# JoeyT1994/TensorNetworkQuantumSimulator.jl

Hardware: AMD Instinct MI355X
Metric: two-site gates/sec at fixed chi (LxL TFIM Trotter layer) (higher is better)
Workload: dtype c64 (ComplexF32; Gram/eigen steps in f64; the chi = 32 plane products as exact bf16 x 3 splits with f32 accumulation, TNQS_NO_BF16X3=1 for f32 matrix instructions)

## Files before the change

### include/tnqs_debug.h

```cpp
#ifndef TNQS_DEBUG_H
#define TNQS_DEBUG_H
#include <stdint.h>
#include "tnqs.h"
#ifdef __cplusplus
extern "C" {
#endif
int tnqs_dbg_jacobi(int dtype, int m, int n, void* A_inout, void* V_out, int* sweeps_out);
int tnqs_dbg_theta_svd_pre(int m, int n, int nq, void* A_inout, const void* Q, void* V_out, int* sweeps_out, int copies, int reps, double* ms_out, double* phase_us_out ,
                           int cap );
int tnqs_dbg_time_jacobi_f32(int m, int n, const void* A, int copies, int reps, double* ms_out, int* sweeps_out);
int tnqs_dbg_chol(int n, const void* G, void* L_out, void* W_out, int* fail_out, double tau);
int tnqs_dbg_fiber_gemm(int dtype, int D, int PA, int K, int PB, int Do, int No, const void* in, const void* X, void* out,
                        double* norm2_out, int use_mfma);
int tnqs_dbg_gram(int dtype, int D, int PA, int K, int PB, const void* X, const void* Y, void* out, int acc64, int use_mfma);
int tnqs_dbg_gram_fused(int PA, int K, int PB, const void* X, const void* Y, const void* M, void* out);
int tnqs_dbg_gauge_gram(int z, const int* chi, int bleg, const void* X, const void* M, void* out);
int tnqs_dbg_pair(int C0, int NMID, int NHI, const void* in, const void* Mx, const void* My, void* out);
int tnqs_dbg_pair_legs(int d, int z, const int* chi, int lx, int ly, const void* in, const void* Mx, const void* My, void* out);
int tnqs_dbg_pair_gram(int d, int z, const int* chi, int lx, int ly, const void* X, const void* Y, const void* M, void* out);
int tnqs_dbg_pair_gram2(int d, int z, const int* chi, int lx, int ly, const void* X, const void* Y, const void* Mx, const void* My, void* out_y, void* out_x);
int tnqs_dbg_bench_plane(int which, int nsites, int lx, int ly, int reps, double* ms);
#define TNQS_DBG_ROUTE_X3 1
#define TNQS_DBG_ROUTE_F32 2
#define TNQS_DBG_ROUTE_F64 3
#define TNQS_DBG_ROUTE_F64_SHARED 4
#define TNQS_DBG_ROUTE_HALF_LINES 5
#define TNQS_DBG_ROUTE_WHOLE_LINES 6
#define TNQS_DBG_ROUTE_SMALL_SCALAR 7
#define TNQS_DBG_ROUTE_SMALL_MFMA16 8
int tnqs_dbg_rowgemm(int D, int K, int nitems, const int* PA, const int* PB, const int* No, const void* in, const void* X, void* out, double* norm2_out,
                     int tpw, int* route_out);
int tnqs_dbg_gram_mfma(int nitems, const int* shape, const void* X, const void* Y, void* out, int nchunks, int* route_out);
int tnqs_dbg_pair16(int d, int nitems, const int* z, const int* chi, const int* lx, const int* ly, const void* in, const void* M, void* out, int spw, int* route_out);
int tnqs_dbg_pair_gram2x16(int d, int nitems, const int* z, const int* chi, const int* lx, const int* ly, const int* both, const void* X, const void* Y, const void* M,
                           void* out_y, void* out_x, int spw);
int tnqs_dbg_svd_tall(int nitems, const int* m, const int* n, void* A, int* chol_fail, int* polished, int* sweeps);
int tnqs_dbg_small_site(int nitems, const int* d, const int* z, const int* chi, const int* jo, const void* psi, const void* M, const int* present, int form,
                        const void* old_msg, const int* has_old, int normalize, void* out, void* new_msg, double* diff_out, int* route_out);
int tnqs_dbg_msg_finalize(int dtype, int nitems, const int* chi, const int* nchunks, const void* partials, const void* old_msg, const int* has_old, int normalize,
                          void* new_msg, double* diff_out);
int tnqs_dbg_default_sequence(tnqs_handle h, int* src, int* dst, int cap, int* n_out);
int tnqs_dbg_default_sequence_graph(int nv, int ne, const int32_t* esrc, const int32_t* edst, int* src, int* dst, int* level, int cap, int* n_out);
int tnqs_dbg_gate_schedule(int nv, int ne, const int32_t* esrc, const int32_t* edst, int ngates, const int32_t* nverts, const int32_t* verts, int update_cache,
                           int* step_of_gate, int* step_is_bp, int cap, int* nsteps_out);
int tnqs_dbg_loop_cgemm(int dtype, int opB, int nitems, const int* m, const int* n, const int* k, const void* A, const void* B, void* C, int guard);
int tnqs_dbg_loop_antiproject(int dtype, int nitems, const int* nr, const int* nc, void* T_inout, const void* f, const void* b);
int tnqs_dbg_loop_trace(int dtype, int nitems, const int* p, const int* q, const void* X, const void* Y, double* out_re_im);
int tnqs_dbg_msg_rescale(int dtype, int nitems, const int* chi, const void* me, const void* mer, const int* present, void* me_out, void* mer_out, int guard);
int tnqs_dbg_edge_scalar(int dtype, int nitems, const int* chi, const void* me, const void* mer, const int* present, double* out_re_im);
int tnqs_dbg_env_prepare(int dtype, int nitems, const int* n, const void* msg, const int* present, void* H_out, void* V_out, int guard);
int tnqs_dbg_env_finish(int dtype, int nitems, const int* n, const void* A, const void* V, const double* cutoff, void* msqrt_out, void* proj_out, int* flags_out, int guard);
int tnqs_dbg_symg_build(int dtype, int nitems, const int* n, const void* AX, const void* VX, const void* AY, const void* VY, double reg, void* rx, void* ry, void* irx, void* iry,
                        void* Ce, void* Ce0, int* flag_out, int guard);
int tnqs_dbg_symg_finish(int dtype, int nitems, const int* n, const void* USigma, const void* Vsvd, const void* irx, const void* iry, void* Xs, void* Xd, double* S, int guard);
int tnqs_dbg_diag(int dtype, int nitems, const int* chi, const double* S, void* out, int guard);
int tnqs_dbg_cscale(int dtype, int nitems, const int* len, const void* src, const double* re, const double* im, void* dst, int guard);
int tnqs_dbg_pending_scale(tnqs_handle h, int v, double* factor);
#ifdef __cplusplus
}
#endif
#endif
```

### tensornetworkquantumsimulator.jl_amd/csrc/api.cpp

```cpp
#include <cmath>
#include <cstring>
#include <string>
#include "engine.hpp"

using namespace tnqs;

struct tnqs_state_s { State* s; };

static thread_local std::string g_err;

template <class F> static int guard(F&& f) {
    try { f(); return TNQS_OK; }
    catch (const Err& e) { g_err = e.what(); return e.code; }
    catch (const std::bad_alloc&) { g_err = "out of host memory"; return TNQS_ERR_HIP; }
    catch (const std::exception& e) { g_err = e.what(); return TNQS_ERR_INVALID; }
    catch (...) { g_err = "unknown error"; return TNQS_ERR_INVALID; }
}
static State* S(tnqs_handle h) { if (!h || !h->s) throw Err(TNQS_ERR_INVALID, "null handle"); return h->s; }

extern "C" {

int tnqs_version(void) { return 102; }
const char* tnqs_last_error(void) { return g_err.c_str(); }
int tnqs_device_count(int* count) {
// ... 208 lines not shown
    return guard([&] { if (nv < 0 || ne < 0 || (ne > 0 && (!esrc || !edst)) || !n_out) throw Err(TNQS_ERR_INVALID, "tnqs_dbg_default_sequence_graph: bad arguments");
                       auto g = dbg_make_graph(nv, ne, esrc, edst); std::vector<int> a, b, l; dbg_default_sequence_graph(*g, a, b, l); *n_out = (int)a.size();
                       for (int i = 0; i < (int)a.size() && i < cap; ++i) { if (src) src[i] = a[i]; if (dst) dst[i] = b[i]; if (level) level[i] = l[i]; } });
}
int tnqs_dbg_gate_schedule(int nv, int ne, const int32_t* esrc, const int32_t* edst, int ngates, const int32_t* nverts, const int32_t* verts, int update_cache,
                           int* step_of_gate, int* step_is_bp, int cap, int* nsteps_out) {
    return guard([&] { if (nv < 0 || ne < 0 || (ne > 0 && (!esrc || !edst)) || ngates < 0 || (ngates > 0 && (!nverts || !verts)) || !nsteps_out) throw Err(TNQS_ERR_INVALID, "tnqs_dbg_gate_schedule: bad arguments");
                       for (int i = 0, o = 0; i < ngates; o += nverts[i], ++i) { if (nverts[i] < 1 || nverts[i] > 2) throw Err(TNQS_ERR_INVALID, "tnqs_dbg_gate_schedule: only one- and two-site gates");
                                                                                 for (int k = 0; k < nverts[i]; ++k) if (verts[o + k] < 0 || verts[o + k] >= nv) throw Err(TNQS_ERR_INVALID, "tnqs_dbg_gate_schedule: vertex out of range"); }
                       auto g = dbg_make_graph(nv, ne, esrc, edst); const GateSchedule steps = build_gate_schedule(*g, ngates, nverts, verts, update_cache != 0); *nsteps_out = (int)steps.size();
                       for (int k = 0; k < (int)steps.size(); ++k) { if (step_is_bp && k < cap) step_is_bp[k] = steps[k].is_bp ? 1 : 0; if (step_of_gate) for (int i = steps[k].begin; i < steps[k].end; ++i) step_of_gate[i] = k; } });
}
int tnqs_dbg_jacobi(int dtype, int m, int n, void* A, void* V, int* sweeps) { return guard([&] { dbg_jacobi(dtype, m, n, A, V, sweeps); }); }
int tnqs_dbg_theta_svd_pre(int m, int n, int nq, void* A, const void* Q, void* V, int* sweeps, int copies, int reps, double* ms, double* phase_us, int cap) { return guard([&] { dbg_theta_svd_pre(m, n, nq, A, Q, V, sweeps, copies, reps, ms, phase_us, cap); }); }
int tnqs_dbg_time_jacobi_f32(int m, int n, const void* A, int copies, int reps, double* ms, int* sweeps) { return guard([&] { dbg_time_jacobi_f32(m, n, A, copies, reps, ms, sweeps); }); }
int tnqs_dbg_chol(int n, const void* G, void* L, void* W, int* fail, double tau) { return guard([&] { dbg_chol(n, G, L, W, fail, tau); }); }
int tnqs_dbg_fiber_gemm(int dtype, int D, int PA, int K, int PB, int Do, int No, const void* in, const void* X, void* out, double* norm2, int use_mfma) {
    return guard([&] { dbg_fiber_gemm(dtype, D, PA, K, PB, Do, No, in, X, out, norm2, use_mfma); });
}
int tnqs_dbg_pair(int C0, int NMID, int NHI, const void* in, const void* Mx, const void* My, void* out) { return guard([&] { dbg_pair(C0, NMID, NHI, in, Mx, My, out); }); }
int tnqs_dbg_pair_legs(int d, int z, const int* chi, int lx, int ly, const void* in, const void* Mx, const void* My, void* out) { return guard([&] { dbg_pair_legs(d, z, chi, lx, ly, in, Mx, My, out); }); }
int tnqs_dbg_pair_gram2(int d, int z, const int* chi, int lx, int ly, const void* X, const void* Y, const void* Mx, const void* My, void* out_y, void* out_x) {
    return guard([&] { dbg_pair_gram2(d, z, chi, lx, ly, X, Y, Mx, My, out_y, out_x); });
}
int tnqs_dbg_bench_plane(int which, int nsites, int lx, int ly, int reps, double* ms) { return guard([&] { dbg_bench_plane(which, nsites, lx, ly, reps, ms); }); }
int tnqs_dbg_pair_gram(int d, int z, const int* chi, int lx, int ly, const void* X, const void* Y, const void* M, void* out) { return guard([&] { dbg_pair_gram(d, z, chi, lx, ly, X, Y, M, out); }); }
int tnqs_dbg_gram_fused(int PA, int K, int PB, const void* X, const void* Y, const void* M, void* out) { return guard([&] { dbg_gram_fused(PA, K, PB, X, Y, M, out); }); }
int tnqs_dbg_gauge_gram(int z, const int* chi, int bleg, const void* X, const void* M, void* out) { return guard([&] { dbg_gauge_gram(z, chi, bleg, X, M, out); }); }
int tnqs_dbg_gram(int dtype, int D, int PA, int K, int PB, const void* X, const void* Y, void* out, int acc64, int use_mfma) {
    return guard([&] { dbg_gram(dtype, D, PA, K, PB, X, Y, out, acc64, use_mfma); });
}
int tnqs_dbg_rowgemm(int D, int K, int nitems, const int* PA, const int* PB, const int* No, const void* in, const void* X, void* out, double* norm2_out, int tpw, int* route_out) {
    return guard([&] { dbg_rowgemm(D, K, nitems, PA, PB, No, in, X, out, norm2_out, tpw, route_out); });
}
int tnqs_dbg_gram_mfma(int nitems, const int* shape, const void* X, const void* Y, void* out, int nchunks, int* route_out) {
    return guard([&] { dbg_gram_mfma(nitems, shape, X, Y, out, nchunks, route_out); });
}
int tnqs_dbg_pair16(int d, int nitems, const int* z, const int* chi, const int* lx, const int* ly, const void* in, const void* M, void* out, int spw, int* route_out) {
    return guard([&] { dbg_pair16(d, nitems, z, chi, lx, ly, in, M, out, spw, route_out); });
}
int tnqs_dbg_pair_gram2x16(int d, int nitems, const int* z, const int* chi, const int* lx, const int* ly, const int* both, const void* X, const void* Y, const void* M,
                           void* out_y, void* out_x, int spw) {
    return guard([&] { dbg_pair_gram2x16(d, nitems, z, chi, lx, ly, both, X, Y, M, out_y, out_x, spw); });
}
int tnqs_dbg_svd_tall(int nitems, const int* m, const int* n, void* A, int* chol_fail, int* polished, int* sweeps) {
    return guard([&] { dbg_svd_tall(nitems, m, n, A, chol_fail, polished, sweeps); });
}
int tnqs_dbg_small_site(int nitems, const int* d, const int* z, const int* chi, const int* jo, const void* psi, const void* M, const int* present, int form,
                        const void* old_msg, const int* has_old, int normalize, void* out, void* new_msg, double* diff_out, int* route_out) {
    return guard([&] { dbg_small_site(nitems, d, z, chi, jo, psi, M, present, form, old_msg, has_old, normalize, out, new_msg, diff_out, route_out); });
}
int tnqs_dbg_msg_finalize(int dtype, int nitems, const int* chi, const int* nchunks, const void* partials, const void* old_msg, const int* has_old, int normalize,
                          void* new_msg, double* diff_out) {
    return guard([&] { dbg_msg_finalize(dtype, nitems, chi, nchunks, partials, old_msg, has_old, normalize, new_msg, diff_out); });
}
int tnqs_dbg_loop_cgemm(int dtype, int opB, int nitems, const int* m, const int* n, const int* k, const void* A, const void* B, void* C, int guard_elems) {
    return guard([&] { dbg_loop_cgemm(dtype, opB, nitems, m, n, k, A, B, C, guard_elems); });
}
int tnqs_dbg_loop_antiproject(int dtype, int nitems, const int* nr, const int* nc, void* T, const void* f, const void* b) { return guard([&] { dbg_loop_antiproject(dtype, nitems, nr, nc, T, f, b); }); }
int tnqs_dbg_loop_trace(int dtype, int nitems, const int* p, const int* q, const void* X, const void* Y, double* out) { return guard([&] { dbg_loop_trace(dtype, nitems, p, q, X, Y, out); }); }
int tnqs_dbg_msg_rescale(int dtype, int nitems, const int* chi, const void* me, const void* mer, const int* present, void* me_out, void* mer_out, int guard_elems) {
    return guard([&] { dbg_msg_rescale(dtype, nitems, chi, me, mer, present, me_out, mer_out, guard_elems); });
}
int tnqs_dbg_edge_scalar(int dtype, int nitems, const int* chi, const void* me, const void* mer, const int* present, double* out_re_im) {
    return guard([&] { dbg_edge_scalar(dtype, nitems, chi, me, mer, present, out_re_im); });
}
int tnqs_dbg_env_prepare(int dtype, int nitems, const int* n, const void* msg, const int* present, void* H_out, void* V_out, int guard_elems) {
    return guard([&] { dbg_env_prepare(dtype, nitems, n, msg, present, H_out, V_out, guard_elems); });
}
int tnqs_dbg_env_finish(int dtype, int nitems, const int* n, const void* A, const void* V, const double* cutoff, void* msqrt_out, void* proj_out, int* flags_out, int guard_elems) {
    return guard([&] { dbg_env_finish(dtype, nitems, n, A, V, cutoff, msqrt_out, proj_out, flags_out, guard_elems); });
}
int tnqs_dbg_symg_build(int dtype, int nitems, const int* n, const void* AX, const void* VX, const void* AY, const void* VY, double reg, void* rx, void* ry, void* irx, void* iry,
                        void* Ce, void* Ce0, int* flag_out, int guard_elems) {
    return guard([&] { dbg_symg_build(dtype, nitems, n, AX, VX, AY, VY, reg, rx, ry, irx, iry, Ce, Ce0, flag_out, guard_elems); });
}
int tnqs_dbg_symg_finish(int dtype, int nitems, const int* n, const void* USigma, const void* Vsvd, const void* irx, const void* iry, void* Xs, void* Xd, double* S, int guard_elems) {
    return guard([&] { dbg_symg_finish(dtype, nitems, n, USigma, Vsvd, irx, iry, Xs, Xd, S, guard_elems); });
}
int tnqs_dbg_diag(int dtype, int nitems, const int* chi, const double* S, void* out, int guard_elems) { return guard([&] { dbg_diag(dtype, nitems, chi, S, out, guard_elems); }); }
int tnqs_dbg_cscale(int dtype, int nitems, const int* len, const void* src, const double* re, const double* im, void* dst, int guard_elems) {
    return guard([&] { dbg_cscale(dtype, nitems, len, src, re, im, dst, guard_elems); });
}
int tnqs_dbg_pending_scale(tnqs_handle h, int v, double* factor) { return guard([&] { if (!factor) throw Err(TNQS_ERR_INVALID, "dbg_pending_scale: null output"); *factor = dbg_pending_scale(S(h), v); }); }
}
```

### tensornetworkquantumsimulator.jl_amd/csrc/engine.hpp

```cpp
#pragma once
#include <hip/hip_runtime_api.h>
#include <climits>
#include <cstdint>
#include <deque>
#include <functional>
#include <map>
#include <memory>
#include <mutex>
#include <stdexcept>
#include <string>
#include <unordered_map>
#include <vector>
#include "../../include/tnqs.h"

namespace tnqs {

struct Err : std::runtime_error {
    int code;
    Err(int c, const std::string& m) : std::runtime_error(m), code(c) {}
};
void hipchk(hipError_t e, const char* what);

class Pool {
public:
// ... 27 lines not shown
    std::vector<std::vector<int>> levels;
    std::vector<int> pos_of;
    std::vector<int> level_of;
    bool in_place = false;
    int nlev = 0;
    std::vector<std::vector<int>> out_level, in_level;
    int levels_until(int L, int from) const { return L > from ? L - from : (L < from ? nlev - from + L : 0); }
    int levels_until_next(int L, int from) const { return L > from ? L - from : nlev - from + L; }
    int horizon(int src, int j, int t) const { const int L = in_level[src][j]; return L < 0 ? INT_MAX : levels_until(L, level_of[t]); }
};

struct Graph {
    int nv = 0, ne = 0;
    std::vector<int> esrc, edst;
    std::vector<std::vector<int>> nbr, nbr_e;
    std::unordered_map<uint64_t, int> emap;
    bool is_tree = false;
    std::vector<int> ecolor; int ncolors = 0;
    mutable std::vector<int> default_seq;
    mutable std::vector<int> default_set_starts;
    mutable std::shared_ptr<const BPPlan> default_plan;
    mutable std::shared_ptr<const BPPlan> forest_plan;
    mutable int spec_penalty = 0;
    int edge(int u, int v) const;
    int leg(int v, int w) const;
    int dedge(int src, int dst) const;
    int src_of(int de) const { return (de & 1) ? edst[de / 2] : esrc[de / 2]; }
    int dst_of(int de) const { return (de & 1) ? esrc[de / 2] : edst[de / 2]; }
};
std::shared_ptr<const BPPlan> plan_for(const Graph& g, const tnqs_bp_opts* o);

struct GateStep { bool is_bp; int begin, end; };
using GateSchedule = std::vector<GateStep>;
struct State;
void validate_gates(const State& s, int ngates, const int32_t* nverts, const int32_t* verts, std::vector<int>& voff, std::vector<size_t>& moff);
GateSchedule build_gate_schedule(const Graph& g, int ngates, const int32_t* nverts, const int32_t* verts, bool update_cache);

struct ProfClass { int64_t launches = 0; double ms = 0, bytes = 0, flops = 0; };
struct Prof {
    bool on = false; ProfClass cls[TNQS_PROF_NCLASSES];
    struct Pending { int cls; hipEvent_t a, b; bool own_a; };
    std::vector<Pending> pending; std::vector<hipEvent_t> ev_free;
    hipEvent_t last_b = nullptr; bool chain = false; hipStream_t last_stream = nullptr;
    ~Prof() { for (auto& p : pending) { if (p.own_a) (void)hipEventDestroy(p.a); (void)hipEventDestroy(p.b); } for (auto e : ev_free) (void)hipEventDestroy(e); }
};

struct RcclComm {
    void* comm = nullptr; int device = 0; void* exch_owned = nullptr;
    long long n_exchanges = 0, bytes_exchanged = 0;
    ~RcclComm();
};

constexpr int kCheckEvents = 16;
struct HostArena {
    char* base = nullptr; size_t cap = 0, off = 0;
    char* ring = nullptr; size_t ring_cap = 0, ring_off = 0;
    hipEvent_t cev[kCheckEvents] = {}; unsigned cevn = 0;
};

struct Check {
    int kind = 0;
    int step = 0;
    int iters_done = 0;
    hipEvent_t ev = nullptr;
    std::function<bool(State*)> eval;
};

struct State {
    std::shared_ptr<Graph> g;
    int dtype = TNQS_C64;
    bool real_io = false;
    int device = 0;
    std::vector<int> d;
    std::vector<char> projected;
    std::vector<int> chi;
    std::vector<Buf> site;
    std::vector<Buf> sscale;
    std::vector<std::vector<double>> pend1; std::vector<char> unit_norm;
    bool in_apply = false;
    std::vector<Buf> msg;
    std::shared_ptr<Pool> pool;
    hipStream_t stream = nullptr; bool own_stream = false;
    hipStream_t aux_stream = nullptr; hipEvent_t ev_fork = nullptr, ev_join = nullptr;
    int rank = 0, nranks = 1; std::vector<int> owner; tnqs_allgather_fn ag_fn = nullptr; void* ag_ctx = nullptr;
    void* exch = nullptr; size_t exch_bytes = 0;
    std::shared_ptr<RcclComm> comm;
    std::shared_ptr<Prof> prof;
    std::vector<Buf> keepalive;
    size_t keep_mark = 0;
    HostArena arena;
    tnqs_apply_stats stats{};
    std::deque<Check> checks;
    int cur_step = -1;

    size_t esz() const { return dtype == TNQS_C64 ? 8 : 16; }
    int scalartype() const { return real_io ? (dtype == TNQS_C64 ? TNQS_F32 : TNQS_F64) : dtype; }
    size_t io_esz() const { return real_io ? esz() / 2 : esz(); }
    bool owns(int v) const { return nranks == 1 || owner[v] == rank; }
    bool force_exchange = false;
    bool msg_hermitian = true;
    bool sharded() const { return nranks > 1 || force_exchange; }
    ~State();
};

State* state_create(int nv, int ne, const int32_t* es, const int32_t* ed, const int32_t* sd, int dtype, int device);
State* state_copy(const State* s);
void state_set_site(State* s, int v, const void* host, int ndim, const int64_t* dims, const int32_t* role);
void state_get_site(State* s, int v, void* host, int ndim, const int32_t* role);
void state_set_site_random(State* s, int v, int nn, const int64_t* bond_dims, uint64_t seed, double scale);
int64_t state_site_size(const State* s, int v);
void state_set_message(State* s, int src, int dst, const void* host, int chi);
void state_get_message(State* s, int src, int dst, void* host, int chi);
void bp_update(State* s, const tnqs_bp_opts* opts, int* niter, double* diff);
void apply_gates(State* s, int ngates, const int32_t* nverts, const int32_t* verts, const double* mats,
                 const tnqs_apply_opts* opts, const tnqs_bp_opts* bp, double* errs);
void truncate_bp(State* s, int maxdim, double cutoff, int normalize, int ngroups, const int32_t* offs,
                 const int32_t* eu, const int32_t* ev, const tnqs_bp_opts* bp);
void rdm_1site(State* s, int v, double* out);
void expect_all(State* s, const double* ops, double* out);
void expect_region(State* s, int nr, const int32_t* rv, const int32_t* parent, const double* ops, double* out4);
void vertex_scalars(State* s, double* out);
void edge_scalars(State* s, double* out);
void rescale(State* s);
void rescale_messages(State* s, int n, const int32_t* eu, const int32_t* ev);
void rescale_vertices(State* s, int n, const int32_t* verts);
void symmetric_gauge(State* s, double regularization);
void site_dim(const State* s, int v, int* d);
void project_site(State* s, int v, int config);
void site_probabilities(State* s, int v, double* out_p);
void sample_bp(State* s, int nsamples, const tnqs_bp_opts* bp, uint64_t seed, const double* uniforms, int32_t* out_config, double* out_prob, tnqs_apply_stats* stats);
void loop_weights(State* s, int ncycles, const int32_t* cycle_len, const int32_t* cycle_verts, double* out_re_im);
void prof_collect(State* s);
void materialize_pending_all(State* s);
void rccl_unique_id(void* out128);
void set_sharding_rccl(State* s, int rank, int nranks, const int32_t* owner, const void* unique_id128, int64_t exch_bytes);
void rccl_allgather(State* s, size_t bytes_per_rank);
void rccl_selftest(int device, int64_t bytes);
void rccl_preflight();

}
```

### tensornetworkquantumsimulator.jl_amd/csrc/engine_batch.cpp

```cpp
#include "engine_internal.hpp"

namespace tnqs {

template <class T> void run_chains(State* s, std::vector<Chain>& chains, int cls, int cls_pair) {
    if (cls_pair < 0) cls_pair = cls;
    const size_t esz = s->esz();
    std::vector<int> nt(chains.size(), 0);
    std::vector<size_t> done(chains.size(), 0);
    for (auto& c : chains) c.result = c.src;
    if (std::is_same<T, float>::value && use_mfma() && use_pair()) {
        std::vector<PairItem> items; double bytes = 0, flops = 0;
        std::vector<std::pair<size_t, std::pair<int, int>>> sel;
        for (size_t ci = 0; ci < chains.size(); ++ci) {
            Chain& c = chains[ci];
            if (c.steps.size() < 2) continue;
            int py = -1, px = -1;
            for (int q = (int)c.steps.size() - 1; q >= 0 && px < 0; --q) {
                int leg = c.steps[q].first;
                bool ok = c.sd.chi[leg] == 32 && leg >= 1 && (c.sd.pre(leg) % 16 == 0);
                if (!ok) continue;
                if (py < 0) py = q; else px = q;
            }
            if (px < 0) continue;
            sel.push_back({ci, {px, py}});
// ... 114 lines not shown
        }
        const int tiles = plan_fiber_gemm(items.data(), (int)items.size(), TR, mf ? tpw : 1);
        const FiberItem* d = upload(s, items);
        ProfScope ps(s, cls, bytes, flops);
        if (mf) launch_mfma_fiber_gemm(s->stream, d, (int)items.size(), tiles, (int)KKmax, (int)KKmax, nullptr);
        else launch_fiber_gemm<T>(s->stream, d, (int)items.size(), tiles, TR, (int)KKmax, nullptr);
    }
    (void)done;
}

void svd_tall(State* s, const std::vector<JacobiItem>& tall, int* d_fail_out, int* d_polish_sweeps) {
    const size_t esz = sizeof(float) * 2;
    const size_t nt = tall.size();
    size_t off = 0; std::vector<size_t> oG(nt), oL(nt), oW(nt), oR0(nt), oRr(nt), oJ(nt), oT(nt);
    for (size_t i = 0; i < nt; ++i) {
        const size_t nn = (size_t)tall[i].n * tall[i].n, mn = (size_t)tall[i].m * tall[i].n;
        oG[i] = off; off += round256(nn * 16); oL[i] = off; off += round256(nn * 16); oW[i] = off; off += round256(nn * 16);
        oR0[i] = off; off += round256(nn * 8); oRr[i] = off; off += round256(nn * 8); oJ[i] = off; off += round256(nn * 16); oT[i] = off; off += round256(mn * 8);
    }
    Buf arena = dalloc(s, off); s->keepalive.push_back(arena);
    Buf fail_buf; if (!d_fail_out) { fail_buf = dalloc(s, nt * sizeof(int)); s->keepalive.push_back(fail_buf); }
    int* const d_fail = d_fail_out ? d_fail_out : reinterpret_cast<int*>(fail_buf->p);
    HIPCHK(hipMemsetAsync(d_fail, 0, nt * sizeof(int), s->stream));
    char* ap = reinterpret_cast<char*>(arena->p);
    std::vector<TallSvdItem> ti, wi; std::vector<CholItem> ci; std::vector<JacobiItem> rj; std::vector<SmallGemmItem> gi; std::vector<CopyItem> cp;
    int nmax = 1, mmax = 1;
    for (size_t i = 0; i < nt; ++i) {
        const int m = tall[i].m, n = tall[i].n; nmax = std::max(nmax, n); mmax = std::max(mmax, m);
        ti.push_back(TallSvdItem{tall[i].A, ap + oG[i], ap + oL[i], ap + oR0[i], ap + oRr[i], m, n});
        ci.push_back(CholItem{ap + oG[i], ap + oL[i], ap + oW[i], n, d_fail + i, 0.0, 1e-14});
        rj.push_back(JacobiItem{ap + oRr[i], nullptr, n, n, tall[i].sweeps_out});
        wi.push_back(TallSvdItem{nullptr, d_fail + i, ap + oW[i], ap + oJ[i], ap + oRr[i], n, n});
        gi.push_back(SmallGemmItem{tall[i].A, ap + oJ[i], ap + oT[i], m, n, n});
        cp.push_back(CopyItem{ap + oT[i], tall[i].A, (size_t)m * n * 8 / 16});
    }
    const TallSvdItem* dt = upload(s, ti); const CholItem* dc = upload(s, ci); const JacobiItem* dj = upload(s, rj);
    const TallSvdItem* dw = upload(s, wi); const SmallGemmItem* dg = upload(s, gi); const CopyItem* dcp = upload(s, cp);
    launch_tall_gram(s->stream, dt, (int)nt, nmax);
    launch_chol_packed(s->stream, dc, (int)nt, nmax);
    launch_tall_rt(s->stream, dt, (int)nt);
    size_t lds = 0; for (auto& j : rj) lds = std::max(lds, jacobi_lds_bytes(j.m, j.n, false, esz));
    launch_jacobi<float>(s->stream, dj, (int)nt, 60, lds, nmax);
    launch_tall_w(s->stream, dw, (int)nt, nmax);
    launch_tall_mj(s->stream, dg, (int)nt);
    launch_copy_items(s->stream, dcp, (int)nt);
    std::vector<JacobiItem> pol;
    for (size_t i = 0; i < nt; ++i) { JacobiItem j{tall[i].A, nullptr, tall[i].m, tall[i].n, d_polish_sweeps ? d_polish_sweeps + i : nullptr}; j.only_if = d_fail + i; pol.push_back(j); }
    const JacobiItem* dp = upload(s, pol);
    launch_jacobi<float>(s->stream, dp, (int)nt, 60, 0, mmax);
    s->stats.n_tall_svd += (int)nt;
}

template <class T> void svd_batch(State* s, const std::vector<JacobiItem>& all, bool with_v) {
    const size_t esz = s->esz();
    const size_t cap = 160 * 1024 - 2048;
    std::vector<JacobiItem> fit, tall, rest, pre;
    static const bool force_global = [] { const char* e = std::getenv("TNQS_JACOBI_GLOBAL"); return e && e[0] == '1'; }();
    for (auto& j : all) {
        if (j.n < 1 || j.m < 1) continue;
        if (j.pre) pre.push_back(j);
        if (!force_global && jacobi_lds_bytes(j.m, j.n, with_v, esz) <= cap && std::max(j.m, j.n) <= 256) fit.push_back(j);
        else if (!force_global && std::is_same<T, float>::value && !with_v && !j.V && use_mfma() && use_chi64() && j.m >= j.n && j.n <= 128 && j.n >= 2 &&
                 jacobi_lds_bytes(j.n, j.n, false, esz) <= cap) tall.push_back(j);
        else rest.push_back(j);
    }
    if (!pre.empty()) {
        const JacobiItem* d = upload_small(s, pre);
        int mm = 1, nn = 1; for (auto& j : pre) { mm = std::max(mm, std::min(j.m, 128)); nn = std::max(nn, std::min(j.n, 64)); }
        launch_theta_svd_pre(s->stream, d, (int)pre.size(), 60, mm, nn);
    }
    if (!fit.empty()) {
        size_t lds = 0; for (auto& j : fit) lds = std::max(lds, jacobi_lds_bytes(j.m, j.n, with_v, esz));
        const JacobiItem* d = upload_small(s, fit);
        int ncols = 1; for (auto& j : fit) ncols = std::max(ncols, j.nhint > 0 ? j.nhint : j.n);
        launch_jacobi<T>(s->stream, d, (int)fit.size(), 60, lds, mmax_of(fit), ncols);
    }
    if (!rest.empty()) {
        const JacobiItem* d = upload(s, rest);
        launch_jacobi<T>(s->stream, d, (int)rest.size(), 60, 0, mmax_of(rest));
    }
    if (!tall.empty()) svd_tall(s, tall);
}

template <class T, class Acc> void run_grams(State* s, std::vector<GramJob>& jobs, int cls) {
    if (jobs.empty()) return;
    const size_t esz = s->esz();
    size_t KKmax = 1;
    for (auto& j : jobs) { j.KK = (j.keep_site ? j.sd.d : 1) * (j.leg >= 0 ? j.sd.chi[j.leg] : 1); KKmax = std::max<size_t>(KKmax, j.KK); }
    constexpr bool f32 = std::is_same<T, float>::value, f32_acc64 = f32 && std::is_same<Acc, double>::value, acc32 = std::is_same<Acc, float>::value;
    bool same = true, f64in = std::is_same<T, double>::value && use_mfma();
    for (auto& j : jobs) { same = same && j.X == j.Y; f64in = f64in && j.M == nullptr && gram_f64in_covers(j.keep_site ? j.sd.d : 1, j.leg >= 0 ? j.sd.chi[j.leg] : 1); }
    GramRoute r = GramRoute::Generic;
    if (jobs[0].M) r = f32_acc64 ? (KKmax == 32 ? GramRoute::Gauge32 : GramRoute::Gauge64) : GramRoute::Fused32;
    else if (f32_acc64 && use_mfma() && same && KKmax <= 64 && KKmax >= 16) r = GramRoute::F64x64;
    else if (f32_acc64 && use_mfma() && use_chi64() && same && KKmax <= 128 && KKmax > 64) r = GramRoute::F64x128;
    else if (f64in) r = GramRoute::F64In;
    else if (f32 && acc32 && use_mfma() && KKmax <= (use_chi64() ? 64 : 32) && KKmax >= 8) r = KKmax <= 32 ? GramRoute::Mfma32 : GramRoute::Mfma64;
    const bool gauge = r == GramRoute::Gauge32 || r == GramRoute::Gauge64;
    const int TR = gram_tile_rows(r, KKmax, esz);
    std::vector<GramItem> items; double bytes = 0, flops = 0; bool all_full = true;
    for (auto& j : jobs) {
        GramItem it{};
        it.X = j.X; it.Y = j.Y; it.M = j.M;
        if (j.leg >= 0) {
            size_t pre = j.sd.pre(j.leg);
            if (j.keep_site) { it.D = j.sd.d; it.PA = (int)(pre / j.sd.d); } else { it.D = 1; it.PA = (int)pre; }
            it.K = j.sd.chi[j.leg]; it.PB = (int)j.sd.post(j.leg);
        } else { it.D = j.sd.d; it.PA = (int)(j.sd.n / j.sd.d); it.K = 1; it.PB = 1; }
        tile_params(it.PA, it.PB, TR, it.TA, it.TB, it.nta, it.ntb);
        if (r == GramRoute::Gauge32) { it.nta = gauge_gram32_units(j.sd.z, j.sd.chi.data(), j.leg); it.ntb = 1; }
        items.push_back(it);
        all_full = all_full && j.KK == (r == GramRoute::F64x128 ? 128 : 64);
        bytes += (j.X == j.Y ? 1.0 : 2.0) * j.sd.n * esz; flops += gauge ? 8.0 * j.sd.n * (j.KK + (r == GramRoute::Gauge32 ? 16.0 : 32.0)) : 8.0 * j.sd.n * j.KK * (j.M ? 2.0 : 1.0);
    }
    std::vector<int> npart(jobs.size());
    const int chunks = plan_gram(items.data(), (int)items.size(), r, f32_acc64, 0, npart.data());
    for (size_t q = 0; q < jobs.size(); ++q) {
        GramJob& j = jobs[q];
        j.nchunks = npart[q];
        j.partial = dalloc(s, (size_t)j.nchunks * j.KK * j.KK * 2 * sizeof(Acc));
        items[q].partial = j.partial->p;
    }
    const GramItem* d = upload(s, items);
    ProfScope ps(s, cls, bytes, flops);
    launch_gram_route<T, Acc>(s->stream, r, d, (int)items.size(), chunks, TR, (int)KKmax, all_full);
}

template void run_chains<float>(State*, std::vector<Chain>&, int, int);
template void run_chains<double>(State*, std::vector<Chain>&, int, int);
template void svd_batch<float>(State*, const std::vector<JacobiItem>&, bool);
template void svd_batch<double>(State*, const std::vector<JacobiItem>&, bool);
template void run_grams<float, float>(State*, std::vector<GramJob>&, int);
template void run_grams<float, double>(State*, std::vector<GramJob>&, int);
template void run_grams<double, double>(State*, std::vector<GramJob>&, int);

}
```

### tensornetworkquantumsimulator.jl_amd/csrc/engine_core.cpp

```cpp
#include "engine_internal.hpp"

namespace tnqs {

double HostTimer::acc[16] = {0}; long HostTimer::cnt[16] = {0};
static struct HostTimerReport { ~HostTimerReport() { if (envflag("TNQS_HOST_TIMING")) for (int k = 0; k < 16; ++k) if (HostTimer::cnt[k])
    std::fprintf(stderr, "[tnqs host timing] phase %d: %.2f ms total, %ld calls, %.1f us each\n", k, HostTimer::acc[k], HostTimer::cnt[k], 1e3 * HostTimer::acc[k] / HostTimer::cnt[k]); } } g_host_timer_report;

void hipchk(hipError_t e, const char* what) {
    if (e != hipSuccess) throw Err(TNQS_ERR_HIP, std::string(what) + ": " + hipGetErrorString(e));
}
void throw_unsupported(const char* what) { throw Err(TNQS_ERR_UNSUPPORTED, what); }

static size_t round_size(size_t b) {
    if (b < 256) return 256;
    if (b <= (1u << 20)) return (b + 255) & ~size_t(255);
    size_t p = size_t(1) << (63 - __builtin_clzll(b));
    size_t step = p >> 3;
    return (b + step - 1) / step * step;
}
Pool::~Pool() { set_defer(false); trim(); }
void Pool::trim() {
    std::lock_guard<std::mutex> lk(mu_);
    for (auto& kv : free_) for (void* p : kv.second) (void)hipFree(p);
    free_.clear(); cached_ = 0;
// ... 32 lines not shown
    const auto& n = nbr[v];
    auto it = std::lower_bound(n.begin(), n.end(), w);
    return (it != n.end() && *it == w) ? int(it - n.begin()) : -1;
}
int Graph::dedge(int src, int dst) const { int e = edge(src, dst); if (e < 0) return -1; return 2 * e + (src == edst[e] ? 1 : 0); }

static std::shared_ptr<Graph> make_graph(int nv, int ne, const int32_t* es, const int32_t* ed) {
    auto g = std::make_shared<Graph>();
    g->nv = nv; g->ne = ne; g->esrc.assign(es, es + ne); g->edst.assign(ed, ed + ne);
    g->nbr.resize(nv); g->nbr_e.resize(nv);
    for (int e = 0; e < ne; ++e) {
        int a = es[e], b = ed[e];
        if (a < 0 || a >= nv || b < 0 || b >= nv || a == b) throw Err(TNQS_ERR_INVALID, "tnqs_create: bad edge endpoints");
        if (g->emap.count(ekey(a, b))) throw Err(TNQS_ERR_INVALID, "tnqs_create: duplicate edge");
        g->emap[ekey(a, b)] = e;
    }
    for (int v = 0; v < nv; ++v) {
        std::vector<std::pair<int, int>> tmp;
        for (int e = 0; e < ne; ++e) { if (es[e] == v) tmp.push_back({ed[e], e}); else if (ed[e] == v) tmp.push_back({es[e], e}); }
        std::sort(tmp.begin(), tmp.end());
        for (auto& p : tmp) { g->nbr[v].push_back(p.first); g->nbr_e[v].push_back(p.second); }
    }
    std::vector<int> par(nv); std::iota(par.begin(), par.end(), 0);
    auto find = [&](int x) { while (par[x] != x) { par[x] = par[par[x]]; x = par[x]; } return x; };
    g->is_tree = true;
    for (int e = 0; e < ne; ++e) { int a = find(es[e]), b = find(ed[e]); if (a == b) { g->is_tree = false; break; } par[a] = b; }
    g->ecolor.assign(ne, -1);
    std::vector<std::vector<char>> used(nv);
    for (int e = 0; e < ne; ++e) {
        int a = es[e], b = ed[e], c = 0;
        for (;; ++c) {
            bool ua = c < (int)used[a].size() && used[a][c], ub = c < (int)used[b].size() && used[b][c];
            if (!ua && !ub) break;
        }
        if ((int)used[a].size() <= c) used[a].resize(c + 1, 0);
        if ((int)used[b].size() <= c) used[b].resize(c + 1, 0);
        used[a][c] = used[b][c] = 1; g->ecolor[e] = c; g->ncolors = std::max(g->ncolors, c + 1);
    }
    return g;
}

std::shared_ptr<Graph> dbg_make_graph(int nv, int ne, const int32_t* es, const int32_t* ed) { return make_graph(nv, ne, es, ed); }

static std::mutex g_recycle_mu;
static std::vector<HostArena> g_spare_arenas;
struct SpareStream { int device; int hi; hipStream_t st; };
static std::vector<SpareStream> g_spare_streams;
static const size_t kMaxSpares = 16;
HostArena acquire_arena() {
    HostArena ar{};
    { std::lock_guard<std::mutex> lk(g_recycle_mu); if (!g_spare_arenas.empty()) { ar = g_spare_arenas.back(); g_spare_arenas.pop_back(); ar.off = 0; ar.ring_off = 0; } }
    if (!ar.base) {
        static const size_t cap = [] { const char* e = std::getenv("TNQS_ARENA_KB"); return e ? std::max<size_t>(16, (size_t)std::atoll(e)) << 10 : size_t(32) << 20; }();
        const size_t ring = size_t(2) << 20;
        HIPCHK(hipHostMalloc((void**)&ar.base, cap + ring, hipHostMallocDefault)); ar.cap = cap - 256;
        ar.ring = ar.base + cap; ar.ring_cap = ring; ar.ring_off = 0;
    }
    return ar;
}
static void arena_free(HostArena& ar) {
    for (hipEvent_t& e : ar.cev) if (e) { (void)hipEventDestroy(e); e = nullptr; }
    if (ar.base) { (void)hipHostFree(ar.base); ar.base = nullptr; }
}
void recycle_arena(HostArena ar) {
    if (!ar.base) return;
    { std::lock_guard<std::mutex> lk(g_recycle_mu); if (g_spare_arenas.size() < kMaxSpares) { ar.off = 0; ar.ring_off = 0; g_spare_arenas.push_back(ar); ar.base = nullptr; } }
    if (ar.base) arena_free(ar);
}
static hipStream_t acquire_stream(int device, int hi = 0) {
    {
        std::lock_guard<std::mutex> lk(g_recycle_mu);
        for (size_t i = 0; i < g_spare_streams.size(); ++i)
            if (g_spare_streams[i].device == device && g_spare_streams[i].hi == hi) { hipStream_t st = g_spare_streams[i].st; g_spare_streams.erase(g_spare_streams.begin() + (std::ptrdiff_t)i); return st; }
    }
    hipStream_t st = nullptr;
    if (hi) { int least = 0, greatest = 0; HIPCHK(hipDeviceGetStreamPriorityRange(&least, &greatest)); HIPCHK(hipStreamCreateWithPriority(&st, hipStreamNonBlocking, greatest)); }
    else HIPCHK(hipStreamCreateWithFlags(&st, hipStreamNonBlocking));
    return st;
}

State::~State() {
    if (own_stream && stream) (void)hipStreamSynchronize(stream);
    if (aux_stream) (void)hipStreamSynchronize(aux_stream);
    keepalive.clear(); site.clear(); msg.clear();
    HostArena ar = arena; arena = HostArena{};
    SpareStream st[2] = {{device, 0, (own_stream && stream) ? stream : nullptr}, {device, 0, aux_stream}};
    {
        std::lock_guard<std::mutex> lk(g_recycle_mu);
        if (ar.base && g_spare_arenas.size() < kMaxSpares) { ar.off = 0; g_spare_arenas.push_back(ar); ar.base = nullptr; }
        for (auto& q : st) if (q.st && g_spare_streams.size() < kMaxSpares) { g_spare_streams.push_back(q); q.st = nullptr; }
    }
    if (ar.base) arena_free(ar);
    for (auto& q : st) if (q.st) (void)hipStreamDestroy(q.st);
    for (hipEvent_t e : {ev_fork, ev_join}) if (e) (void)hipEventDestroy(e);
}
hipStream_t aux_stream_of(State* s) {
    if (!s->aux_stream) {
        s->aux_stream = acquire_stream(s->device);
        HIPCHK(hipEventCreateWithFlags(&s->ev_fork, hipEventDisableTiming));
        HIPCHK(hipEventCreateWithFlags(&s->ev_join, hipEventDisableTiming));
    }
    return s->aux_stream;
}
void sync(State* s) {
    HIPCHK(hipStreamSynchronize(s->stream));
    s->keepalive.clear(); s->keep_mark = 0;
    s->arena.off = 0;
    if (s->prof) s->prof->chain = false;
}

void prof_collect(State* s) {
    Prof& P = *s->prof;
    if (P.pending.empty()) return;
    HIPCHK(hipStreamSynchronize(s->stream));
    for (auto& p : P.pending) {
        float ms = 0; (void)hipEventElapsedTime(&ms, p.a, p.b);
        P.cls[p.cls].ms += ms;
    }
    for (auto& p : P.pending) { if (p.own_a) P.ev_free.push_back(p.a); P.ev_free.push_back(p.b); }
    P.pending.clear(); P.last_b = nullptr; P.chain = false;
}

int64_t state_site_size(const State* s, int v) { return (int64_t)site_dims(s, v).n; }

template <class T> static void fill_product_up(State* s, int v) {
    std::vector<T> h(2 * s->d[v], T(0)); h[0] = T(1);
    Buf b = dalloc(s, s->d[v] * s->esz());
    HIPCHK(hipMemcpyAsync(b->p, h.data(), s->d[v] * s->esz(), hipMemcpyHostToDevice, s->stream));
    HIPCHK(hipStreamSynchronize(s->stream));
    s->site[v] = b;
}

State* state_create(int nv, int ne, const int32_t* es, const int32_t* ed, const int32_t* sd, int dtype, int device) {
    if (nv <= 0 || ne < 0) throw Err(TNQS_ERR_INVALID, "tnqs_create: nv must be > 0 and ne >= 0");
    if (dtype != TNQS_C64 && dtype != TNQS_C128 && dtype != TNQS_F32 && dtype != TNQS_F64) throw Err(TNQS_ERR_INVALID, "tnqs_create: unknown dtype");
    const bool real_io = (dtype == TNQS_F32 || dtype == TNQS_F64);
    if (dtype == TNQS_F32) dtype = TNQS_C64; else if (dtype == TNQS_F64) dtype = TNQS_C128;
    int ndev = 0;
    if (hipGetDeviceCount(&ndev) != hipSuccess || ndev <= 0) throw Err(TNQS_ERR_HIP, "tnqs_create: no HIP device available (the HIP path has no CPU fallback)");
    if (device < 0 || device >= ndev) throw Err(TNQS_ERR_INVALID, "tnqs_create: bad device index");
    HIPCHK(hipSetDevice(device));
    auto s = std::make_unique<State>();
    s->g = make_graph(nv, ne, es, ed);
    s->dtype = dtype; s->real_io = real_io; s->device = device;
    s->d.assign(nv, 2);
    if (sd) for (int v = 0; v < nv; ++v) { if (sd[v] < 1 || sd[v] > 16) throw Err(TNQS_ERR_INVALID, "tnqs_create: site dimension out of range"); s->d[v] = sd[v]; }
    s->chi.assign(ne, 1);
    s->site.resize(nv); s->sscale.assign(nv, nullptr); s->msg.assign(2 * (size_t)ne, nullptr);
    s->pend1.assign(nv, {}); s->unit_norm.assign(nv, 0); s->projected.assign(nv, 0);
    s->pool = std::make_shared<Pool>(device);
    s->prof = std::make_shared<Prof>();
    s->stream = acquire_stream(device); s->own_stream = true;
    for (int v = 0; v < nv; ++v) { if (dtype == TNQS_C64) fill_product_up<float>(s.get(), v); else fill_product_up<double>(s.get(), v); }
    return s.release();
}

State* state_copy(const State* o) {
    auto s = std::make_unique<State>();
    s->g = o->g; s->dtype = o->dtype; s->real_io = o->real_io; s->device = o->device; s->d = o->d; s->chi = o->chi;
    s->site = o->site; s->sscale = o->sscale; s->msg = o->msg; s->pool = o->pool; s->prof = o->prof;
    s->pend1 = o->pend1; s->unit_norm = o->unit_norm; s->projected = o->projected;
    s->rank = o->rank; s->nranks = o->nranks; s->owner = o->owner; s->ag_fn = o->ag_fn; s->ag_ctx = o->ag_ctx;
    s->exch = o->exch; s->exch_bytes = o->exch_bytes; s->comm = o->comm; s->force_exchange = o->force_exchange; s->msg_hermitian = o->msg_hermitian;
    HIPCHK(hipSetDevice(o->device));
    if (o->own_stream) { HIPCHK(hipStreamSynchronize(o->stream)); s->stream = acquire_stream(o->device); s->own_stream = true; }
    else { s->stream = o->stream; s->own_stream = false; }
    return s.release();
}

template <class T> static void permute_dispatch(State* s, const PermItem& it) { launch_permute<T>(s->stream, it); }

static std::vector<char> widen_real(const State* s, const void* host, size_t n) {
    std::vector<char> out(n * s->esz());
    if (s->dtype == TNQS_C64) { const float* p = static_cast<const float*>(host); float* q = reinterpret_cast<float*>(out.data()); for (size_t i = 0; i < n; ++i) { q[2 * i] = p[i]; q[2 * i + 1] = 0.f; } }
    else { const double* p = static_cast<const double*>(host); double* q = reinterpret_cast<double*>(out.data()); for (size_t i = 0; i < n; ++i) { q[2 * i] = p[i]; q[2 * i + 1] = 0.0; } }
    return out;
}
// ... 146 lines not shown
```

### tensornetworkquantumsimulator.jl_amd/csrc/engine_gates.cpp

```cpp
#include "engine_internal.hpp"

namespace tnqs {

struct Gate1 { int v; const double* mat; };
struct Gate2 { int v1, v2; const double* mat; int index; };

template <class T> static void materialize_scale_t(State* s, const std::vector<int>& verts) {
    std::vector<ScaleItem> sc; std::vector<Buf> outs; std::vector<int> vs;
    for (int v : verts) {
        if (v < 0 || v >= (int)s->site.size() || !s->site[v] || !s->sscale[v]) continue;
        Buf out = dalloc(s, s->site[v]->bytes);
        ScaleItem it{}; it.src = s->site[v]->p; it.dst = out->p; it.n = s->site[v]->bytes / s->esz(); it.factor = reinterpret_cast<const double*>(s->sscale[v]->p);
        sc.push_back(it); outs.push_back(out); vs.push_back(v);
    }
    if (sc.empty()) return;
    HIPCHK(hipSetDevice(s->device));
    const ScaleItem* d = upload(s, sc);
    { ProfScope ps(s, TNQS_PROF_SMALL, 0, 0); launch_scale<T>(s->stream, d, (int)sc.size()); }
    for (size_t i = 0; i < vs.size(); ++i) { s->keepalive.push_back(s->site[vs[i]]); s->keepalive.push_back(s->sscale[vs[i]]); s->site[vs[i]] = outs[i]; s->sscale[vs[i]] = nullptr; }
}
void materialize_scale(State* s, const std::vector<int>& verts) {
    if (s->dtype == TNQS_C64) materialize_scale_t<float>(s, verts); else materialize_scale_t<double>(s, verts);
}
void materialize_scale_all(State* s) {
    std::vector<int> all(s->site.size()); std::iota(all.begin(), all.end(), 0);
    materialize_scale(s, all);
}
template <class T> static void apply_one_site_batch(State* s, const std::vector<Gate1>& gates_in, bool normalize, bool force);
void materialize_pending(State* s, const std::vector<int>& verts) {
    std::vector<std::vector<double>> mats; std::vector<Gate1> gs; std::vector<char> norm_was;
    for (int v : verts) {
        if (v < 0 || v >= (int)s->pend1.size() || s->pend1[v].empty()) continue;
        mats.push_back(std::move(s->pend1[v])); s->pend1[v].clear(); norm_was.push_back(s->unit_norm[v]);
        gs.push_back(Gate1{v, nullptr});
    }
    if (gs.empty()) return;
    for (size_t k = 0; k < gs.size(); ++k) gs[k].mat = mats[k].data();
    HIPCHK(hipSetDevice(s->device));
    if (s->dtype == TNQS_C64) apply_one_site_batch<float>(s, gs, false, true); else apply_one_site_batch<double>(s, gs, false, true);
    for (size_t k = 0; k < gs.size(); ++k) s->unit_norm[gs[k].v] = norm_was[k];
}
void materialize_pending_all(State* s) {
    std::vector<int> all(s->site.size()); std::iota(all.begin(), all.end(), 0);
    materialize_pending(s, all);
}

template <class T> static void norm_and_replace(State* s, const std::vector<int>& verts, const std::vector<Buf>& outs, const Buf& norm_partials,
                                                const std::vector<int>& tile_begin, const std::vector<int>& ntiles, bool normalize) {
    if (normalize) {
        std::vector<NormFactorItem> nf;
        Buf fac = dalloc(s, verts.size() * 256);
        for (size_t i = 0; i < verts.size(); ++i) {
            NormFactorItem it{}; it.norm_partials = reinterpret_cast<const double*>(norm_partials->p) + tile_begin[i]; it.npart = ntiles[i];
            it.factor = reinterpret_cast<double*>(reinterpret_cast<char*>(fac->p) + 256 * i);
            nf.push_back(it);
        }
        const NormFactorItem* d = upload_small(s, nf);
        { ProfScope ps(s, TNQS_PROF_SMALL, 0, 0); launch_norm_factor(s->stream, d, (int)nf.size()); }
        for (size_t i = 0; i < verts.size(); ++i) { s->site[verts[i]] = outs[i]; s->sscale[verts[i]] = sub_buffer(fac, 256 * i, 8); }
    } else {
        for (size_t i = 0; i < verts.size(); ++i) s->site[verts[i]] = outs[i];
    }
}

static bool is_unitary(const double* m, int d, double tol) {
    for (int a = 0; a < d; ++a) for (int b = 0; b < d; ++b) {
        double re = 0, im = 0;
        for (int t = 0; t < d; ++t) { const double* x = m + 2 * (t + d * a); const double* y = m + 2 * (t + d * b); re += x[0] * y[0] + x[1] * y[1]; im += x[0] * y[1] - x[1] * y[0]; }
        if (std::fabs(re - (a == b ? 1.0 : 0.0)) > tol || std::fabs(im) > tol) return false;
    }
    return true;
}
static std::vector<double> matmul_dd(const double* a, const double* b, int d) {
    std::vector<double> c(2 * (size_t)d * d, 0.0);
    for (int i = 0; i < d; ++i) for (int j = 0; j < d; ++j) {
        double re = 0, im = 0;
        for (int t = 0; t < d; ++t) { const double* x = a + 2 * (i + d * t); const double* y = b + 2 * (t + d * j); re += x[0] * y[0] - x[1] * y[1]; im += x[0] * y[1] + x[1] * y[0]; }
        c[2 * (i + d * j)] = re; c[2 * (i + d * j) + 1] = im;
    }
    return c;
}

template <class T> static void apply_one_site_batch(State* s, const std::vector<Gate1>& gates_in, bool normalize, bool force) {
    if (gates_in.empty()) return;
    const size_t esz = s->esz();
    std::vector<std::vector<double>> composed; composed.reserve(gates_in.size());
    std::vector<Gate1> gates;
    const bool may_defer = !force && defer_site1() && (!s->sharded() || s->in_apply);
    const double utol = s->dtype == TNQS_C64 ? 1e-6 : 1e-13;
    for (auto& g1 : gates_in) {
        const int d = s->d[g1.v];
        std::vector<double>& pend = s->pend1[g1.v];
        if (may_defer && is_unitary(g1.mat, d, utol) && (!normalize || s->unit_norm[g1.v])) {
            pend = pend.empty() ? std::vector<double>(g1.mat, g1.mat + 2 * (size_t)d * d) : matmul_dd(g1.mat, pend.data(), d);
            s->stats.n_deferred_1site += 1;
            continue;
        }
        if (!pend.empty()) { composed.push_back(matmul_dd(g1.mat, pend.data(), d)); pend.clear(); gates.push_back(Gate1{g1.v, composed.back().data()}); }
        else gates.push_back(g1);
        s->unit_norm[g1.v] = normalize ? 1 : 0;
    }
    if (gates.empty()) return;
    if (std::is_same<T, float>::value) {
        bool all2 = true; for (auto& g1 : gates) all2 = all2 && s->d[g1.v] == 2;
        if (all2) {
            const int NBX = 64;
            std::vector<Site1Item> items; std::vector<int> verts, tb, nt; std::vector<Buf> outs; double bytes = 0, flops = 0;
            for (auto& g1 : gates) {
                if (!s->owns(g1.v)) continue;
                SD sd = site_dims(s, g1.v);
                Site1Item it{}; Buf out = dalloc(s, sd.n * esz);
                it.in = s->site[g1.v]->p; it.out = out->p; it.npairs = sd.n / 2;
                const double* m = g1.mat;
                it.g[0] = (float)m[0]; it.g[1] = (float)m[1]; it.g[2] = (float)m[4]; it.g[3] = (float)m[5];
                it.g[4] = (float)m[2]; it.g[5] = (float)m[3]; it.g[6] = (float)m[6]; it.g[7] = (float)m[7];
                verts.push_back(g1.v); outs.push_back(out); tb.push_back((int)items.size() * NBX); nt.push_back(NBX);
                items.push_back(it);
                bytes += 2.0 * sd.n * esz; flops += 8.0 * sd.n * 2;
            }
            if (items.empty()) return;
            Buf np = dalloc(s, items.size() * NBX * sizeof(double));
            const Site1Item* d = upload(s, items);
            { ProfScope ps(s, TNQS_PROF_GATE_APPLY, bytes, flops);
              launch_site1_c64(s->stream, d, (int)items.size(), NBX, normalize ? reinterpret_cast<double*>(np->p) : nullptr); }
            norm_and_replace<T>(s, verts, outs, np, tb, nt, normalize);
            return;
        }
    }
    std::vector<FiberItem> items; std::vector<int> verts, tb, nt; std::vector<Buf> outs;
    size_t KKmax = 1; double bytes = 0, flops = 0;
    for (auto& g1 : gates) KKmax = std::max<size_t>(KKmax, s->d[g1.v]);
    const int TR = pick_TR(KKmax, esz, 1);
    std::vector<T> hx;
    std::vector<size_t> xoff;
    for (auto& g1 : gates) {
        int d = s->d[g1.v]; xoff.push_back(hx.size());
        for (int nn = 0; nn < d; ++nn) for (int kk = 0; kk < d; ++kk) { hx.push_back((T)g1.mat[2 * (nn + d * kk)]); hx.push_back((T)g1.mat[2 * (nn + d * kk) + 1]); }
    }
    const char* dxp;
    {
        std::vector<char> raw(reinterpret_cast<char*>(hx.data()), reinterpret_cast<char*>(hx.data()) + hx.size() * sizeof(T));
        dxp = upload(s, raw);
    }
    size_t gi = 0;
// ... 15 lines not shown
    const FiberItem* d = upload(s, items);
    { ProfScope ps(s, TNQS_PROF_GATE_APPLY, bytes, flops);
      launch_fiber_gemm<T>(s->stream, d, (int)items.size(), tiles, TR, (int)KKmax, reinterpret_cast<double*>(np->p)); }
    norm_and_replace<T>(s, verts, outs, np, tb, nt, normalize);
}

static std::vector<Gate2> absorb_pending(const State* s, const std::vector<Gate2>& gates_in, std::vector<std::vector<double>>& absorbed) {
    absorbed.reserve(gates_in.size());
    std::vector<Gate2> gates = gates_in;
    for (auto& g2 : gates) {
        const std::vector<double>& p1 = s->pend1[g2.v1]; const std::vector<double>& p2 = s->pend1[g2.v2];
        if (p1.empty() && p2.empty()) continue;
        const int d1 = s->d[g2.v1], d2 = s->d[g2.v2], dd = d1 * d2;
        std::vector<double> kron(2 * (size_t)dd * dd, 0.0);
        for (int t1 = 0; t1 < d1; ++t1) for (int s1 = 0; s1 < d1; ++s1) for (int t2 = 0; t2 < d2; ++t2) for (int s2 = 0; s2 < d2; ++s2) {
            const double ar = p1.empty() ? (t1 == s1 ? 1.0 : 0.0) : p1[2 * (t1 + d1 * s1)], ai = p1.empty() ? 0.0 : p1[2 * (t1 + d1 * s1) + 1];
            const double br = p2.empty() ? (t2 == s2 ? 1.0 : 0.0) : p2[2 * (t2 + d2 * s2)], bi = p2.empty() ? 0.0 : p2[2 * (t2 + d2 * s2) + 1];
            const size_t e = (size_t)(t1 * d2 + t2) + (size_t)dd * (s1 * d2 + s2);
            kron[2 * e] = ar * br - ai * bi; kron[2 * e + 1] = ar * bi + ai * br;
        }
        absorbed.push_back(matmul_dd(g2.mat, kron.data(), dd));
        g2.mat = absorbed.back().data();
    }
    return gates;
}

static int operator_sum(const double* mat, int d1, int d2, std::vector<std::complex<double>>& fa, std::vector<std::complex<double>>& fb) {
    const int dd = d1 * d2, na = d1 * d1, nb = d2 * d2;
    std::vector<std::complex<double>> O((size_t)na * nb);
    const std::complex<double>* gm = reinterpret_cast<const std::complex<double>*>(mat);
    double amax = 0;
    for (int s1p = 0; s1p < d1; ++s1p) for (int s1 = 0; s1 < d1; ++s1) for (int s2p = 0; s2p < d2; ++s2p) for (int s2 = 0; s2 < d2; ++s2) {
        auto v = gm[(s1p * d2 + s2p) + (size_t)dd * (s1 * d2 + s2)];
        O[(s1p + d1 * s1) + (size_t)na * (s2p + d2 * s2)] = v; amax = std::max(amax, std::abs(v));
    }
    int kp = 0;
    for (; kp < std::min(na, nb); ++kp) {
        int pi = 0, pj = 0; double best = 0;
        for (int j = 0; j < nb; ++j) for (int i = 0; i < na; ++i) { double a = std::abs(O[i + (size_t)na * j]); if (a > best) { best = a; pi = i; pj = j; } }
        if (!(best > 1e-13 * amax)) break;
        const std::complex<double> piv = O[pi + (size_t)na * pj];
        std::vector<std::complex<double>> col(na), row(nb);
        for (int i = 0; i < na; ++i) col[i] = O[i + (size_t)na * pj];
        for (int j = 0; j < nb; ++j) row[j] = O[pi + (size_t)na * j] / piv;
        for (int j = 0; j < nb; ++j) for (int i = 0; i < na; ++i) O[i + (size_t)na * j] -= col[i] * row[j];
        fa.insert(fa.end(), col.begin(), col.end()); fb.insert(fb.end(), row.begin(), row.end());
    }
    return kp;
}

struct ReadBack {
    size_t info = 0, low = 0, low2 = 0, terr = 0, chol = 0, env = 0, total = 0;
    ReadBack(size_t ngates, size_t nsites, size_t nflags)
        : low(round256(ngates * 32)), low2(low + round256(ngates * 4)), terr(low2 + round256(ngates * 4)), chol(terr + round256(ngates * 8)),
          env(chol + round256(nsites * sizeof(int))), total(env + round256(nflags * sizeof(int))) {}
    const int* info_of(const char* st) const { return reinterpret_cast<const int*>(st + info); }
    const double* terr_of(const char* st) const { return reinterpret_cast<const double*>(st + terr); }
    const int* chol_of(const char* st) const { return reinterpret_cast<const int*>(st + chol); }
    const int* env_of(const char* st) const { return reinterpret_cast<const int*>(st + env); }
};

struct GateBook {
    int index, cap, d1, d2, K, chi_cap; bool low;
    void book(tnqs_apply_stats& st, const int* hi) const {
        int Mr, Nc, ncolJ; theta_dims(hi, d1, d2, Mr, Nc, ncolJ);
        st.n_lowrank_svd += (ncolJ < Nc) ? 1 : 0; st.n_svd_sweeps += hi[4]; st.n_svd_sweeps_max = std::max(st.n_svd_sweeps_max, hi[4]);
        const int r1d = hi[0] * d1, r2d = hi[1] * d2;
        if (low && ncolJ == Nc && r1d >= r2d && K < r2d && chi_cap <= K) st.n_lowrank_fallbacks += 1;
    }
};

template <class T> static void launch_small_svd(hipStream_t st, const SmallSvdItem* ds, const JacobiItem* dj, const std::vector<JacobiItem>& sji) {
    launch_small_svd_prepare<T>(st, ds, (int)sji.size());
    size_t lds = 0; for (auto& j : sji) lds = std::max(lds, jacobi_lds_bytes(j.m, j.n, false, 16));
    launch_jacobi<double>(st, dj, (int)sji.size(), 60, jacobi_lds(lds), mmax_of(sji));
    launch_small_svd_finish(st, ds, (int)sji.size());
}
template <class T> static void launch_eigen_from_identity(State* s, const EnvItem* di, const JacobiItem* dj, const std::vector<JacobiItem>& ji) {
    size_t lds = 0; for (auto& j : ji) lds = std::max(lds, jacobi_lds_bytes(j.n, j.n, true, 16));
    { ProfScope ps(s, TNQS_PROF_SMALL, 0, 0); launch_env_prepare<T>(s->stream, di, (int)ji.size()); }
    { ProfScope ps(s, TNQS_PROF_JACOBI, 0, 0); launch_jacobi<double>(s->stream, dj, (int)ji.size(), 60, jacobi_lds(lds), mmax_of(ji)); }
}

enum class ReadRoute { deferred, one_trip, two_trips };

template <class T> struct TwoSiteBatch {
    static constexpr bool F32 = std::is_same<T, float>::value;
    struct SiteJob { int v, other, bleg; bool owned; SD sd; std::vector<int> env_idx; std::vector<int> env_leg; };
    struct EnvRec { int de; int n; void *H, *V, *msq, *prj; };
    struct GateWS { Buf lam1, lam2, idx1, idx2, theta, thetaV, theta0, X1, X2, S, lowA, lowB, lowG, lowL, lowW, lowQ, lowB1, lowG2, lowL2, lowLc; int n1, n2, chi, cap; };
    struct RgGroup { int kk = 0; std::vector<FiberItem> sub; std::vector<int> sv, stb, snt; std::vector<Buf> so; int wgs = 0; Buf npr; const FiberItem* d = nullptr; };
    struct RgPlan { bool valid = false; std::vector<RgGroup> groups; std::vector<char> via; double rby = 0, rfl = 0; };

    State* s; const Graph& g; const tnqs_apply_opts& ao; double* errs;
    const size_t esz; const bool sharded;
    const bool qr2;
    bool may_defer = false; double sqrt_cutoff = 0;
    std::vector<std::vector<double>> absorbed; std::vector<Gate2> gates; int ng;
    std::vector<SiteJob> sj; std::vector<char> part;
    std::vector<EnvRec> envs; Buf env_arena;
    std::vector<int> own_idx;
    std::vector<Chain> chains; std::vector<const void*> fused_M, gauged_of; std::vector<GramJob> jobs;
    std::vector<Buf> GA, GV, GW; std::vector<char> is_chol, is_small, small_done;
    hipEvent_t ev_small = nullptr;
    std::vector<size_t> slot; size_t stride = 0; std::vector<char> cross;
    ReadBack rb{0, 0, 0}; Buf d_rb, d_texp; const char* st_all = nullptr;
    std::vector<int> h_flags, h_cholfail, hinfo, info; std::vector<double> hterr, terr;
    std::vector<GateWS> ws; std::vector<int> pg; int npg = 0;
    std::vector<GateItem> gitems; const GateItem* d_gitems = nullptr; bool lowrank_on_batch = false; int cap_max = 1; size_t x2_max = 0;
    ReadRoute route = ReadRoute::two_trips;
    RgPlan spec_plan;
    std::vector<const double*> Sptr; Buf S_keep;
    std::vector<Chain> pch;

    TwoSiteBatch(State* st, const std::vector<Gate2>& gates_in, const tnqs_apply_opts& o, double* e, bool allow_spec)
        : s(st), g(*st->g), ao(o), errs(e), esz(st->esz()), sharded(st->sharded()), qr2(!F32 && use_qr2()), ng((int)gates_in.size()) {
        may_defer = allow_spec && !sharded && ao.maxdim > 0 && !qr2;
        for (size_t k = 0; k < gates_in.size() && may_defer; ++k) {
            const int v1 = gates_in[k].v1, v2 = gates_in[k].v2; const int chi = s->chi[g.edge(v1, v2)];
            const int Mr = std::max(s->d[v1], s->d[v2]) * std::max(s->d[v1], s->d[v2]) * chi, Nc = std::min(s->d[v1], s->d[v2]) * std::min(s->d[v1], s->d[v2]) * chi;
            may_defer = chi == ao.maxdim && Nc >= chi && Mr <= 256 && jacobi_lds(jacobi_lds_bytes(Mr, Nc, false, esz)) > 0;
        }
        sqrt_cutoff = ao.sqrt_cutoff >= 0 ? ao.sqrt_cutoff : 10.0 * (s->dtype == TNQS_C64 ? 1.1920928955078125e-07 : 2.220446049250313e-16);
        gates = absorb_pending(s, gates_in, absorbed);
    }
    ~TwoSiteBatch() { if (ev_small) (void)hipStreamWaitEvent(s->stream, ev_small, 0); }

    int nof(size_t i) const { return sj[i].sd.d * sj[i].sd.chi[sj[i].bleg]; }
    bool small_shape(size_t i) const { const int n = nof(i); return sj[i].sd.n / (size_t)n < (size_t)n && n <= 256 && use_small_svd(); }
    template <class X> X* dev(size_t off) const { return reinterpret_cast<X*>(reinterpret_cast<char*>(d_rb->p) + off); }
    GateBook book_of(int q) const { const GateItem& it = gitems[q]; return GateBook{gates[pg[q]].index, ws[pg[q]].cap, it.d1, it.d2, it.kappa * it.chi, it.chi_cap, it.lowG != nullptr}; }

    void materialize_inputs() { std::vector<int> vs; for (auto& g2 : gates) { vs.push_back(g2.v1); vs.push_back(g2.v2); } materialize_scale(s, vs); }

    void environments() {
        sj.resize(2 * (size_t)ng); part.assign(ng, 0);
        for (int gi = 0; gi < ng; ++gi) {
            for (int side = 0; side < 2; ++side) {
                SiteJob& j = sj[2 * gi + side];
                j.v = side == 0 ? gates[gi].v1 : gates[gi].v2; j.other = side == 0 ? gates[gi].v2 : gates[gi].v1;
                j.sd = site_dims(s, j.v); j.bleg = g.leg(j.v, j.other); j.owned = s->owns(j.v);
                if (j.owned) part[gi] = 1;
                if (!j.owned) continue;
                for (int l = 0; l < j.sd.z; ++l) {
                    if (l == j.bleg) continue;
                    int de = g.dedge(g.nbr[j.v][l], j.v);
                    if (!s->msg[de]) continue;
                    EnvRec r; r.de = de; r.n = j.sd.chi[l];
                    j.env_idx.push_back((int)envs.size()); j.env_leg.push_back(l);
                    envs.push_back(r);
                }
            }
        }
        for (int gi = 0; gi < ng; ++gi) if (part[gi]) pg.push_back(gi);
        npg = (int)pg.size();
        h_flags.assign(2 * envs.size() + 2, 0); h_cholfail.assign(sj.size(), 0);
        rb = ReadBack((size_t)npg, sj.size(), h_flags.size());
        d_rb = dalloc(s, rb.total);
        std::vector<EnvItem> ei; std::vector<JacobiItem> ji; std::vector<EnvFinishItem> fi;
        size_t env_bytes = 0;
        for (auto& r : envs) { const size_t nn = (size_t)r.n * r.n; env_bytes += 2 * round256(nn * 16) + 2 * round256(nn * esz); }
        env_arena = dalloc(s, std::max<size_t>(256, env_bytes));
        char* ap = reinterpret_cast<char*>(env_arena->p);
        ei.reserve(envs.size()); ji.reserve(envs.size()); fi.reserve(envs.size());
        for (size_t i = 0; i < envs.size(); ++i) {
            EnvRec& r = envs[i]; size_t nn = (size_t)r.n * r.n;
            r.H = ap; ap += round256(nn * 16); r.V = ap; ap += round256(nn * 16); r.msq = ap; ap += round256(nn * esz); r.prj = ap; ap += round256(nn * esz);
            ei.push_back(EnvItem{s->msg[r.de]->p, r.H, r.V, r.n});
            ji.push_back(JacobiItem{r.H, r.V, r.n, r.n, nullptr});
            fi.push_back(EnvFinishItem{r.H, r.V, r.msq, r.prj, r.n, sqrt_cutoff, dev<int>(rb.env) + 2 * i});
        }
        if (envs.empty()) return;
        const EnvItem* de = upload_small(s, ei); const JacobiItem* dj = upload_small(s, ji); const EnvFinishItem* df = upload_small(s, fi);
        { ProfScope ps(s, TNQS_PROF_SMALL, 0, 0); launch_env_prepare<T>(s->stream, de, (int)ei.size()); }
        size_t lds = 0; for (auto& r : envs) lds = std::max(lds, jacobi_lds_bytes(r.n, r.n, true, 16));
        { ProfScope ps(s, TNQS_PROF_JACOBI, 0, 0); launch_jacobi<double>(s->stream, dj, (int)ji.size(), 60, jacobi_lds(lds), mmax_of(ji)); }
        { ProfScope ps(s, TNQS_PROF_SMALL, 0, 0); launch_env_finish<T>(s->stream, df, (int)fi.size()); }
    }

    void gauge() {
        for (size_t i = 0; i < sj.size(); ++i) if (sj[i].owned) own_idx.push_back((int)i);
        chains.resize(own_idx.size());
        fused_M.assign(own_idx.size(), nullptr);
        for (size_t q = 0; q < own_idx.size(); ++q) {
            const SiteJob& j = sj[own_idx[q]];
            Chain& c = chains[q]; c.v = j.v; c.src = s->site[j.v]->p; c.sd = j.sd;
            for (size_t e = 0; e < j.env_idx.size(); ++e) c.steps.push_back({j.env_leg[e], envs[j.env_idx[e]].msq});
            if (!(F32 && use_mfma() && use_pair() && !c.steps.empty() && c.steps[0].first == (j.bleg == 0 ? 1 : 0))) continue;
            const bool bulk = c.steps.size() == 3 && j.sd.n / ((size_t)j.sd.d * j.sd.chi[j.bleg]) >= (size_t)j.sd.d * j.sd.chi[j.bleg] &&
                              gauge_gram64_covers(j.sd.d, j.sd.z, j.sd.chi.data(), j.bleg, c.steps[0].first);
            const bool legs16 = j.sd.n >= (size_t)(1u << 14) && gauge_gram32_covers(j.sd.d, j.sd.z, j.sd.chi.data(), j.bleg, c.steps[0].first);
            if (bulk || legs16) { fused_M[q] = c.steps[0].second; c.steps.erase(c.steps.begin()); }
        }
        if (!may_defer) settle(s, true);
        run_chains<T>(s, chains, TNQS_PROF_GATE_MODEPROD);
        GA.resize(sj.size()); GV.resize(sj.size()); GW.resize(sj.size()); is_chol.assign(sj.size(), 0); is_small.assign(sj.size(), 0); small_done.assign(sj.size(), 0);
        gauged_of.assign(sj.size(), nullptr);
        for (size_t q = 0; q < own_idx.size(); ++q) gauged_of[own_idx[q]] = chains[q].result;
    }

    void add_small_svd(size_t i, std::vector<SmallSvdItem>& si, std::vector<JacobiItem>& sji) {
        const int n = nof(i); const size_t Nout = sj[i].sd.n / (size_t)n;
        Buf M = dalloc(s, (size_t)n * Nout * 16); s->keepalive.push_back(M);
        const SD& sd = sj[i].sd; const int b = sj[i].bleg;
        si.push_back(SmallSvdItem{gauged_of[i], M->p, GA[i]->p, GV[i]->p, sd.d, (int)(sd.pre(b) / sd.d), sd.chi[b], (int)sd.post(b)});
        sji.push_back(JacobiItem{M->p, nullptr, n, (int)Nout, nullptr});
    }

    void early_small_svd() {
        if (sharded) return;
        std::vector<SmallSvdItem> si; std::vector<JacobiItem> sji;
        for (size_t q = 0; q < own_idx.size(); ++q) {
            const size_t i = own_idx[q];
            if (!small_shape(i) || fused_M[q]) continue;
            const int n = nof(i);
            GA[i] = dalloc(s, (size_t)n * n * 16); GV[i] = dalloc(s, (size_t)n * n * 16); GW[i] = GV[i]; is_small[i] = 1; small_done[i] = 1;
            add_small_svd(i, si, sji);
        }
        if (si.empty()) return;
        const SmallSvdItem* ds = upload_small(s, si); const JacobiItem* dj = upload_small(s, sji);
        hipStream_t side = aux_stream_of(s);
        HIPCHK(hipEventRecord(s->ev_fork, s->stream)); HIPCHK(hipStreamWaitEvent(side, s->ev_fork, 0));
        launch_small_svd<T>(side, ds, dj, sji);
        HIPCHK(hipEventRecord(s->ev_join, side)); ev_small = s->ev_join;
    }

    void* my_slot(size_t i) const { return reinterpret_cast<char*>(s->exch) + (size_t)s->rank * stride + slot[i]; }
    Buf gather_grams() {
        exchange(s, stride);
        Buf keep = dalloc(s, std::max<size_t>(256, stride * (size_t)s->nranks));
        HIPCHK(hipMemcpyAsync(keep->p, s->exch, stride * (size_t)s->nranks, hipMemcpyDeviceToDevice, s->stream));
        return keep;
    }
    Buf gathered(const Buf& keep, size_t i) const { return sub_buffer(keep, (size_t)s->owner[sj[i].v] * stride + slot[i], (size_t)nof(i) * nof(i) * 16); }

    void grams() {
        std::vector<int> job_of(own_idx.size(), -1);
        for (size_t q = 0; q < own_idx.size(); ++q) {
            const SiteJob& sjq = sj[own_idx[q]];
            if (small_done[own_idx[q]]) continue;
            GramJob j{}; j.X = chains[q].result; j.Y = chains[q].result; j.sd = sjq.sd; j.leg = sjq.bleg; j.keep_site = true; j.M = fused_M[q];
            job_of[q] = (int)jobs.size(); jobs.push_back(j);
        }
        {
            std::vector<GramJob> jf, jf16, jp; std::vector<size_t> idf, idf16, idp;
            for (size_t q = 0; q < jobs.size(); ++q) {
                if (jobs[q].M && jobs[q].sd.chi[jobs[q].leg] == 16) { jf16.push_back(jobs[q]); idf16.push_back(q); }
                else if (jobs[q].M) { jf.push_back(jobs[q]); idf.push_back(q); } else { jp.push_back(jobs[q]); idp.push_back(q); }
            }
            run_grams<T, double>(s, jf, TNQS_PROF_GATE_GRAM);
            run_grams<T, double>(s, jf16, TNQS_PROF_GATE_GRAM);
            run_grams<T, double>(s, jp, TNQS_PROF_GATE_GRAM);
            for (size_t q = 0; q < jf.size(); ++q) jobs[idf[q]] = jf[q];
            for (size_t q = 0; q < jf16.size(); ++q) jobs[idf16[q]] = jf16[q];
            for (size_t q = 0; q < jp.size(); ++q) jobs[idp[q]] = jp[q];
        }
        slot.assign(sj.size(), 0); cross.assign(sj.size(), 0);
        if (sharded) {
            std::vector<size_t> rank_bytes(s->nranks, 0);
            for (size_t i = 0; i < sj.size(); ++i) {
                if (s->owner[sj[i].v] == s->owner[sj[i].other]) continue;
                cross[i] = 1;
                int r = s->owner[sj[i].v]; slot[i] = rank_bytes[r]; rank_bytes[r] += round256((size_t)nof(i) * nof(i) * 16);
            }
            for (size_t b : rank_bytes) stride = std::max(stride, b);
            if (stride) check_exchange(s, stride);
        }
        std::vector<ReduceItem> ri; int elems = 0;
        for (size_t q = 0; q < own_idx.size(); ++q) {
            if (job_of[q] < 0) continue;
            const GramJob& jb = jobs[job_of[q]];
            size_t i = own_idx[q]; int n = jb.KK; size_t nn = (size_t)n * n;
            GA[i] = dalloc(s, nn * 16);
            ri.push_back(ReduceItem{jb.partial->p, cross[i] ? my_slot(i) : GA[i]->p, (int)nn, jb.nchunks, 1, elems}); elems += (int)nn;
        }
        const ReduceItem* dr = upload(s, ri);
        { ProfScope ps(s, TNQS_PROF_SMALL, 0, 0); launch_reduce<double, double>(s->stream, dr, (int)ri.size(), elems); }
        if (sharded && stride) {
            Buf keep = gather_grams();
            for (size_t i = 0; i < sj.size(); ++i) if (part[i / 2] && cross[i]) GA[i] = gathered(keep, i);
        }
    }

    void factor_G(bool allow_chol, bool fallback = false) {
        std::vector<JacobiItem> ji, sji; std::vector<EnvItem> idn; std::vector<CholItem> ci; std::vector<SmallSvdItem> si; int cmax = 1;
        int* d_cholfail = dev<int>(rb.chol);
        if (!fallback) HIPCHK(hipMemsetAsync(d_cholfail, 0, std::max<size_t>(1, sj.size()) * sizeof(int), s->stream));
        for (size_t i = 0; i < sj.size(); ++i) {
            if (!part[i / 2] || small_done[i]) continue;
            if (fallback && !(is_chol[i] && h_cholfail[i])) continue;
            int n = nof(i);
            if (!GV[i]) GV[i] = dalloc(s, (size_t)n * n * 16);
            const size_t Nout = sj[i].sd.n / (size_t)n;
            const bool ch = allow_chol && n <= (use_chi64() ? 128 : 96) && Nout >= (size_t)n;
            is_chol[i] = ch ? 1 : 0;
            if (!ch && sj[i].owned && Nout < (size_t)n && n <= 256 && use_small_svd()) {
                GW[i] = GV[i]; is_small[i] = 1;
                add_small_svd(i, si, sji);
                continue;
            }
            if (ch) {
                GW[i] = dalloc(s, (size_t)n * n * 16);
                ci.push_back(CholItem{GA[i]->p, GV[i]->p, GW[i]->p, n, d_cholfail + i, qr2 ? 1e-15 : rank_tau(F32, n)}); cmax = std::max(cmax, n);
            } else {
                GW[i] = GV[i];
                idn.push_back(EnvItem{nullptr, GV[i]->p, GV[i]->p, n});
                ji.push_back(JacobiItem{GA[i]->p, GV[i]->p, n, n, nullptr});
            }
        }
        if (!si.empty()) {
            const SmallSvdItem* ds = upload_small(s, si); const JacobiItem* dj = upload_small(s, sji);
            ProfScope ps(s, TNQS_PROF_JACOBI, 0, 0);
            launch_small_svd<T>(s->stream, ds, dj, sji);
        }
        if (!ci.empty()) {
            const CholItem* dc = upload_small(s, ci); ProfScope ps(s, TNQS_PROF_JACOBI, 0, 0);
            if (cmax <= 96) launch_chol(s->stream, dc, (int)ci.size(), cmax); else launch_chol_packed(s->stream, dc, (int)ci.size(), cmax);
        }
        if (!ji.empty()) {
            const EnvItem* di = upload_small(s, idn); const JacobiItem* dj = upload_small(s, ji);
            launch_eigen_from_identity<T>(s, di, dj, ji);
        }
    }

    void gate_items() {
        ws.resize(ng); gitems.resize(pg.size());
        for (int gi = 0; gi < ng; ++gi) {
            GateWS& w = ws[gi];
            const SiteJob& a = sj[2 * gi]; const SiteJob& b = sj[2 * gi + 1];
            int chi = a.sd.chi[a.bleg];
            w.n1 = a.sd.d * chi; w.n2 = b.sd.d * chi; w.chi = chi;
            int Mr = w.n1 * a.sd.d, Nc = w.n2 * b.sd.d;
            if (Mr > 512 || Nc > 512) throw Err(TNQS_ERR_UNSUPPORTED, "two-site gate: d^2*chi > 512 is not supported by the theta SVD kernels");
            int cap = std::min(Mr, Nc); if (ao.maxdim > 0) cap = std::min(cap, ao.maxdim);
            w.cap = cap; cap_max = std::max(cap_max, cap);
// ... 56 lines not shown
            it.theta = w.theta->p; it.thetaV = w.thetaV->p; it.theta0 = w.theta0->p; it.X1 = w.X1->p; it.X2 = w.X2->p; it.S = (double*)w.S->p;
            it.maxdim = ao.maxdim; it.cutoff = ao.cutoff; it.normalize = ao.normalize_tensors; it.chi_cap = cap;
            auto site_tau = [&](size_t i, int n) { return (qr2 && !small_shape(i)) ? -rank_tau(false, n) : rank_tau(F32, n); };
            it.tau1 = site_tau(2 * (size_t)gi, w.n1); it.tau2 = site_tau(2 * (size_t)gi + 1, w.n2); it.rk1 = nullptr; it.rk2 = nullptr;
        }
        d_texp = dalloc(s, std::max<size_t>(1, (size_t)npg * sizeof(int)));
        for (int q = 0; q < npg; ++q) {
            gitems[q].info = dev<int>(rb.info) + 8 * q; gitems[q].truncerr = dev<double>(rb.terr) + q;
            gitems[q].lowfail = dev<const int>(rb.low) + q; gitems[q].texp = reinterpret_cast<int*>(d_texp->p) + q;
        }
        d_gitems = upload(s, gitems);
    }

    void run_theta() {
        HIPCHK(hipMemsetAsync(d_rb->p, 0, rb.terr, s->stream));
        ProfScope ps(s, TNQS_PROF_SMALL, 0, 0);
        launch_gate_theta<T>(s->stream, d_gitems, npg);
        if (lowrank_on_batch) launch_gate_theta_mm<T>(s->stream, d_gitems, npg);
        std::vector<CholItem> lc, lc2; int kmax = 1;
        std::vector<GateItem> g2, g3; std::vector<LowQr2Item> qi;
        for (int q = 0; q < npg; ++q) {
            if (!gitems[q].lowG) continue;
            const int K = gitems[q].kappa * gitems[q].chi; GateWS& w = ws[pg[q]];
            int* fail1 = dev<int>(rb.low) + q;
            lc.push_back(CholItem{gitems[q].lowG, const_cast<void*>(gitems[q].lowL), (K <= 96 || !F32) ? w.lowW->p : nullptr, K, fail1, !F32 ? 1e-12 : rank_tau(true, K)});
            kmax = std::max(kmax, K);
            if (!F32) {
                int* fail2 = dev<int>(rb.low2) + q;
                lc2.push_back(CholItem{w.lowG2->p, w.lowL2->p, nullptr, K, fail2, 1e-3});
                GateItem a = gitems[q]; a.lowB = w.lowB1->p; a.lowG = w.lowG2->p; a.lowL = w.lowL2->p; g2.push_back(a);
                GateItem b = gitems[q]; b.lowL = w.lowLc->p; g3.push_back(b);
                qi.push_back(LowQr2Item{w.lowB->p, w.lowW->p, w.lowB1->p, gitems[q].lowL, w.lowL2->p, w.lowLc->p, gitems[q].info, gitems[q].d2, fail1, fail2});
            }
        }
        if (!lc.empty()) {
            const CholItem* dc = upload_small(s, lc); launch_lowrank_g(s->stream, d_gitems, npg);
            if (kmax <= 96) launch_chol(s->stream, dc, (int)lc.size(), kmax); else launch_chol_packed(s->stream, dc, (int)lc.size(), kmax);
            if (F32) launch_lowrank_m<T>(s->stream, d_gitems, npg);
            else {
                const LowQr2Item* dq = upload_small(s, qi); const GateItem* d2 = upload_small(s, g2); const GateItem* d3 = upload_small(s, g3); const CholItem* dc2 = upload_small(s, lc2);
                launch_lowrank_bw(s->stream, dq, (int)qi.size());
                launch_lowrank_g(s->stream, d2, (int)g2.size());
                if (kmax <= 96) launch_chol(s->stream, dc2, (int)lc2.size(), kmax); else launch_chol_packed(s->stream, dc2, (int)lc2.size(), kmax);
                launch_lowrank_ll(s->stream, dq, (int)qi.size());
                launch_lowrank_m<T>(s->stream, d3, (int)g3.size());
            }
        }
        launch_theta_scale<T>(s->stream, d_gitems, npg);
    }

    void svd_and_finish(const int* dims) {
        std::vector<JacobiItem> ji; std::vector<int> ncfull;
        for (int q = 0; q < npg; ++q) {
            int gi = pg[q];
            JacobiItem j{};
            if (dims) {
                int Mr, Nc, ncolJ; theta_dims(dims + 8 * q, gitems[q].d1, gitems[q].d2, Mr, Nc, ncolJ);
                j = JacobiItem{ws[gi].theta->p, ws[gi].thetaV->p, Mr, ncolJ, gitems[q].info + 4};
                ncfull.push_back(Nc);
            } else {
                const int Mr = std::max(ws[gi].n1 * gitems[q].d1, ws[gi].n2 * gitems[q].d2), Nc = std::min(ws[gi].n1 * gitems[q].d1, ws[gi].n2 * gitems[q].d2);
                j = JacobiItem{ws[gi].theta->p, ws[gi].thetaV->p, Mr, Nc, gitems[q].info + 4, gitems[q].info, gitems[q].d1, gitems[q].d2,
                               gitems[q].lowG ? gitems[q].kappa * gitems[q].chi : 0};
                if (F32 && use_precond_svd()) {
                    auto rub = [&](size_t i) { const int n = nof(i); return (int)std::min<size_t>((size_t)n, sj[i].sd.n / (size_t)n); };
                    const int a1 = rub(2 * (size_t)gi) * gitems[q].d1, a2 = rub(2 * (size_t)gi + 1) * gitems[q].d2;
                    if (gitems[q].lowQ) { j.QB = gitems[q].lowQ; j.Vout = ws[gi].thetaV->p; j.pre = 2; }
                    else if (theta_svd_pre_covers(std::max(a1, a2), std::min(a1, a2))) { j.Vout = ws[gi].thetaV->p; j.pre = 1; }
                    j.cap = ws[gi].cap;
                }
                ncfull.push_back(Nc);
            }
            j.V = nullptr;
            ji.push_back(j);
        }
        { ProfScope ps(s, TNQS_PROF_JACOBI, 0, 0); svd_batch<T>(s, ji, false); }
        std::vector<RecoverItem> rv;
        for (int q = 0; q < npg; ++q) rv.push_back(RecoverItem{ws[pg[q]].theta0->p, ws[pg[q]].theta->p, ws[pg[q]].thetaV->p, ji[q].m, ncfull[q], ji[q].n, ji[q].dyn, ji[q].dm, ji[q].dn, ji[q].pre});
        const RecoverItem* dr = upload_small(s, rv);
        { ProfScope ps(s, TNQS_PROF_JACOBI, 0, 0); { int nmax = 1; for (int nc : ncfull) nmax = std::max(nmax, nc); if (F32 && use_mfma()) launch_recover_v_mfma(s->stream, dr, npg, nmax); else launch_recover_v<T>(s->stream, dr, npg, nmax); } }
        { ProfScope ps(s, TNQS_PROF_SMALL, 0, 0); launch_gate_finish<T>(s->stream, d_gitems, npg); }
    }

    void read_results() {
        st_all = readback<char>(s, d_rb->p, rb.total);
        HIPCHK(hipStreamSynchronize(s->stream)); drained(s);
        if (npg) { const int* a = rb.info_of(st_all); const double* b = rb.terr_of(st_all);
                   std::copy(a, a + (size_t)npg * 8, hinfo.begin()); std::copy(b, b + npg, hterr.begin()); }
    }
    void read_and_settle() {
        read_results();
        if (!envs.empty()) std::copy(rb.env_of(st_all), rb.env_of(st_all) + 2 * envs.size(), h_flags.begin());
        if (!sj.empty()) std::copy(rb.chol_of(st_all), rb.chol_of(st_all) + sj.size(), h_cholfail.begin());
        settle(s, true);
    }
    void retheta() {
        d_gitems = upload(s, gitems);
        run_theta();
        if (npg) HIPCHK(hipMemcpyAsync(hinfo.data(), dev<int>(rb.info), (size_t)npg * 32, hipMemcpyDeviceToHost, s->stream));
        HIPCHK(hipStreamSynchronize(s->stream)); drained(s);
    }
    bool chol_failures() const { for (size_t i = 0; i < sj.size(); ++i) if (part[i / 2] && is_chol[i] && h_cholfail[i]) return true; return false; }
    void redo_with_eigen() {
        factor_G(false, true);
        for (int q = 0; q < npg; ++q) { int gi = pg[q]; GateItem& it = gitems[q]; it.GW1 = GW[2 * gi]->p; it.GW2 = GW[2 * gi + 1]->p; it.chol1 = is_chol[2 * gi]; it.chol2 = is_chol[2 * gi + 1]; }
        retheta();
        s->stats.n_chol_fallbacks += 1;
    }

    void second_pass() {
        std::vector<size_t> rs; std::vector<int> rq;
        for (int q = 0; q < npg; ++q) for (int side = 0; side < 2; ++side) {
            const size_t i = 2 * (size_t)pg[q] + side;
            if (((hinfo[8 * q + 6] >> side) & 1) && !small_shape(i)) { rs.push_back(i); rq.push_back(q); }
        }
        if (!sharded && rs.empty()) return;
        const size_t m = rs.size();
        std::vector<Buf> X1(m), Q1(m), G2(m), V2(m), GVn(m), GWn(m); Buf d_rk = dalloc(s, std::max<size_t>(1, m) * sizeof(int));
        std::vector<Qr2RinvItem> ri; std::vector<FiberItem> fi; std::vector<GramJob> gj; std::vector<size_t> own_k; size_t KKmax = 1;
        for (size_t k = 0; k < m; ++k) {
            const size_t i = rs[k]; const int q = rq[k]; const bool second = (i & 1) != 0; const int n = nof(i); const size_t nn = (size_t)n * n;
            X1[k] = dalloc(s, nn * 16); V2[k] = dalloc(s, nn * 16); GVn[k] = dalloc(s, nn * 16); GWn[k] = dalloc(s, nn * 16);
            ri.push_back(Qr2RinvItem{GW[i]->p, second ? gitems[q].lam2 : gitems[q].lam1, second ? gitems[q].idx2 : gitems[q].idx1, gitems[q].info + (second ? 1 : 0), n, X1[k]->p});
            if (sj[i].owned) { own_k.push_back(k); KKmax = std::max<size_t>(KKmax, (size_t)n); Q1[k] = dalloc(s, sj[i].sd.n * esz); }
        }
        const int TR = pick_TR(KKmax, esz, 1);
        for (size_t k : own_k) {
            const size_t i = rs[k]; const SiteJob& j = sj[i]; const int chi = j.sd.chi[j.bleg];
            FiberItem it{}; it.in = gauged_of[i]; it.out = Q1[k]->p; it.X = X1[k]->p;
            it.D = j.sd.d; it.PA = (int)(j.sd.pre(j.bleg) / j.sd.d); it.K = chi; it.PB = (int)j.sd.post(j.bleg); it.Do = j.sd.d; it.No = chi;
            fi.push_back(it);
            GramJob g2{}; g2.X = Q1[k]->p; g2.Y = Q1[k]->p; g2.sd = j.sd; g2.leg = j.bleg; g2.keep_site = true; gj.push_back(g2);
        }
        if (m) { const Qr2RinvItem* d = upload(s, ri); ProfScope ps(s, TNQS_PROF_SMALL, 0, 0); launch_qr2_rinv(s->stream, d, (int)m); }
        if (!fi.empty()) {
            const int tiles = plan_fiber_gemm(fi.data(), (int)fi.size(), TR, 1);
            Buf np = dalloc(s, std::max(1, tiles) * sizeof(double)); const FiberItem* d = upload(s, fi);
            { ProfScope ps(s, TNQS_PROF_GATE_APPLY, 0, 0); launch_fiber_gemm<T>(s->stream, d, (int)fi.size(), tiles, TR, (int)KKmax, reinterpret_cast<double*>(np->p)); }
            s->keepalive.push_back(np);
            run_grams<T, double>(s, gj, TNQS_PROF_GATE_GRAM);
            std::vector<ReduceItem> rd; int elems = 0;
            for (size_t t = 0; t < own_k.size(); ++t) {
                const size_t k = own_k[t], i = rs[k]; const int nn = gj[t].KK * gj[t].KK;
                void* dst;
                if (cross[i]) dst = my_slot(i);
                else { G2[k] = dalloc(s, (size_t)nn * 16); dst = G2[k]->p; }
                rd.push_back(ReduceItem{gj[t].partial->p, dst, nn, gj[t].nchunks, 1, elems}); elems += nn;
            }
            const ReduceItem* d2 = upload(s, rd); ProfScope ps(s, TNQS_PROF_SMALL, 0, 0); launch_reduce<double, double>(s->stream, d2, (int)rd.size(), elems);
        }
        if (sharded && stride) {
            Buf keep = gather_grams();
            for (size_t k = 0; k < m; ++k) if (cross[rs[k]]) G2[k] = gathered(keep, rs[k]);
        }
        if (!m) return;
        std::vector<EnvItem> idn; std::vector<JacobiItem> ji;
        for (size_t k = 0; k < m; ++k) { const int n = nof(rs[k]); idn.push_back(EnvItem{nullptr, V2[k]->p, V2[k]->p, n}); ji.push_back(JacobiItem{G2[k]->p, V2[k]->p, n, n, nullptr}); }
        const EnvItem* di = upload(s, idn); const JacobiItem* dj = upload(s, ji);
        launch_eigen_from_identity<T>(s, di, dj, ji);
        std::vector<Qr2ComposeItem> ci;
        for (size_t k = 0; k < m; ++k) {
            const size_t i = rs[k]; const int q = rq[k]; const bool second = (i & 1) != 0; const int n = nof(i);
            ci.push_back(Qr2ComposeItem{G2[k]->p, V2[k]->p, X1[k]->p, GV[i]->p, second ? gitems[q].lam2 : gitems[q].lam1, second ? gitems[q].idx2 : gitems[q].idx1,
                                        gitems[q].info + (second ? 1 : 0), n, rank_tau(false, n), GVn[k]->p, GWn[k]->p, reinterpret_cast<int*>(d_rk->p) + k});
        }
        { const Qr2ComposeItem* d = upload(s, ci); ProfScope ps(s, TNQS_PROF_SMALL, 0, 0); launch_qr2_compose(s->stream, d, (int)m); }
        for (size_t k = 0; k < m; ++k) {
            const size_t i = rs[k]; GateItem& it = gitems[rq[k]];
            GV[i] = GVn[k]; GW[i] = GWn[k]; s->keepalive.push_back(X1[k]); if (Q1[k]) s->keepalive.push_back(Q1[k]); s->keepalive.push_back(G2[k]); s->keepalive.push_back(V2[k]);
            if (i & 1) { it.GV2 = GV[i]->p; it.GW2 = GW[i]->p; it.chol2 = 2; it.rk2 = reinterpret_cast<int*>(d_rk->p) + k; }
            else { it.GV1 = GV[i]->p; it.GW1 = GW[i]->p; it.chol1 = 2; it.rk1 = reinterpret_cast<int*>(d_rk->p) + k; }
        }
        s->keepalive.push_back(d_rk);
        retheta();
        for (size_t k = 0; k < m; ++k) s->stats.n_qr2_sites += sj[rs[k]].owned ? 1 : 0;
    }

    void defer(char* stage) {
        std::vector<GateBook> books(npg);
        for (int q = 0; q < npg; ++q) books[q] = book_of(q);
        std::vector<char> chol_site(sj.size(), 0);
        for (size_t i = 0; i < sj.size(); ++i) chol_site[i] = (part[i / 2] && is_chol[i]) ? 1 : 0;
        post_check(s, stage, d_rb->p, rb.total, 0, s->cur_step, 0, [st = (const char*)stage, L = rb, books = std::move(books), chol_site = std::move(chol_site), nenv = envs.size(), errs = errs, qr2 = qr2](State* z) {
            const int* hi = L.info_of(st); const double* ht = L.terr_of(st); const int* fl = L.env_of(st); const int* cf = L.chol_of(st);
            for (size_t q = 0; q < books.size(); ++q) if (hi[8 * q + 2] != books[q].cap || hi[8 * q + 3] != 0 || (qr2 && hi[8 * q + 6] != 0)) return false;
            for (size_t i = 0; i < nenv; ++i) if (!fl[2 * i] || fl[2 * i + 1]) return false;
            for (size_t i = 0; i < chol_site.size(); ++i) if (chol_site[i] && cf[i]) return false;
            for (size_t q = 0; q < books.size(); ++q) {
                books[q].book(z->stats, hi + 8 * q);
                if (errs) errs[books[q].index] = ht[q];
            }
            return true;
        });
        for (size_t i = 0; i < envs.size(); ++i) { h_flags[2 * i] = 1; h_flags[2 * i + 1] = 0; }
        s->stats.n_spec_batches += 1;
    }

    void theta_svd(HostTimer& ht_a, HostTimer& ht_s4) {
        if (ev_small) { HIPCHK(hipStreamWaitEvent(s->stream, ev_small, 0)); ev_small = nullptr; }
        run_theta();
        info.assign(8 * (size_t)ng, 0); terr.assign(ng, 0.0);
        hinfo.assign(8 * (size_t)std::max(1, npg), 0); hterr.assign(std::max(1, npg), 0.0);
        bool one_trip = (!qr2 || may_defer) && npg > 0;
        for (int q = 0; q < npg && one_trip; ++q) {
            const int gi = pg[q];
            const int Mr = std::max(ws[gi].n1 * gitems[q].d1, ws[gi].n2 * gitems[q].d2), Nc = std::min(ws[gi].n1 * gitems[q].d1, ws[gi].n2 * gitems[q].d2);
            one_trip = jacobi_lds(jacobi_lds_bytes(Mr, Nc, false, esz)) > 0 && Mr <= 256;
        }
        const size_t rb_bytes = rb.total + 1024;
        char* stage = (may_defer && one_trip) ? ring_alloc(s, rb.total) : nullptr;
        route = stage ? ReadRoute::deferred : one_trip ? ReadRoute::one_trip : ReadRoute::two_trips;
        auto run_ahead = [&]() {
            svd_and_finish(nullptr);
            if (!sharded && ao.maxdim > 0) spec_plan = plan_epilogue([&](int gi) { return ws[gi].cap; }, [&](size_t q) { return (const void*)s->site[sj[own_idx[q]].v]->p; }, nullptr);
            ht_a.stop(); ht_s4.stop();
        };
        switch (route) {
        case ReadRoute::deferred:
            run_ahead();
            defer(stage);
            break;
        case ReadRoute::one_trip:
            run_ahead();
            reserve_readback(s, rb_bytes);
            read_and_settle();
            if (chol_failures()) { redo_with_eigen(); svd_and_finish(hinfo.data()); read_results(); }
            break;
        case ReadRoute::two_trips:
            reserve_readback(s, rb_bytes);
            ht_a.stop(); ht_s4.stop();
            read_and_settle();
            if (chol_failures()) redo_with_eigen();
            if (qr2) second_pass();
            svd_and_finish(hinfo.data());
            read_results();
            break;
        }
    }

    void book_results() {
        for (size_t i = 0; i < envs.size(); ++i)
            if (h_flags[2 * i + 1]) throw Err(TNQS_ERR_NUMERIC, "simple_update: incoming message has a negative eigenvalue above sqrt_cutoff (DomainError in the reference, src/utils.jl:21)");
        for (int q = 0; q < npg; ++q) {
            if (route == ReadRoute::deferred) { info[8 * (size_t)pg[q] + 2] = ws[pg[q]].cap; continue; }
            const int* hi = hinfo.data() + 8 * q;
            std::copy(hi, hi + 8, info.begin() + 8 * (size_t)pg[q]);
            { static const bool dbg = envflag("TNQS_DEBUG_SWEEPS");
              if (dbg) { int Mr, Nc, ncolJ; theta_dims(hi, gitems[q].d1, gitems[q].d2, Mr, Nc, ncolJ);
                         std::fprintf(stderr, "[tnqs sweeps] gate %d: r1 %d r2 %d theta %d x %d, SVD on %d columns, %d sweeps, chi' %d\n", pg[q], hi[0], hi[1], Mr, Nc, ncolJ, hi[4], hi[2]); } }
            book_of(q).book(s->stats, hi);
            terr[pg[q]] = hterr[q];
        }
    }

    void share_records() {
        Sptr.assign(ng, nullptr);
        if (!sharded) { for (int gi = 0; gi < ng; ++gi) Sptr[gi] = (const double*)ws[gi].S->p; return; }
        std::vector<size_t> slot(ng, 0); std::vector<size_t> rank_bytes(s->nranks, 0);
        for (int gi = 0; gi < ng; ++gi) {
            int r = s->owner[gates[gi].v1]; slot[gi] = rank_bytes[r];
            rank_bytes[r] += round256(32 + (size_t)cap_max * 8 + (s->owner[gates[gi].v1] != s->owner[gates[gi].v2] ? x2_max : 0));
        }
        size_t stride = 0; for (size_t b : rank_bytes) stride = std::max(stride, b);
        check_exchange(s, stride);
        char* base = reinterpret_cast<char*>(s->exch);
        std::vector<RecordPackItem> rp;
        std::vector<int> qof(ng, -1); for (int q = 0; q < npg; ++q) qof[pg[q]] = q;
        for (int gi = 0; gi < ng; ++gi) {
            if (s->owner[gates[gi].v1] != s->rank) continue;
            const SiteJob& b = sj[2 * gi + 1]; const int q = qof[gi];
            const bool straddles = s->owner[gates[gi].v1] != s->owner[gates[gi].v2];
            rp.push_back(RecordPackItem{base + (size_t)s->rank * stride + slot[gi], gitems[q].info, gitems[q].truncerr, reinterpret_cast<const double*>(ws[gi].S->p),
                                        ws[gi].cap, ws[gi].X2->p, straddles ? (long long)((size_t)ws[gi].n2 * b.sd.d * ws[gi].cap * esz / 8) : 0LL, (long long)(32 + (size_t)cap_max * 8)});
        }
        if (!rp.empty()) { const RecordPackItem* d = upload(s, rp); launch_record_pack(s->stream, d, (int)rp.size()); }
        exchange(s, stride);
        S_keep = dalloc(s, std::max<size_t>(256, stride * (size_t)s->nranks));
        HIPCHK(hipMemcpyAsync(S_keep->p, base, stride * (size_t)s->nranks, hipMemcpyDeviceToDevice, s->stream));
        std::vector<double> allhdr(4 * (size_t)std::max(1, ng));
        std::vector<const void*> srcs(ng);
        for (int gi = 0; gi < ng; ++gi) srcs[gi] = reinterpret_cast<char*>(S_keep->p) + (size_t)s->owner[gates[gi].v1] * stride + slot[gi];
        Buf d_hdr = dalloc(s, (size_t)std::max(1, ng) * 32);
        const void* const* d_srcs = upload(s, srcs);
        launch_header_gather(s->stream, d_srcs, ng, reinterpret_cast<double*>(d_hdr->p));
        if (ng) HIPCHK(hipMemcpyAsync(allhdr.data(), d_hdr->p, (size_t)ng * 32, hipMemcpyDeviceToHost, s->stream));
        HIPCHK(hipStreamSynchronize(s->stream)); drained(s);
        for (int gi = 0; gi < ng; ++gi) {
            info[8 * gi + 2] = (int)allhdr[4 * gi]; info[8 * gi + 3] = (int)allhdr[4 * gi + 1]; terr[gi] = allhdr[4 * gi + 2];
            const size_t off = (size_t)s->owner[gates[gi].v1] * stride + slot[gi];
            Sptr[gi] = reinterpret_cast<const double*>(reinterpret_cast<const char*>(S_keep->p) + off + 32);
            const SiteJob& b = sj[2 * gi + 1];
            if (b.owned && s->owner[gates[gi].v1] != s->rank)
                ws[gi].X2 = sub_buffer(S_keep, off + 32 + (size_t)cap_max * 8, (size_t)ws[gi].n2 * b.sd.d * ws[gi].cap * esz);
        }
    }

    template <class ChiOf, class InOf> RgPlan plan_epilogue(ChiOf chi_of, InOf in_of, std::vector<char>* skip) {
        RgPlan P; P.via.assign(own_idx.size(), 0);
        std::vector<FiberItem> rg; std::vector<int> rverts; std::vector<Buf> routs;
        if (F32 && use_mfma())
            for (size_t q = 0; q < own_idx.size(); ++q) {
                if (skip && (*skip)[q]) continue;
                size_t i = own_idx[q]; int gi = (int)i / 2; int chin = chi_of(gi); const SiteJob& j = sj[i];
                FiberItem it{};
                it.D = j.sd.d; it.PA = (int)(j.sd.pre(j.bleg) / j.sd.d); it.K = j.sd.chi[j.bleg]; it.PB = (int)j.sd.post(j.bleg); it.Do = j.sd.d; it.No = chin;
                if (!rowgemm_covers(it) || it.D != 2 || (it.K == 64 && !use_chi64())) continue;
                const size_t nout = j.sd.n / it.K * chin;
                Buf out = dalloc(s, nout * esz);
                it.in = in_of(q); it.out = out->p; it.X = (i & 1) ? ws[gi].X2->p : ws[gi].X1->p;
                rowgemm_tiles(it); it.want_norm = ao.normalize_tensors ? 1 : 0;
                rg.push_back(it); rverts.push_back(j.v); routs.push_back(out);
                P.rby += (double)(j.sd.n + nout) * esz; P.rfl += 8.0 * j.sd.n * j.sd.d * chin; P.via[q] = 1; if (skip) (*skip)[q] = 1;
            }
        for (int kk : {64, 32}) {
            RgGroup G; G.kk = kk;
            for (size_t q = 0; q < rg.size(); ++q) if (rg[q].K == kk) { G.sub.push_back(rg[q]); G.sv.push_back(rverts[q]); G.so.push_back(routs[q]); }
            if (G.sub.empty()) continue;
            G.snt.resize(G.sub.size());
            G.wgs = tnqs::plan_rowgemm(G.sub.data(), (int)G.sub.size(), 32, G.snt.data());
            for (auto& it : G.sub) G.stb.push_back(it.tile_begin);
            G.npr = dalloc(s, (size_t)G.wgs * sizeof(double));
            G.d = upload(s, G.sub);
            P.groups.push_back(std::move(G));
        }
        P.valid = true;
        return P;
    }

    void epilogue() {
        pch.resize(own_idx.size());
        for (size_t q = 0; q < own_idx.size(); ++q) {
            const SiteJob& j = sj[own_idx[q]];
            Chain& c = pch[q]; c.v = j.v; c.src = s->site[j.v]->p; c.sd = j.sd;
            for (size_t e = 0; e < j.env_idx.size(); ++e)
                if (!h_flags[2 * j.env_idx[e]]) c.steps.push_back({j.env_leg[e], envs[j.env_idx[e]].prj});
        }
        run_chains<T>(s, pch, TNQS_PROF_GATE_MODEPROD);
        if (own_idx.empty()) return;
        std::vector<FiberItem> items; std::vector<int> verts, tb, nt; std::vector<Buf> outs;
        size_t KKmax = 1, NNmax = 1; double bytes = 0, flops = 0;
        for (size_t q = 0; q < own_idx.size(); ++q) {
            size_t i = own_idx[q];
            KKmax = std::max<size_t>(KKmax, (size_t)sj[i].sd.d * sj[i].sd.chi[sj[i].bleg]);
            NNmax = std::max<size_t>(NNmax, (size_t)sj[i].sd.d * info[8 * (i / 2) + 2]);
        }
        int TR = pick_TR(KKmax, esz, 1);
        bool mf = false;
        if (F32 && use_mfma() && KKmax >= 8) { int t = mfma_fiber_tile_rows((int)KKmax, (int)NNmax); if (t > 0) { TR = t; mf = true; } }
        const bool f64mf = !F32 && use_mfma() && KKmax >= 4 && KKmax <= 64 && NNmax <= 64;
        std::vector<char> via64(own_idx.size(), 0);
        {
            bool spec_ok = spec_plan.valid;
            for (size_t q = 0; q < own_idx.size() && spec_ok; ++q) { const int gi = (int)own_idx[q] / 2; spec_ok = info[8 * gi + 2] == ws[gi].cap && pch[q].steps.empty() && pch[q].result == s->site[sj[own_idx[q]].v]->p; }
            RgPlan fresh_plan;
            if (!spec_ok) {
                spec_plan = RgPlan{};
                fresh_plan = plan_epilogue([&](int gi) { return info[8 * gi + 2]; }, [&](size_t q) { return pch[q].result; }, &via64);
            } else for (size_t q = 0; q < own_idx.size(); ++q) via64[q] = via64[q] || spec_plan.via[q];
            RgPlan& P = spec_ok ? spec_plan : fresh_plan;
            bool booked = false;
            for (auto& G : P.groups) {
                { ProfScope ps(s, TNQS_PROF_GATE_APPLY, booked ? 0.0 : P.rby, booked ? 0.0 : P.rfl); booked = true; launch_mfma_rowgemm(s->stream, G.d, (int)G.sub.size(), G.wgs, 2, G.kk, reinterpret_cast<double*>(G.npr->p)); }
                norm_and_replace<T>(s, G.sv, G.so, G.npr, G.stb, G.snt, ao.normalize_tensors != 0);
            }
        }
        for (size_t q = 0; q < own_idx.size(); ++q) {
            if (via64[q]) continue;
            size_t i = own_idx[q];
            int gi = (int)i / 2; int chin = info[8 * gi + 2];
            const SiteJob& j = sj[i];
            size_t pre = j.sd.pre(j.bleg), post = j.sd.post(j.bleg);
            int chi = j.sd.chi[j.bleg];
            size_t nout = j.sd.n / chi * chin;
            FiberItem it{}; Buf out = dalloc(s, nout * esz);
            it.in = pch[q].result; it.out = out->p; it.X = (i & 1) ? ws[gi].X2->p : ws[gi].X1->p;
            it.D = j.sd.d; it.PA = (int)(pre / j.sd.d); it.K = chi; it.PB = (int)post; it.Do = j.sd.d; it.No = chin;
            it.want_norm = ao.normalize_tensors ? 1 : 0;
            verts.push_back(j.v); outs.push_back(out); items.push_back(it);
            bytes += (double)(j.sd.n + nout) * esz; flops += 8.0 * j.sd.n * j.sd.d * chin;
        }
        nt.resize(items.size());
        const int tiles = f64mf ? plan_fiber_gemm_f64(items.data(), (int)items.size(), nt.data(), 32)
                                : plan_fiber_gemm(items.data(), (int)items.size(), TR, mf ? (TR == 32 ? 16 : 4) : 1, nt.data());
        for (auto& it : items) tb.push_back(it.tile_begin);
        Buf np = dalloc(s, std::max(1, tiles) * sizeof(double));
        const FiberItem* d = upload(s, items);
        if (!items.empty())
        { ProfScope ps(s, TNQS_PROF_GATE_APPLY, bytes, flops);
          if (f64mf) launch_mfma_fiber_gemm_f64(s->stream, d, (int)items.size(), tiles, (int)KKmax, (int)NNmax, reinterpret_cast<double*>(np->p), true);
          else if (mf) launch_mfma_fiber_gemm(s->stream, d, (int)items.size(), tiles, (int)KKmax, (int)NNmax, reinterpret_cast<double*>(np->p));
          else launch_fiber_gemm<T>(s->stream, d, (int)items.size(), tiles, TR, (int)KKmax, reinterpret_cast<double*>(np->p)); }
        norm_and_replace<T>(s, verts, outs, np, tb, nt, ao.normalize_tensors != 0);
    }

    void bond_messages() {
        std::vector<DiagItem> di;
        for (int gi = 0; gi < ng; ++gi) {
            int e = g.edge(gates[gi].v1, gates[gi].v2); int chin = info[8 * gi + 2];
            s->chi[e] = chin;
            for (int dir = 0; dir < 2; ++dir) {
                Buf m = dalloc(s, (size_t)chin * chin * esz);
                di.push_back(DiagItem{m->p, Sptr[gi], chin});
                s->msg[2 * e + dir] = m;
            }
            if (errs && route != ReadRoute::deferred) errs[gates[gi].index] = terr[gi];
        }
        const DiagItem* d = upload_small(s, di);
        { ProfScope ps(s, TNQS_PROF_SMALL, 0, 0); launch_diag<T>(s->stream, d, (int)di.size()); }
        for (auto& g2 : gates) { s->pend1[g2.v1].clear(); s->pend1[g2.v2].clear(); s->unit_norm[g2.v1] = s->unit_norm[g2.v2] = ao.normalize_tensors ? 1 : 0; }
        s->stats.n_two_site += ng;
    }
};

template <class T> static void apply_two_site_batch(State* s, const std::vector<Gate2>& gates_in, const tnqs_apply_opts& ao, double* errs, bool allow_spec = false) {
    if (gates_in.empty()) return;
    TwoSiteBatch<T> b(s, gates_in, ao, errs, allow_spec);
    PhaseScope phase_scope(s, TNQS_PROF_PHASE_GATE_BATCH);
    HostTimer ht_a(3);
    if (!ao.normalize_tensors) b.materialize_inputs();
    HostTimer ht_s1(8);
    b.environments();
    ht_s1.stop(); HostTimer ht_s2(9);
    b.gauge();
    b.early_small_svd();
    ht_s2.stop(); HostTimer ht_s3(10);
    b.grams();
    b.factor_G(use_chol());
    ht_s3.stop(); HostTimer ht_s4(11);
    b.gate_items();
    b.theta_svd(ht_a, ht_s4);
    { HostTimer ht_b(4); b.book_results(); }
    b.share_records();
    HostTimer ht_c(5);
    for (int gi = 0; gi < b.ng; ++gi) if (b.info[8 * gi + 3] != 0) throw Err(TNQS_ERR_NUMERIC, "simple_update: internal bond capacity exceeded");
    b.epilogue();
    b.bond_messages();
    soft_sync(s);
}

template <class T> static void apply_gates_t(State* s, int ngates, const int32_t* nverts, const int32_t* verts, const double* mats,
                                             const tnqs_apply_opts* opts, const tnqs_bp_opts* bp, double* errs) {
    HIPCHK(hipSetDevice(s->device));
    tnqs_apply_opts ao; ao.maxdim = 0; ao.cutoff = -1; ao.normalize_tensors = 1; ao.sqrt_cutoff = -1; ao.update_cache = 1;
    if (opts) ao = *opts;
    std::vector<int> voff; std::vector<size_t> moff;
    validate_gates(*s, ngates, nverts, verts, voff, moff);
    if (errs) std::fill(errs, errs + ngates, 0.0);
    if (s->real_io) {
        bool cplx = false;
        for (size_t k = 1; k < moff[ngates] && !cplx; k += 2) cplx = mats[k] != 0.0;
        if (cplx) s->real_io = false;
    }
    const GateSchedule steps = build_gate_schedule(*s->g, ngates, nverts, verts, ao.update_cache != 0);
    auto batch = [&](const GateStep& st, bool ahead) {
        std::vector<Gate1> b1; std::vector<Gate2> b2;
        for (int i = st.begin; i < st.end; ++i) {
            const int32_t* vs = verts + voff[i];
            if (nverts[i] == 1) b1.push_back(Gate1{vs[0], mats + moff[i]}); else b2.push_back(Gate2{vs[0], vs[1], mats + moff[i], i});
        }
        apply_one_site_batch<T>(s, b1, ao.normalize_tensors != 0, false);
        apply_two_site_batch<T>(s, b2, ao, errs, ahead);
        s->stats.n_batches += 1;
        soft_sync(s);
    };
    auto update = [&](int iters_before) { bp_update_t<T>(s, bp, nullptr, nullptr, iters_before == 0, iters_before); };
    RunAhead run_ahead(s, steps, batch, update);
    run_ahead.run();
    if (s->sharded()) materialize_pending_all(s);
    sync(s);
}

void apply_gates(State* s, int ngates, const int32_t* nverts, const int32_t* verts, const double* mats,
                 const tnqs_apply_opts* opts, const tnqs_bp_opts* bp, double* errs) {
    s->stats = tnqs_apply_stats{};
    if (s->dtype == TNQS_C64) apply_gates_t<float>(s, ngates, nverts, verts, mats, opts, bp, errs);
    else apply_gates_t<double>(s, ngates, nverts, verts, mats, opts, bp, errs);
}

template <class T> static void truncate_t(State* s, int maxdim, double cutoff, int normalize, int ngroups, const int32_t* offs,
                                          const int32_t* eu, const int32_t* ev, const tnqs_bp_opts* bp) {
    const Graph& g = *s->g;
    HIPCHK(hipSetDevice(s->device));
    if (maxdim <= 0) throw Err(TNQS_ERR_INVALID, "truncate: maxdim must be a positive integer");
    tnqs_apply_opts ao; ao.maxdim = maxdim; ao.cutoff = cutoff; ao.normalize_tensors = normalize; ao.sqrt_cutoff = -1; ao.update_cache = 1;
    std::vector<std::vector<double>> idmats;
    auto ident = [&](int dd) { std::vector<double> m(2 * (size_t)dd * dd, 0.0); for (int i = 0; i < dd; ++i) m[2 * (size_t)(i + (size_t)dd * i)] = 1.0; return m; };
    auto run_group = [&](const std::vector<std::pair<int, int>>& edges) {
        std::vector<Gate2> b2; std::set<int> seen; idmats.clear(); idmats.reserve(edges.size());
        for (auto& pr : edges) {
            int e = g.edge(pr.first, pr.second);
            if (e < 0) throw Err(TNQS_ERR_INVALID, "truncate: colour group contains a non-edge");
            if (s->chi[e] == 1) continue;
            if (seen.count(pr.first) || seen.count(pr.second)) throw Err(TNQS_ERR_INVALID, "truncate: edges of one colour group must be vertex-disjoint");
            seen.insert(pr.first); seen.insert(pr.second);
            idmats.push_back(ident(s->d[pr.first] * s->d[pr.second]));
            b2.push_back(Gate2{pr.first, pr.second, idmats.back().data(), 0});
        }
        apply_two_site_batch<T>(s, b2, ao, nullptr);
        if (!b2.empty()) s->stats.n_batches += 1;
// ... 22 lines not shown
```

### tensornetworkquantumsimulator.jl_amd/csrc/engine_internal.hpp

```cpp
#pragma once
#include "engine.hpp"
#include "kernels.hpp"
#include <algorithm>
#include <array>
#include <chrono>
#include <climits>
#include <cmath>
#include <complex>
#include <cstdio>
#include <cstdlib>
#include <cstring>
#include <functional>
#include <limits>
#include <memory>
#include <mutex>
#include <numeric>
#include <set>
#include <type_traits>
#include <unordered_map>

namespace tnqs {

#define HIPCHK(x) hipchk((x), #x)

inline bool envflag(const char* name) { const char* e = std::getenv(name); return e && e[0] == '1'; }
#define TNQS_SWITCH(fn, expr) inline bool fn() { static const bool v = (expr); return v; }
TNQS_SWITCH(use_mfma, !envflag("TNQS_NO_MFMA"))
TNQS_SWITCH(use_pair, !envflag("TNQS_NO_PAIR"))
TNQS_SWITCH(use_bra_products, !envflag("TNQS_NO_BRA_PRODUCTS"))
TNQS_SWITCH(use_prodcache, !envflag("TNQS_NO_PRODCACHE"))
TNQS_SWITCH(use_chol, !envflag("TNQS_NO_CHOL"))
TNQS_SWITCH(use_qr2, !envflag("TNQS_NO_QR2"))
TNQS_SWITCH(use_lowrank, !envflag("TNQS_NO_LOWRANK"))
TNQS_SWITCH(use_precond_svd, !envflag("TNQS_NO_PRECOND_SVD"))
TNQS_SWITCH(use_small_svd, !envflag("TNQS_NO_SMALLSVD"))
TNQS_SWITCH(defer_site1, !envflag("TNQS_NO_DEFER_1SITE"))
TNQS_SWITCH(use_chi64, !envflag("TNQS_NO_CHI64"))
TNQS_SWITCH(speculation_on, !envflag("TNQS_NO_SPECULATION"))
#undef TNQS_SWITCH
inline size_t bp_cache_budget() { static const size_t v = [] { const char* e = std::getenv("TNQS_BP_CACHE_MB"); return (e ? (size_t)std::atoll(e) : (size_t)49152) << 20; }(); return v; }
inline size_t bp_ws_budget() { static const size_t v = [] { const char* e = std::getenv("TNQS_BP_WS_MB"); return (e ? (size_t)std::atoll(e) : (size_t)24576) << 20; }(); return v; }
inline size_t jacobi_lds(size_t bytes) { static const bool g = envflag("TNQS_JACOBI_GLOBAL"); return (g || bytes > 160 * 1024 - 2048) ? 0 : bytes; }
inline int mmax_of(const std::vector<JacobiItem>& ji) { int m = 1; for (auto& j : ji) m = std::max(m, std::max(j.m, j.n)); return m; }

struct HostTimer {
    static double acc[16]; static long cnt[16];
    int k; std::chrono::steady_clock::time_point t0; bool on;
    explicit HostTimer(int kk) : k(kk), t0(std::chrono::steady_clock::now()), on(true) {}
    void stop() { if (on) { static std::mutex mu; std::lock_guard<std::mutex> lk(mu); acc[k] += std::chrono::duration<double, std::milli>(std::chrono::steady_clock::now() - t0).count(); cnt[k]++; on = false; } }
    ~HostTimer() { stop(); }
};

void sync(State* s);
hipStream_t aux_stream_of(State* s);
void recycle_arena(HostArena ar);
HostArena acquire_arena();
inline void drain_for_arena_reuse(State* s) {
    HIPCHK(hipStreamSynchronize(s->stream));
    if (s->aux_stream && s->aux_stream != s->stream) HIPCHK(hipStreamSynchronize(s->aux_stream));
}
template <class X> const X* readback(State* s, const void* dsrc, size_t count) {
    const size_t bytes = count * sizeof(X);
    HostArena& ar = s->arena;
    if (!ar.base) ar = acquire_arena();
    const size_t aligned = (std::max<size_t>(bytes, 1) + 255) & ~size_t(255);
    if (aligned > ar.cap) throw Err(TNQS_ERR_UNSUPPORTED, "read-back too large for the staging arena");
    if (ar.off + aligned > ar.cap) { drain_for_arena_reuse(s); ar.off = 0; }
    char* h = ar.base + ar.off; ar.off += aligned;
    if (bytes) HIPCHK(hipMemcpyAsync(h, dsrc, bytes, hipMemcpyDeviceToHost, s->stream));
    return reinterpret_cast<const X*>(h);
}
inline void reserve_readback(State* s, size_t bytes) {
    HostArena& ar = s->arena;
    if (!ar.base) ar = acquire_arena();
    if (bytes > ar.cap) throw Err(TNQS_ERR_UNSUPPORTED, "read-backs of one batch too large for the staging arena");
    if (ar.off + bytes > ar.cap) { drain_for_arena_reuse(s); ar.off = 0; }
}
inline void soft_sync(State* s) { s->keep_mark = s->keepalive.size(); }
inline void drained(State* s) {
    s->prof->chain = false;
    s->arena.off = 0;
    if (s->keep_mark) { s->keepalive.erase(s->keepalive.begin(), s->keepalive.begin() + (std::ptrdiff_t)std::min(s->keep_mark, s->keepalive.size())); s->keep_mark = 0; }
}
void materialize_scale(State* s, const std::vector<int>& verts);
void materialize_scale_all(State* s);
void materialize_pending(State* s, const std::vector<int>& verts);
void materialize_pending_all(State* s);
inline Buf dalloc(State* s, size_t bytes) {
    auto b = std::make_shared<DevBuf>();
    b->pool = s->pool; b->bytes = bytes;
    b->p = s->pool->alloc(bytes ? bytes : 1, &b->rounded);
    return b;
}
template <class Item> const Item* upload(State* s, const std::vector<Item>& v) {
    if (v.empty()) return nullptr;
    size_t bytes = v.size() * sizeof(Item);
    HostArena& ar = s->arena;
    if (!ar.base) ar = acquire_arena();
    size_t aligned = (bytes + 255) & ~size_t(255);
    if (aligned > ar.cap) throw Err(TNQS_ERR_UNSUPPORTED, "descriptor batch too large");
    if (ar.off + aligned > ar.cap) { drain_for_arena_reuse(s); ar.off = 0; s->prof->chain = false; }
    char* h = ar.base + ar.off; ar.off += aligned;
    std::memcpy(h, v.data(), bytes);
    Buf b = dalloc(s, bytes);
    HIPCHK(hipMemcpyAsync(b->p, h, bytes, hipMemcpyHostToDevice, s->stream));
    s->keepalive.push_back(b);
    return reinterpret_cast<const Item*>(b->p);
}

template <class Item> const Item* upload_small(State* s, const std::vector<Item>& v) {
    if (v.empty()) return nullptr;
    const size_t bytes = v.size() * sizeof(Item);
    HostArena& ar = s->arena;
    if (!ar.base) ar = acquire_arena();
    const size_t aligned = (bytes + 255) & ~size_t(255);
    if (aligned > ar.cap) throw Err(TNQS_ERR_UNSUPPORTED, "descriptor batch too large");
    if (ar.off + aligned > ar.cap) { drain_for_arena_reuse(s); ar.off = 0; s->prof->chain = false; }
    char* h = ar.base + ar.off; ar.off += aligned;
    std::memcpy(h, v.data(), bytes);
    return reinterpret_cast<const Item*>(h);
}

struct ProfScope {
    State* s; int cls; hipEvent_t a = nullptr, b = nullptr; bool own_a = true;
    ProfScope(State* st, int c, double bytes, double flops) : s(st), cls(c) {
        Prof& P = *s->prof;
        if (!P.on) return;
        P.cls[c].bytes += bytes; P.cls[c].flops += flops; P.cls[c].launches += 1;
        auto get = [&]() { hipEvent_t e; if (!P.ev_free.empty()) { e = P.ev_free.back(); P.ev_free.pop_back(); } else HIPCHK(hipEventCreate(&e)); return e; };
        if (P.chain && P.last_b && P.last_stream == s->stream) { a = P.last_b; own_a = false; }
        else { a = get(); own_a = true; HIPCHK(hipEventRecord(a, s->stream)); }
        b = get();
    }
    ~ProfScope() {
        if (!a) return;
        Prof& P = *s->prof;
        (void)hipEventRecord(b, s->stream);
        P.pending.push_back({cls, a, b, own_a});
        P.last_b = b; P.chain = true; P.last_stream = s->stream;
    }
};

struct PhaseScope {
    State* s; int cls; hipEvent_t a = nullptr, b = nullptr; long count = 1;
    PhaseScope(State* st, int c) : s(st), cls(c) {
        Prof& P = *s->prof;
        if (!P.on) return;
        auto get = [&]() { hipEvent_t e; if (!P.ev_free.empty()) { e = P.ev_free.back(); P.ev_free.pop_back(); } else HIPCHK(hipEventCreate(&e)); return e; };
        a = get(); b = get();
        HIPCHK(hipEventRecord(a, s->stream));
    }
    ~PhaseScope() {
        if (!a) return;
        Prof& P = *s->prof;
        (void)hipEventRecord(b, s->stream);
        P.cls[cls].launches += count;
        P.pending.push_back({cls, a, b, true});
    }
};

struct ChiVec {
    int inl[8]; int n = 0; std::vector<int> big;
    void push_back(int c) { if (n < 8 && big.empty()) inl[n++] = c; else { if (big.empty()) big.assign(inl, inl + n); big.push_back(c); ++n; } }
    int* data() { return big.empty() ? inl : big.data(); }
    const int* data() const { return big.empty() ? inl : big.data(); }
    int& operator[](size_t i) { return data()[i]; }
    const int& operator[](size_t i) const { return data()[i]; }
    size_t size() const { return (size_t)n; }
    bool empty() const { return n == 0; }
    const int* begin() const { return data(); }
    const int* end() const { return data() + n; }
};
struct SD {
    int z = 0, d = 1; ChiVec chi; size_t n = 1;
    size_t pre(int j) const { size_t p = d; for (int i = 0; i < j; ++i) p *= chi[i]; return p; }
    size_t post(int j) const { size_t p = 1; for (int i = j + 1; i < z; ++i) p *= chi[i]; return p; }
};
inline SD site_dims(const State* s, int v) {
    SD r; const Graph& g = *s->g;
    r.z = (int)g.nbr[v].size(); r.d = s->d[v]; r.n = r.d;
    for (int j = 0; j < r.z; ++j) { int c = s->chi[g.nbr_e[v][j]]; r.chi.push_back(c); r.n *= c; }
    return r;
}

inline size_t site_nelem(const State* s, int v) { size_t n = (size_t)s->d[v]; for (int e : s->g->nbr_e[v]) n *= (size_t)s->chi[e]; return n; }
inline size_t round256(size_t b) { return (b + 255) & ~size_t(255); }
void exchange(State* s, size_t bytes_per_rank);
void check_exchange(const State* s, size_t bytes_per_rank);



struct Chain {
    int v = -1; const void* src = nullptr; SD sd;
    const void* y = nullptr;
    std::vector<std::pair<int, const void*>> steps;
    const void* result = nullptr; Buf tmp[2];
    bool ordered = false;
    std::vector<std::vector<int>> trail;
};


struct GramJob {
    const void* X; const void* Y; SD sd; int leg;   bool keep_site;
    Buf partial; int nchunks = 0; int KK = 0;
    const void* M = nullptr;
    Buf final_msg;
};

template <class T> void run_chains(State* s, std::vector<Chain>& chains, int cls, int cls_pair = -1);
template <class T, class Acc> void run_grams(State* s, std::vector<GramJob>& jobs, int cls);
template <class T> void svd_batch(State* s, const std::vector<JacobiItem>& all, bool with_v);
void svd_tall(State* s, const std::vector<JacobiItem>& tall, int* d_fail = nullptr, int* d_polish_sweeps = nullptr);
template <class T> void bp_update_t(State* s, const tnqs_bp_opts* o, int* niter_out, double* diff_out, bool optimistic = false, int iters_before = 0);

constexpr size_t kMaxPendingChecks = 12;
static_assert(kMaxPendingChecks < (size_t)kCheckEvents, "a pending check's event must not be handed out again (HostArena::cev is a ring)");
constexpr int kPenaltySteps = 12;
constexpr size_t kRunAheadMaxSiteBytes = size_t(2) << 30;

struct Snapshot {
    std::vector<int> chi; std::vector<Buf> site, sscale, msg; std::vector<std::vector<double>> pend1; std::vector<char> unit_norm;
    tnqs_apply_stats stats{}; bool real_io = false;
    explicit Snapshot(const State& s) : chi(s.chi), site(s.site), sscale(s.sscale), msg(s.msg), pend1(s.pend1), unit_norm(s.unit_norm), stats(s.stats), real_io(s.real_io) {}
    void restore(State& s) const { s.chi = chi; s.site = site; s.sscale = sscale; s.msg = msg; s.pend1 = pend1; s.unit_norm = unit_norm; s.stats = stats; s.real_io = real_io; }
};
struct SpecFailed { int kind, step, iters_done; };

void settle(State* s, bool block);
char* ring_alloc(State* s, size_t bytes);
void post_check(State* s, char* stage, const void* dsrc, size_t bytes, int kind, int cur_step, int iters_done, std::function<bool(State*)> eval);
void drop_checks(State* s);

struct RunAhead {
    using BatchFn = std::function<void(const GateStep&, bool ahead)>;
    using UpdateFn = std::function<void(int iters_before)>;
    RunAhead(State* s, const GateSchedule& steps, BatchFn batch, UpdateFn update);
    void run();
private:
    State* const s; const Graph& g; const GateSchedule& steps; const BatchFn batch; const UpdateFn update;
    struct InApply { State* s; explicit InApply(State* st) : s(st) { s->in_apply = true; } ~InApply() { s->in_apply = false; s->cur_step = -1; } } in_apply;
    const bool deep;
    std::vector<std::unique_ptr<Snapshot>> snaps;
    size_t k = 0; bool careful = false;
    bool ahead() const { return deep && g.spec_penalty == 0 && !careful; }
    void step();
    void snapshot_in_front();
    void settle_behind(bool was_ahead);
    void drop_old_snaps();
    const Snapshot* snapshot_for(const SpecFailed& f) const;
    void recover(const SpecFailed& f);
    void unwind();
};

}
```

### tensornetworkquantumsimulator.jl_amd/csrc/kernels.hip

```cpp
#include "kernels.hpp"
#include "device_common.hpp"

namespace tnqs {

template <class T, int NB>
__global__ __launch_bounds__(256) void fiber_gemm_kernel(const FiberItem* __restrict__ items, int nitems, int TR,
                                                         double* __restrict__ norm_partials) {
    extern __shared__ __attribute__((aligned(16))) char smem[];
    cx<T>* tile = reinterpret_cast<cx<T>*>(smem);
    __shared__ double sh_red[17];
    const int tid = threadIdx.x;
    int lo = 0, hi = nitems - 1;
    const int gt = blockIdx.x;
    while (lo < hi) { int mid = (lo + hi + 1) >> 1; if (items[mid].tile_begin <= gt) lo = mid; else hi = mid - 1; }
    const FiberItem it = items[lo];
    const int lt = gt - it.tile_begin;
    const int ta = lt % it.nta, tb = lt / it.nta;
    const int a0 = ta * it.TA, b0 = tb * it.TB;
    const int na = min(it.TA, it.PA - a0), nb = min(it.TB, it.PB - b0);
    const int D = it.D, K = it.K, TA = it.TA, TB = it.TB, KK = D * K;
    const size_t PA = it.PA;
    const cx<T>* __restrict__ in = reinterpret_cast<const cx<T>*>(it.in);
    const int ntile_el = D * TA * K * TB;
    for (int e = tid; e < ntile_el; e += 256) {
// ... 68 lines not shown
    const int KB = (KK + 1) >> 1;
    const int nblk = KB * KB;
    const int ntiles = it.nta * it.ntb;
    const int t_begin = lc * it.tiles_per_chunk;
    const int t_end = min(ntiles, t_begin + it.tiles_per_chunk);
    cx<Acc>* __restrict__ part = reinterpret_cast<cx<Acc>*>(it.partial) + (size_t)lc * KK * KK;
    const int ntile_el = D * TA * K * TB;
    for (int pass0 = 0; pass0 < nblk; pass0 += 256 * MAXB) {
        cx<Acc> acc[MAXB][4];
        int bi[MAXB], bj[MAXB];
#pragma unroll
        for (int j = 0; j < MAXB; ++j) {
            int q = pass0 + tid + 256 * j;
            int qq = min(q, nblk - 1);
            bi[j] = qq % KB; bj[j] = qq / KB;
#pragma unroll
            for (int c = 0; c < 4; ++c) acc[j][c] = cmake<Acc>(0, 0);
        }
        for (int t = t_begin; t < t_end; ++t) {
            const int ta = t % it.nta, tb = t / it.nta;
            const int a0 = ta * TA, b0 = tb * TB;
            const int na = min(TA, it.PA - a0), nb = min(TB, it.PB - b0);
            __syncthreads();
            for (int e = tid; e < ntile_el; e += 256) {
                int s = e % D; int r1 = e / D; int al = r1 % TA; int r2 = r1 / TA; int k = r2 % K; int bl = r2 / K;
                cx<T> vx = cmake<T>(0, 0), vy = cmake<T>(0, 0);
                if (al < na && bl < nb) {
                    size_t off = s + D * ((size_t)(a0 + al) + PA * ((size_t)k + (size_t)K * (b0 + bl)));
                    vx = Xg[off];
                    if (!same) vy = Yg[off];
                }
                int li = (al + TA * bl) * KKp + (s + D * k);
                Xt[li] = vx;
                if (!same) Yt[li] = vy;
            }
            for (int e = tid; e < TA * TB; e += 256) { Xt[e * KKp + KK] = cmake<T>(0, 0); if (!same) Yt[e * KKp + KK] = cmake<T>(0, 0); }
            __syncthreads();
            const int nrow = TA * TB;
            for (int rr = 0; rr < nrow; ++rr) {
                const cx<T>* xr = Xt + rr * KKp;
                const cx<T>* yr = Yt + rr * KKp;
#pragma unroll
                for (int j = 0; j < MAXB; ++j) {
                    cx<T> x0 = xr[2 * bi[j]], x1 = xr[2 * bi[j] + 1];
                    cx<T> y0 = yr[2 * bj[j]], y1 = yr[2 * bj[j] + 1];
                    cx<Acc> X0 = cmake<Acc>(x0.re, x0.im), X1 = cmake<Acc>(x1.re, x1.im);
                    cx<Acc> Y0 = cmake<Acc>(y0.re, y0.im), Y1 = cmake<Acc>(y1.re, y1.im);
                    cfma_conj(acc[j][0], X0, Y0); cfma_conj(acc[j][1], X1, Y0);
                    cfma_conj(acc[j][2], X0, Y1); cfma_conj(acc[j][3], X1, Y1);
                }
            }
        }
#pragma unroll
        for (int j = 0; j < MAXB; ++j) {
            int q = pass0 + tid + 256 * j;
            if (q < nblk) {
                int i0 = 2 * bi[j], j0 = 2 * bj[j];
                part[i0 + (size_t)KK * j0] = acc[j][0];
                if (i0 + 1 < KK) part[i0 + 1 + (size_t)KK * j0] = acc[j][1];
                if (j0 + 1 < KK) {
                    part[i0 + (size_t)KK * (j0 + 1)] = acc[j][2];
                    if (i0 + 1 < KK) part[i0 + 1 + (size_t)KK * (j0 + 1)] = acc[j][3];
                }
            }
        }
    }
}

template <class T, class Acc>
void launch_gram(hipStream_t s, const GramItem* d_items, int nitems, int total_chunks, int TR, int KKmax) {
    if (total_chunks <= 0) return;
    size_t lds = 2 * (size_t)TR * (KKmax + 1) * sizeof(cx<T>);
    hipLaunchKernelGGL((gram_kernel<T, Acc, 4>), dim3(total_chunks), dim3(256), lds, s, d_items, nitems, TR); TNQS_CHECK_LAUNCH();
}
template void launch_gram<float, float>(hipStream_t, const GramItem*, int, int, int, int);
template void launch_gram<float, double>(hipStream_t, const GramItem*, int, int, int, int);
template void launch_gram<double, double>(hipStream_t, const GramItem*, int, int, int, int);

int gram_tile_rows(GramRoute r, size_t KKmax, size_t esz) {
    const int tr = pick_TR(KKmax + 1, esz, 2);
    return r == GramRoute::Generic ? tr : r == GramRoute::F64In ? 32 : 64;
}
int plan_gram(GramItem* it, int n, GramRoute r, bool f32_acc64, int max_chunks, int* npart) {
    if (max_chunks <= 0) max_chunks = std::max(1, (f32_acc64 ? 1024 : 2048) / n);
    const int per_chunk = (r == GramRoute::Mfma32 || r == GramRoute::Fused32) ? 4 : (r == GramRoute::F64x64 || r == GramRoute::Gauge64) ? 2 : 1;
    const int chunks = lay_out(it, n, &GramItem::chunk_begin, npart, [&](GramItem& g) {
        const int ntiles = g.nta * g.ntb, nch = std::min(max_chunks, ntiles);
        g.tiles_per_chunk = (ntiles + nch - 1) / nch; g.nchunks = (ntiles + g.tiles_per_chunk - 1) / g.tiles_per_chunk;
        return g.nchunks; });
    if (npart) for (int i = 0; i < n; ++i) npart[i] *= per_chunk;
    return chunks;
}
template <class T, class Acc>
void launch_gram_route(hipStream_t s, GramRoute r, const GramItem* d, int n, int chunks, int TR, int KKmax, bool all_full) {
    switch (r) {
    case GramRoute::Gauge32: launch_mfma_gauge_gram32(s, d, n, chunks); break; case GramRoute::Gauge64: launch_mfma_gauge_gram64(s, d, n, chunks); break;
    case GramRoute::F64x64: launch_mfma_gram64_f64(s, d, n, chunks, KKmax, all_full); break; case GramRoute::F64x128: launch_mfma_gram128_f64(s, d, n, chunks, KKmax, all_full); break;
    case GramRoute::Mfma32: launch_mfma_gram32(s, d, n, chunks, KKmax); break; case GramRoute::Mfma64: launch_mfma_gram64(s, d, n, chunks, KKmax); break;
    case GramRoute::Fused32: launch_mfma_gram32_fused(s, d, n, chunks); break; case GramRoute::F64In: launch_mfma_gram_f64in(s, d, n, chunks); break;
    case GramRoute::Generic: launch_gram<T, Acc>(s, d, n, chunks, TR, KKmax); break;
    }
}
template void launch_gram_route<float, float>(hipStream_t, GramRoute, const GramItem*, int, int, int, int, bool);
template void launch_gram_route<float, double>(hipStream_t, GramRoute, const GramItem*, int, int, int, int, bool);
template void launch_gram_route<double, double>(hipStream_t, GramRoute, const GramItem*, int, int, int, int, bool);

template <class Acc, class Out>
__global__ __launch_bounds__(256) void reduce_kernel(const ReduceItem* __restrict__ items, int nitems, int total) {
    int ge = blockIdx.x * 256 + threadIdx.x;
    if (ge >= total) return;
    int lo = 0, hi = nitems - 1;
    while (lo < hi) { int mid = (lo + hi + 1) >> 1; if (items[mid].elem_begin <= ge) lo = mid; else hi = mid - 1; }
    const ReduceItem it = items[lo];
    int e = ge - it.elem_begin;
    const cx<Acc>* p = reinterpret_cast<const cx<Acc>*>(it.partial);
    Acc re = 0, im = 0;
    for (int c = 0; c < it.nchunks; ++c) { cx<Acc> v = p[(size_t)c * it.n2 + e]; re += v.re; im += v.im; }
    if (it.conj) im = -im;
    reinterpret_cast<cx<Out>*>(it.out)[e] = cmake<Out>((Out)re, (Out)im);
}
template <class Acc, class Out>
void launch_reduce(hipStream_t s, const ReduceItem* d_items, int nitems, int total_elems) {
    if (total_elems <= 0) return;
    hipLaunchKernelGGL((reduce_kernel<Acc, Out>), dim3((total_elems + 255) / 256), dim3(256), 0, s, d_items, nitems, total_elems); TNQS_CHECK_LAUNCH();
}
template void launch_reduce<double, double>(hipStream_t, const ReduceItem*, int, int);
template void launch_reduce<float, float>(hipStream_t, const ReduceItem*, int, int);
template void launch_reduce<double, float>(hipStream_t, const ReduceItem*, int, int);

}
```

### tensornetworkquantumsimulator.jl_amd/csrc/kernels.hpp

```cpp
#pragma once
#include <algorithm>
#include <cstdlib>
#include <hip/hip_runtime_api.h>
#include <cstddef>
#include <cstdint>

namespace tnqs {

struct FiberItem {
    const void* in; void* out; const void* X;
    int D, PA, K, PB;
    int Do, No;
    int TA, TB, nta, ntb;
    int tile_begin;
    int tpw;
    int want_norm;
};

struct GramItem {
    const void* X; const void* Y; void* partial;
    int D, PA, K, PB;
    int TA, TB, nta, ntb;
    int chunk_begin, nchunks, tiles_per_chunk;
    const void* M;
// ... 48 lines not shown

struct EnvItem {
    const void* msg; void* H; void* V; int n;
};
struct EnvFinishItem {
    const void* A; const void* V; void* msqrt; void* proj; int n; double cutoff; int* flags;
};

struct GateItem {
    const void* GA1; const void* GV1; const void* GA2; const void* GV2;
    const void* GW1; const void* GW2; int chol1, chol2;
    int n1, n2;
    int d1, d2, chi;
    const double* gate;
    double* lam1; double* lam2;
    int* idx1; int* idx2;
    void* theta; void* thetaV;
    void* theta0;
    void* X1; void* X2;
    double* S;
    int* info;
    double* truncerr;
    int maxdim; double cutoff; int normalize; int chi_cap;
    double tau1, tau2; const int* rk1; const int* rk2;
    int kappa; const double* opA; const double* opB; void* lowA; void* lowB; void* lowG; const void* lowL; const int* lowfail;
    int* texp;
    const void* lowW; void* lowQ;
};
template <class T> void launch_theta_scale(hipStream_t s, const GateItem* d_items, int nitems);
void launch_lowrank_g(hipStream_t s, const GateItem* d_items, int nitems);
template <class T> void launch_lowrank_m(hipStream_t s, const GateItem* d_items, int nitems);
struct LowQr2Item { const void* B; const void* W1; void* B1; const void* L1; const void* L2; void* Lc; const int* info; int d2; int* fail1; const int* fail2; };
void launch_lowrank_bw(hipStream_t s, const LowQr2Item* d_items, int nitems);
void launch_lowrank_ll(hipStream_t s, const LowQr2Item* d_items, int nitems);
struct Qr2RinvItem { const void* GW; const double* lam; const int* idx; const int* r; int n; void* X1; };
struct Qr2ComposeItem { const void* A2; const void* V2; const void* X1; const void* GV1; const double* lam1; const int* idx1; const int* r1;
                        int n; double tau; void* GVout; void* GWout; int* rk; };
void launch_qr2_rinv(hipStream_t s, const Qr2RinvItem* d_items, int nitems);
void launch_qr2_compose(hipStream_t s, const Qr2ComposeItem* d_items, int nitems);

struct Site1Item { const void* in; void* out; float g[8]; size_t npairs; };
struct DiagItem { void* out; const double* S; int chi; };
struct ScaleItem { const void* src; void* dst; size_t n; const double* factor; };
struct NormFactorItem { const double* norm_partials; int npart; double* factor; };
struct MsgRescaleItem { const void* me; const void* mer; void* me_out; void* mer_out; int chi; };
template <class T> void launch_msg_rescale(hipStream_t s, const MsgRescaleItem* d_items, int nitems);
struct EdgeScalarItem { const void* me; const void* mer; int chi; double* out; };
template <class T> void launch_edge_scalar(hipStream_t s, const EdgeScalarItem* d_items, int nitems);
struct CScaleItem { const void* src; void* dst; size_t n; double re, im; };
template <class T> void launch_cscale(hipStream_t s, const CScaleItem* d_items, int nitems);
struct SymGaugeItem { const void* AX; const void* VX; const void* AY; const void* VY; void* rx; void* ry; void* irx; void* iry;
                      void* Ce; void* Ce0; void* Vsvd; void* Xs; void* Xd; double* S; int n; double reg; int* flag; };
template <class T> void launch_symg_build(hipStream_t s, const SymGaugeItem* d_items, int nitems);
template <class T> void launch_symg_finish(hipStream_t s, const SymGaugeItem* d_items, int nitems);
struct RecordPackItem { void* dst; const int* info; const double* terr; const double* S; int nS; const void* X2; long long x2_words; long long x2_off; };
void launch_record_pack(hipStream_t s, const RecordPackItem* d_items, int nitems);
void launch_header_gather(hipStream_t s, const void* const* d_srcs, int n, double* d_out);
struct PermItem { const void* in; void* out; int ndim; int dims_out[8]; long long stride_in[8]; size_t n; };

template <class Item, class Count> int lay_out(Item* it, int n, int Item::*begin, int* nwg, Count count) {
    int w = 0; for (int i = 0; i < n; ++i) { const int c = count(it[i]); it[i].*begin = w; w += c; if (nwg) nwg[i] = c; } return w;
}
[[noreturn]] void throw_unsupported(const char* what);
inline int pick_TR(size_t KK, size_t esz, int copies) {
    for (int tr : {64, 32, 16, 8, 4}) if (KK * tr * esz * copies <= 64 * 1024) return tr;
    throw_unsupported("bond dimension too large for the fiber-tile kernels (d*chi*16*elemsize must fit 64 KiB of LDS)");
}
inline void tile_params(size_t PA, size_t PB, int TR, int& TA, int& TB, int& nta, int& ntb) {
    TA = (int)std::min<size_t>(PA, TR); TB = std::max(1, TR / TA); TB = (int)std::min<size_t>(TB, PB);
    nta = (int)((PA + TA - 1) / TA); ntb = (int)((PB + TB - 1) / TB);
}

template <class T> void launch_fiber_gemm(hipStream_t s, const FiberItem* d_items, int nitems, int total_tiles,
                                          int TR, int KKmax, double* d_norm_partials);
inline int plan_fiber_gemm(FiberItem* it, int n, int TR, int tpw, int* nwg = nullptr) {
    for (int i = 0; i < n; ++i) tile_params(it[i].PA, it[i].PB, TR, it[i].TA, it[i].TB, it[i].nta, it[i].ntb);
    return lay_out(it, n, &FiberItem::tile_begin, nwg, [&](FiberItem& f) { f.tpw = tpw; return (f.nta * f.ntb + tpw - 1) / tpw; });
}
template <class T, class Acc> void launch_gram(hipStream_t s, const GramItem* d_items, int nitems, int total_chunks,
                                               int TR, int KKmax);
enum class GramRoute { Generic, Mfma32, Mfma64, Fused32, F64x64, F64x128, F64In, Gauge64, Gauge32 };
int gram_tile_rows(GramRoute r, size_t KKmax, size_t esz);
int plan_gram(GramItem* it, int n, GramRoute r, bool f32_acc64, int max_chunks, int* npart);
template <class T, class Acc> void launch_gram_route(hipStream_t s, GramRoute r, const GramItem* d_items, int nitems, int total_chunks, int TR, int KKmax,
                                                     bool all_full = false);
template <class Acc, class Out> void launch_reduce(hipStream_t s, const ReduceItem* d_items, int nitems, int total_elems);
template <class T> void launch_msg_finalize(hipStream_t s, const MsgFinalItem* d_items, int nitems);
struct RecoverItem { const void* A0; const void* A; void* V; int m; int n; int nu; const int* dyn; int dm, dn; int pre;  };
inline size_t jacobi_lds_bytes(int m, int n, bool withV, size_t esz) { return ((size_t)(m + 2) * n + (withV ? (size_t)(n + 2) * n : 0)) * esz; }
template <class T> void launch_jacobi(hipStream_t s, const JacobiItem* d_items, int nitems, int max_sweeps, size_t lds_bytes, int mmax, int ncols = 0);
inline bool theta_svd_pre_covers(int m, int n) { return n >= 2 && n <= 64 && m >= n && m <= 128; }
inline size_t theta_svd_pre_lds_bytes(int m, int n) { return ((((size_t)(m + 2) * n * 8) + 15) & ~(size_t)15) + (size_t)(n + 1) * n * 16; }
void launch_theta_svd_pre(hipStream_t s, const JacobiItem* d_items, int nitems, int max_sweeps, int mmax, int nmax);
struct SmallSvdItem { const void* src; void* M; void* GA; void* GV; int d, low, chi_b, hi; };
template <class T> void launch_small_svd_prepare(hipStream_t s, const SmallSvdItem* d_items, int nitems);
void launch_small_svd_finish(hipStream_t s, const SmallSvdItem* d_items, int nitems);
__host__ __device__ inline double rank_tau(bool f32_state, int n) { return f32_state ? 1e-12 : 4.0 * (double)n * 2.220446049250313e-16; }
struct CholItem { const void* G; void* L; void* Winv; int n; int* fail; double tau; double shift; };
struct TallSvdItem { const void* A; void* G; const void* L; void* R0; void* Rrot; int m, n; };
struct SmallGemmItem { const void* A; const void* B; void* C; int m, n, k; };
struct CopyItem { const void* src; void* dst; size_t n16; };
bool rowgemm_covers(const FiberItem& it);
void rowgemm_tiles(FiberItem& it);
int plan_rowgemm(FiberItem* it, int n, int cap, int* nwg = nullptr, int tpw = 0);
void launch_mfma_rowgemm(hipStream_t s, const FiberItem* d_items, int nitems, int total_wgs, int D, int K, double* d_norm_partials);
bool launch_x3_gram64(hipStream_t s, const GramItem* d_items, int nitems, int total_chunks, int KKmax);
void launch_x3_rowgemm64(hipStream_t s, const FiberItem* d_items, int nitems, int total_wgs, int D, double* d_norm_partials);
void launch_tall_gram(hipStream_t s, const TallSvdItem* d_items, int nitems, int nmax);
void launch_tall_rt(hipStream_t s, const TallSvdItem* d_items, int nitems);
void launch_tall_w(hipStream_t s, const TallSvdItem* d_items, int nitems, int nmax);
void launch_tall_mj(hipStream_t s, const SmallGemmItem* d_items, int nitems);
void launch_copy_items(hipStream_t s, const CopyItem* d_items, int nitems);
void launch_chol(hipStream_t s, const CholItem* d_items, int nitems, int nmax);
void launch_chol_packed(hipStream_t s, const CholItem* d_items, int nitems, int nmax);
template <class T> void launch_recover_v(hipStream_t s, const RecoverItem* d_items, int nitems, int nmax);
void launch_recover_v_mfma(hipStream_t s, const RecoverItem* d_items, int nitems, int nmax);
template <class T> void launch_env_prepare(hipStream_t s, const EnvItem* d_items, int nitems);
template <class T> void launch_env_finish(hipStream_t s, const EnvFinishItem* d_items, int nitems);
template <class T> void launch_gate_theta(hipStream_t s, const GateItem* d_items, int nitems);
template <class T> void launch_gate_theta_mm(hipStream_t s, const GateItem* d_items, int nitems);
template <class T> void launch_gate_finish(hipStream_t s, const GateItem* d_items, int nitems);
template <class T> void launch_diag(hipStream_t s, const DiagItem* d_items, int nitems);
template <class T> void launch_scale(hipStream_t s, const ScaleItem* d_items, int nitems);
void launch_norm_factor(hipStream_t s, const NormFactorItem* d_items, int nitems);
template <class T> void launch_permute(hipStream_t s, const PermItem& item);
template <class T> void launch_identity(hipStream_t s, void* out, int n);
template <class T> void launch_random_fill(hipStream_t s, void* out, size_t n, unsigned long long seed, double scale, bool real_only);
void launch_sum_doubles(hipStream_t s, const double* in, int n, double* out);
int plan_site_prob(size_t n, int d);
template <class T> void launch_site_prob_partial(hipStream_t s, const void* tabs, const void* psi, size_t n, int d, int nblocks, double* d_partial);
void launch_site_draw(hipStream_t s, const double* d_partial, int nblocks, int d, double neg_tol, const double* d_uniform, unsigned long long seed,
                      unsigned long long sample, unsigned long long step, bool draw, double* d_p, int* d_x, double* d_px, int* d_status);
template <class T> void launch_site_project(hipStream_t s, const void* psi, void* out, size_t nout, int d, const int* d_x, int x_host);
struct LoopGemmItem { const void* A; const void* B; void* C; int m, n, k, opB; int I0, J0; long long si0, si1, sj0, sj1;
                      int tile_begin, ntm, ntn; };
int plan_loop_cgemm(LoopGemmItem* it, int n);
template <class T> void launch_loop_cgemm(hipStream_t s, const LoopGemmItem* d_items, int nitems, int total_tiles);
struct LoopProjItem { void* T; const void* f; const void* b; int nr, nc; int wg_begin; };
int plan_loop_antiproject(LoopProjItem* it, int n);
template <class T> void launch_loop_antiproject(hipStream_t s, const LoopProjItem* d_items, int nitems, int total_wgs);
struct LoopTraceItem { const void* X; const void* Y; int p, q; double* partial; double* out; int wg_begin, nwg; };
int plan_loop_trace(LoopTraceItem* it, int n);
template <class T> void launch_loop_trace(hipStream_t s, const LoopTraceItem* d_items, int nitems, int total_wgs);
void launch_site1_c64(hipStream_t s, const Site1Item* d_items, int nitems, int nbx, double* d_norm_partials);

struct PairGeom { long long cstr, sx, sy, t0, t1, t2; int n0, n1, n2; };
struct PairItem {
    const void* in; void* out; const void* Mx; const void* My;
    PairGeom g;
    int slice_begin;
    int spw;
};
struct PairGramItem {
    const void* X; const void* Y; const void* M; void* partial;
    PairGeom g;
    int wg_begin;
    int spw;
};

struct PlaneGeom { long long cstr, sx, sy, t0, t1, t2, t3; int n0, n1, n2, n3; int nslices() const { return n0 * n1 * n2 * n3; } };
inline bool plane_geometry(int d, int z, const int* chi, int lx, int ly, int DIM, PlaneGeom& g) {
    if (lx == ly || lx < 0 || ly < 0 || lx >= z || ly >= z || chi[lx] != DIM || chi[ly] != DIM) return false;
    auto pre = [&](int j) { long long p = d; for (int i = 0; i < j; ++i) p *= chi[i]; return p; };
    const int p = lx < ly ? lx : ly, q = lx < ly ? ly : lx;
    g.sx = pre(lx); g.sy = pre(ly);
    g.n1 = g.n2 = g.n3 = 1; g.t1 = g.t2 = g.t3 = 0;
    if (pre(p) % 16 == 0) {
        g.cstr = 2; g.n0 = (int)(pre(p) / 16); g.t0 = 16;
        g.n1 = (int)(pre(q) / (pre(p) * DIM)); g.t1 = pre(p) * DIM;
        long long post = 1; for (int i = q + 1; i < z; ++i) post *= chi[i];
        g.n2 = (int)post; g.t2 = pre(q) * DIM;
        return true;
    }
    if (pre(p) != 2) return false;
    int a = -1;
    for (int i = 0; i < z; ++i) if (i != p && i != q && chi[i] % 8 == 0) { a = i; break; }
    if (a < 0) return false;
    g.cstr = pre(a); g.n0 = chi[a] / 8; g.t0 = 8 * pre(a);
    int k = 0;
    for (int i = 0; i < z; ++i) {
        if (i == p || i == q || i == a) continue;
        if (k == 0) { g.n1 = chi[i]; g.t1 = pre(i); } else if (k == 1) { g.n2 = chi[i]; g.t2 = pre(i); } else if (k == 2) { g.n3 = chi[i]; g.t3 = pre(i); } else return false;
        ++k;
    }
    return true;
}
inline bool pair_geometry(int d, int z, const int* chi, int lx, int ly, PairGeom& g) {
// ... 51 lines not shown
```

### tensornetworkquantumsimulator.jl_amd/csrc/kernels_chi64.hip

```cpp
#include <stdexcept>
#include "kernels.hpp"
#include "launch_util.hpp"
#include "mfma_common.hpp"

namespace tnqs {

template <bool M3>
__global__ __launch_bounds__(256, 2) void mfma_gram64_kernel(const GramItem* __restrict__ items, int nitems) {
    constexpr int TR = 64, TRP = TR + 4, NU = 8;
    extern __shared__ __attribute__((aligned(16))) char smem[];
    float* const Xr = reinterpret_cast<float*>(smem);
    float* const Xi = Xr + 64 * TRP;
    float* const Yr = Xi + 64 * TRP;
    float* const Yi = Yr + 64 * TRP;
    const int tid = threadIdx.x;
    int lo = 0, hi = nitems - 1;
    const int gc = blockIdx.x;
    while (lo < hi) { int mid = (lo + hi + 1) >> 1; if (items[mid].chunk_begin <= gc) lo = mid; else hi = mid - 1; }
    const GramItem it = items[lo];
    const int lc = gc - it.chunk_begin;
    const int D = it.D, K = it.K, TA = it.TA, TB = it.TB, KK = D * K;
    const long long PA = it.PA;
    const bool same = (it.X == it.Y);
    const cf* __restrict__ Xg = reinterpret_cast<const cf*>(it.X);
// ... 334 lines not shown
        const cf* p = in + base_in(t) + lane_in + kst * (h + 2 * HL * hf);
        if (D == 1) {
#pragma unroll
            for (int j = 0; j < HL; ++j) { const v2f v = ldg2(p + kst * 2 * j); hb[hf][2 * j] = v[0]; hb[hf][2 * j + 1] = v[1]; }
        } else {
#pragma unroll
            for (int j = 0; j < HL; ++j) { const v4f v = ldg4(p + kst * 2 * j);
                                           hb[hf][4 * j] = v[0]; hb[hf][4 * j + 1] = v[1]; hb[hf][4 * j + 2] = v[2]; hb[hf][4 * j + 3] = v[3]; }
        }
    };
    double nrm = 0;
    int t = t_begin + w;
    if (t < t_end) { issue_half(t, 0); issue_half(t, 1); }
    for (; t < t_end; t += 4) {
        CAcc32<M3> C[NB];
#pragma unroll
        for (int hf = 0; hf < 2; ++hf) {
#pragma unroll
            for (int q = 0; q < HQ; ++q) {
                const float br = hb[hf][2 * q], bi = hb[hf][2 * q + 1];
                const float bd = M3 ? bi - br : bi, bs = M3 ? br + bi : -bi;
#pragma unroll
                for (int nb = 0; nb < NB; ++nb) {
                    const v2f a = Xl[((q + HQ * hf) * NB + nb) * 64 + lane];
                    if (hf == 0 && q == 0) C[nb].template mac_bpre<true>(a[0], a[1], br, bd, bs);
                    else C[nb].template mac_bpre<false>(a[0], a[1], br, bd, bs);
                }
            }
            __builtin_amdgcn_sched_barrier(0);
            if (t + 4 < t_end) issue_half(t + 4, hf);
        }
#pragma unroll
        for (int nb = 0; nb < NB; ++nb) C[nb].finish();
        float nf = 0.f;
        if (D == 1) {
            cf* p = out + base_out(t) + lane_out;
#pragma unroll
            for (int nb = 0; nb < NB; ++nb)
#pragma unroll
                for (int r = 0; r < 16; ++r) {
                    const int n = 32 * nb + (r & 3) + 8 * (r >> 2) + 4 * h;
                    if (n < No) { cf v; v.re = C[nb].a[r]; v.im = C[nb].b[r]; stgc(p + PA * n, v); nf += v.re * v.re + v.im * v.im; }
                }
        } else {
            cf* p = out + base_out(t) + lane_out;
#pragma unroll
            for (int nb = 0; nb < NB; ++nb)
#pragma unroll
                for (int r = 0; r < 16; r += 2) {
                    const int nn = 32 * nb + (r & 3) + 8 * (r >> 2) + 4 * h;
                    const int n = nn >> 1;
                    if (n < No) {
                        v4f v = {C[nb].a[r], C[nb].b[r], C[nb].a[r + 1], C[nb].b[r + 1]};
                        stg4(p + 2 * PA * n, v);
                        nf += v[0] * v[0] + v[1] * v[1] + v[2] * v[2] + v[3] * v[3];
                    }
                }
        }
        nrm += (double)nf;
    }
    if (it.want_norm) {
        nrm = wave_sum(nrm);
        if (lane == 0) sh_red[w] = nrm;
        __syncthreads();
        if (tid == 0) norm_partials[gw] = sh_red[0] + sh_red[1] + sh_red[2] + sh_red[3];
    }
}
static int rowgemm_variant(const FiberItem& it) {
    if (it.D != it.Do || (it.D != 1 && it.D != 2) || it.No < 1 || it.No > it.K) return -1;
    if (it.K == 64) return it.D == 1 ? 0 : 1;
    if (it.K == 32) return it.D == 1 ? 2 : 3;
    return -1;
}
bool rowgemm_covers(const FiberItem& it) {
    if (it.PA >= 32) { if (it.PA % 32 != 0) return false; }
    else if (it.PA < 1 || 32 % it.PA != 0 || it.PB % (32 / it.PA) != 0) return false;
    return rowgemm_variant(it) >= 0;
}
void rowgemm_tiles(FiberItem& it) {
    it.TA = 32; it.TB = 1;
    if (it.PA >= 32) { it.nta = it.PA / 32; it.ntb = it.PB; } else { it.nta = 1; it.ntb = it.PB / (32 / it.PA); }
}
int plan_rowgemm(FiberItem* it, int n, int cap, int* nwg, int tpw) {
    if (tpw <= 0) { double t = 0; for (int i = 0; i < n; ++i) t += (double)it[i].nta * it[i].ntb; tpw = (int)std::max(4.0, std::min((double)cap, t / 2048.0)); tpw &= ~3; }
    return lay_out(it, n, &FiberItem::tile_begin, nwg, [&](FiberItem& f) { f.tpw = tpw; return (f.nta * f.ntb + tpw - 1) / tpw; });
}
template <int KB, int NB, int D> static void launch_rowgemm_t(hipStream_t s, const FiberItem* d_items, int nitems, int total_wgs, double* d_norm_partials) {
    const size_t lds = (size_t)(16 * KB) * NB * 64 * sizeof(v2f);
    constexpr bool fits3 = KB * NB <= 4;
    if (fits3) {
        set_max_dynamic_lds((const void*)mfma_rowgemm_kernel<KB, NB, D, fits3>, lds);
        hipLaunchKernelGGL((mfma_rowgemm_kernel<KB, NB, D, fits3>), dim3(total_wgs), dim3(256), lds, s, d_items, nitems, d_norm_partials);
    } else {
        set_max_dynamic_lds((const void*)mfma_rowgemm_kernel<KB, NB, D, false>, lds);
        hipLaunchKernelGGL((mfma_rowgemm_kernel<KB, NB, D, false>), dim3(total_wgs), dim3(256), lds, s, d_items, nitems, d_norm_partials);
    }
    TNQS_CHECK_LAUNCH();
}
void launch_mfma_rowgemm(hipStream_t s, const FiberItem* d_items, int nitems, int total_wgs, int D, int K, double* d_norm_partials) {
    if (total_wgs <= 0) return;
    if (D * K == 64 && mfma_use_x3()) { launch_x3_rowgemm64(s, d_items, nitems, total_wgs, D, d_norm_partials); return; }
    if (K == 64 && D == 1) launch_rowgemm_t<2, 2, 1>(s, d_items, nitems, total_wgs, d_norm_partials);
    else if (K == 64 && D == 2) launch_rowgemm_t<4, 4, 2>(s, d_items, nitems, total_wgs, d_norm_partials);
    else if (K == 32 && D == 1) launch_rowgemm_t<1, 1, 1>(s, d_items, nitems, total_wgs, d_norm_partials);
    else if (K == 32 && D == 2) launch_rowgemm_t<2, 2, 2>(s, d_items, nitems, total_wgs, d_norm_partials);
    else throw std::runtime_error("launch_mfma_rowgemm: shape not covered");
}

template <bool ROW, int DIAGJ, bool M3>
__device__ __forceinline__ void gram128_set(const float* __restrict__ Xr, const float* __restrict__ Xi, int TRP, int l15, int kq, int P, int q0, int q1, int q2,
                                            v4d& r0, v4d& r1, v4d& r2, v4d& i0, v4d& i1, v4d& i2, v4d& c0, v4d& c1, v4d& c2) {
    const int Q[3] = {q0, q1, q2};
    v4d r[3] = {r0, r1, r2}, i[3] = {i0, i1, i2}, c[3] = {c0, c1, c2};
    gram_f64_shared<3, ROW, DIAGJ, M3>(Xr, Xi, TRP, l15, kq, P, Q, r, i, c);
    r0 = r[0]; r1 = r[1]; r2 = r[2]; i0 = i[0]; i1 = i[1]; i2 = i[2]; c0 = c[0]; c1 = c[1]; c2 = c[2];
}
template <bool M3, bool SHARED>
__global__ __launch_bounds__(256) void mfma_gram128_f64_kernel(const GramItem* __restrict__ items, int nitems) {
    constexpr int TR = 64, TRP = TR + 4, NU = 16, KKP = 128, NBW = 9;
    extern __shared__ __attribute__((aligned(16))) char smem[];
    float* const Xbuf = reinterpret_cast<float*>(smem);
    const int tid = threadIdx.x;
    int lo = 0, hi = nitems - 1;
    const int gc = blockIdx.x;
    while (lo < hi) { int mid = (lo + hi + 1) >> 1; if (items[mid].chunk_begin <= gc) lo = mid; else hi = mid - 1; }
    const GramItem it = items[lo];
    const int lc = gc - it.chunk_begin;
    const int D = it.D, K = it.K, TA = it.TA, TB = it.TB, KK = D * K;
    const long long PA = it.PA;
    const cf* __restrict__ Xg = reinterpret_cast<const cf*>(it.X);
    const int ntiles = it.nta * it.ntb;
    const int t_begin = lc * it.tiles_per_chunk;
    const int t_end = min(ntiles, t_begin + it.tiles_per_chunk);
    const int lane = tid & 63, w = tid >> 6, l15 = lane & 15, kq = lane >> 4;
    const int nb = (KK + 15) >> 4, nblk = nb * (nb + 1) / 2;
    int bI[NBW], bJ[NBW]; bool bOn[NBW];
#pragma unroll
    for (int q = 0; q < NBW; ++q) {
        int idx = w + 4 * q; bOn[q] = idx < nblk;
        int I = 0, rem = bOn[q] ? idx : 0; while (rem >= nb - I) { rem -= nb - I; ++I; }
        bI[q] = I; bJ[q] = I + rem;
    }
    if (SHARED) {
        const int rI[9] = {0, 1, 3, 4, 6, 7, 0, 3, 6}, rJ[9] = {7, 7, 7, 7, 7, 7, 6, 6, 6};
#pragma unroll
        for (int q = 0; q < NBW; ++q) {
            bOn[q] = true;
            if (w < 3) { const int st = q / 3, k = q % 3; bI[q] = st == 1 ? w + 3 : w; bJ[q] = st == 0 ? w + k : (st == 1 ? w + 3 + k : w + 3 + k); }
            else { bI[q] = rI[q]; bJ[q] = rJ[q]; }
        }
    }
    v4d Cr[NBW], Ci[NBW], Cc[NBW];
#pragma unroll
    for (int q = 0; q < NBW; ++q)
#pragma unroll
        for (int r = 0; r < 4; ++r) { Cr[q][r] = 0.0; Ci[q][r] = 0.0; Cc[q][r] = 0.0; }
    for (int e = tid; e < 4 * KKP * TRP; e += 256) Xbuf[e] = 0.f;
    const TileMap m = make_map(tid, D, TA, TB, PA, K);
    const long long kstride = (long long)D * PA;
    const bool fast = m.U <= 256 && (K + m.KP - 1) / m.KP <= NU;
    v4f px[NU];
    auto tile_origin = [&](int t, int& a0, int& b0, int& na, int& nbb) {
        int ta = t % it.nta, tb = t / it.nta;
        a0 = ta * TA; b0 = tb * TB; na = min(TA, it.PA - a0); nbb = min(TB, it.PB - b0);
    };
    const bool straight = fast && m.active && m.vec == 2 && K == m.KP * NU;
    auto issue_loads = [&](int t) {
// ... 124 lines not shown
```

Baseline: 6635.

## Pipeline consecutive two-site gate batches across streams with held site commits

Adds a pipelined route for two-site gate batches. Batch planning (gram chunk counts, rowgemm tiles) is pinned up front, the theta/SVD chain is enqueued, and site replacements are held and committed later, so the next batch's host-side planning and device work can overlap the previous batch's readback instead of synchronizing after each one. A second stream and events are added, and arena wraps are forbidden while pipelining. This adds complexity, risks an error when the staging arena is too small, and falls back to the eigen path when a Cholesky fails.

```diff
diff --git a/include/tnqs_debug.h b/include/tnqs_debug.h
--- a/include/tnqs_debug.h
+++ b/include/tnqs_debug.h
@@ -56,6 +56,7 @@
 int tnqs_dbg_diag(int dtype, int nitems, const int* chi, const double* S, void* out, int guard);
 int tnqs_dbg_cscale(int dtype, int nitems, const int* len, const void* src, const double* re, const double* im, void* dst, int guard);
 int tnqs_dbg_pending_scale(tnqs_handle h, int v, double* factor);
+int tnqs_dbg_pipelined_batches(long long* count);
 #ifdef __cplusplus
 }
 #endif
diff --git a/tensornetworkquantumsimulator.jl_amd/csrc/api.cpp b/tensornetworkquantumsimulator.jl_amd/csrc/api.cpp
--- a/tensornetworkquantumsimulator.jl_amd/csrc/api.cpp
+++ b/tensornetworkquantumsimulator.jl_amd/csrc/api.cpp
@@ -314,5 +314,6 @@
 int tnqs_dbg_cscale(int dtype, int nitems, const int* len, const void* src, const double* re, const double* im, void* dst, int guard_elems) {
     return guard([&] { dbg_cscale(dtype, nitems, len, src, re, im, dst, guard_elems); });
 }
+int tnqs_dbg_pipelined_batches(long long* count) { return guard([&] { if (!count) throw Err(TNQS_ERR_INVALID, "dbg_pipelined_batches: null output"); *count = pipelined_batches(); }); }
 int tnqs_dbg_pending_scale(tnqs_handle h, int v, double* factor) { return guard([&] { if (!factor) throw Err(TNQS_ERR_INVALID, "dbg_pending_scale: null output"); *factor = dbg_pending_scale(S(h), v); }); }
 }
diff --git a/tensornetworkquantumsimulator.jl_amd/csrc/engine.hpp b/tensornetworkquantumsimulator.jl_amd/csrc/engine.hpp
--- a/tensornetworkquantumsimulator.jl_amd/csrc/engine.hpp
+++ b/tensornetworkquantumsimulator.jl_amd/csrc/engine.hpp
@@ -133,6 +133,7 @@
     std::shared_ptr<Pool> pool;
     hipStream_t stream = nullptr; bool own_stream = false;
     hipStream_t aux_stream = nullptr; hipEvent_t ev_fork = nullptr, ev_join = nullptr;
+    hipEvent_t ev_pipe[7] = {}; bool in_pipe = false; hipStream_t pipe_stream = nullptr;
     int rank = 0, nranks = 1; std::vector<int> owner; tnqs_allgather_fn ag_fn = nullptr; void* ag_ctx = nullptr;
     void* exch = nullptr; size_t exch_bytes = 0;
     std::shared_ptr<RcclComm> comm;
@@ -182,6 +183,7 @@
 void sample_bp(State* s, int nsamples, const tnqs_bp_opts* bp, uint64_t seed, const double* uniforms, int32_t* out_config, double* out_prob, tnqs_apply_stats* stats);
 void loop_weights(State* s, int ncycles, const int32_t* cycle_len, const int32_t* cycle_verts, double* out_re_im);
 void prof_collect(State* s);
+long long pipelined_batches();
 void materialize_pending_all(State* s);
 void rccl_unique_id(void* out128);
 void set_sharding_rccl(State* s, int rank, int nranks, const int32_t* owner, const void* unique_id128, int64_t exch_bytes);
diff --git a/tensornetworkquantumsimulator.jl_amd/csrc/engine_batch.cpp b/tensornetworkquantumsimulator.jl_amd/csrc/engine_batch.cpp
--- a/tensornetworkquantumsimulator.jl_amd/csrc/engine_batch.cpp
+++ b/tensornetworkquantumsimulator.jl_amd/csrc/engine_batch.cpp
@@ -220,7 +220,7 @@
     if (!tall.empty()) svd_tall(s, tall);
 }
 
-template <class T, class Acc> void run_grams(State* s, std::vector<GramJob>& jobs, int cls) {
+template <class T, class Acc> void run_grams(State* s, std::vector<GramJob>& jobs, int cls, int plan_items) {
     if (jobs.empty()) return;
     const size_t esz = s->esz();
     size_t KKmax = 1;
@@ -252,7 +252,7 @@
         bytes += (j.X == j.Y ? 1.0 : 2.0) * j.sd.n * esz; flops += gauge ? 8.0 * j.sd.n * (j.KK + (r == GramRoute::Gauge32 ? 16.0 : 32.0)) : 8.0 * j.sd.n * j.KK * (j.M ? 2.0 : 1.0);
     }
     std::vector<int> npart(jobs.size());
-    const int chunks = plan_gram(items.data(), (int)items.size(), r, f32_acc64, 0, npart.data());
+    const int chunks = plan_gram(items.data(), (int)items.size(), r, f32_acc64, plan_items > 0 ? gram_max_chunks(plan_items, f32_acc64) : 0, npart.data());
     for (size_t q = 0; q < jobs.size(); ++q) {
         GramJob& j = jobs[q];
         j.nchunks = npart[q];
@@ -268,8 +268,8 @@
 template void run_chains<double>(State*, std::vector<Chain>&, int, int);
 template void svd_batch<float>(State*, const std::vector<JacobiItem>&, bool);
 template void svd_batch<double>(State*, const std::vector<JacobiItem>&, bool);
-template void run_grams<float, float>(State*, std::vector<GramJob>&, int);
-template void run_grams<float, double>(State*, std::vector<GramJob>&, int);
-template void run_grams<double, double>(State*, std::vector<GramJob>&, int);
-
-}
+template void run_grams<float, float>(State*, std::vector<GramJob>&, int, int);
+template void run_grams<float, double>(State*, std::vector<GramJob>&, int, int);
+template void run_grams<double, double>(State*, std::vector<GramJob>&, int, int);
+
+}
diff --git a/tensornetworkquantumsimulator.jl_amd/csrc/engine_core.cpp b/tensornetworkquantumsimulator.jl_amd/csrc/engine_core.cpp
--- a/tensornetworkquantumsimulator.jl_amd/csrc/engine_core.cpp
+++ b/tensornetworkquantumsimulator.jl_amd/csrc/engine_core.cpp
@@ -138,9 +138,10 @@
 State::~State() {
     if (own_stream && stream) (void)hipStreamSynchronize(stream);
     if (aux_stream) (void)hipStreamSynchronize(aux_stream);
+    if (pipe_stream) (void)hipStreamSynchronize(pipe_stream);
     keepalive.clear(); site.clear(); msg.clear();
     HostArena ar = arena; arena = HostArena{};
-    SpareStream st[2] = {{device, 0, (own_stream && stream) ? stream : nullptr}, {device, 0, aux_stream}};
+    SpareStream st[3] = {{device, 0, (own_stream && stream) ? stream : nullptr}, {device, 0, aux_stream}, {device, 1, pipe_stream}};
     {
         std::lock_guard<std::mutex> lk(g_recycle_mu);
         if (ar.base && g_spare_arenas.size() < kMaxSpares) { ar.off = 0; g_spare_arenas.push_back(ar); ar.base = nullptr; }
@@ -149,6 +150,11 @@
     if (ar.base) arena_free(ar);
     for (auto& q : st) if (q.st) (void)hipStreamDestroy(q.st);
     for (hipEvent_t e : {ev_fork, ev_join}) if (e) (void)hipEventDestroy(e);
+    for (hipEvent_t e : ev_pipe) if (e) (void)hipEventDestroy(e);
+}
+hipStream_t pipe_stream_of(State* s) {
+    if (!s->pipe_stream) s->pipe_stream = acquire_stream(s->device, 1);
+    return s->pipe_stream;
 }
 hipStream_t aux_stream_of(State* s) {
     if (!s->aux_stream) {
diff --git a/tensornetworkquantumsimulator.jl_amd/csrc/engine_gates.cpp b/tensornetworkquantumsimulator.jl_amd/csrc/engine_gates.cpp
--- a/tensornetworkquantumsimulator.jl_amd/csrc/engine_gates.cpp
+++ b/tensornetworkquantumsimulator.jl_amd/csrc/engine_gates.cpp
@@ -1,4 +1,5 @@
 #include "engine_internal.hpp"
+#include <atomic>
 
 namespace tnqs {
 
@@ -45,8 +46,10 @@
     materialize_pending(s, all);
 }
 
+struct HeldSite { int v; Buf site, scale; bool set_scale;
+                  void commit(State* s) const { s->site[v] = site; if (set_scale) s->sscale[v] = scale; } };
 template <class T> static void norm_and_replace(State* s, const std::vector<int>& verts, const std::vector<Buf>& outs, const Buf& norm_partials,
-                                                const std::vector<int>& tile_begin, const std::vector<int>& ntiles, bool normalize) {
+                                                const std::vector<int>& tile_begin, const std::vector<int>& ntiles, bool normalize, std::vector<HeldSite>* hold = nullptr) {
     if (normalize) {
         std::vector<NormFactorItem> nf;
         Buf fac = dalloc(s, verts.size() * 256);
@@ -57,9 +60,9 @@
         }
         const NormFactorItem* d = upload_small(s, nf);
         { ProfScope ps(s, TNQS_PROF_SMALL, 0, 0); launch_norm_factor(s->stream, d, (int)nf.size()); }
-        for (size_t i = 0; i < verts.size(); ++i) { s->site[verts[i]] = outs[i]; s->sscale[verts[i]] = sub_buffer(fac, 256 * i, 8); }
+        for (size_t i = 0; i < verts.size(); ++i) { const HeldSite h{verts[i], outs[i], sub_buffer(fac, 256 * i, 8), true}; if (hold) hold->push_back(h); else h.commit(s); }
     } else {
-        for (size_t i = 0; i < verts.size(); ++i) s->site[verts[i]] = outs[i];
+        for (size_t i = 0; i < verts.size(); ++i) { const HeldSite h{verts[i], outs[i], nullptr, false}; if (hold) hold->push_back(h); else h.commit(s); }
     }
 }
 
@@ -241,6 +244,11 @@
     { ProfScope ps(s, TNQS_PROF_JACOBI, 0, 0); launch_jacobi<double>(s->stream, dj, (int)ji.size(), 60, jacobi_lds(lds), mmax_of(ji)); }
 }
 
+struct BatchPins {
+    int gram_items[3] = {0, 0, 0};
+    double rg_tiles[2] = {0, 0};
+    size_t KKmax = 1, NNmax = 1;
+};
 enum class ReadRoute { deferred, one_trip, two_trips };
 
 template <class T> struct TwoSiteBatch {
@@ -270,7 +278,8 @@
     ReadRoute route = ReadRoute::two_trips;
     RgPlan spec_plan;
     std::vector<const double*> Sptr; Buf S_keep;
-    std::vector<Chain> pch;
+    std::vector<Chain> pch; bool pch_built = false;
+    const BatchPins* pins = nullptr; std::vector<HeldSite> held;
 
     TwoSiteBatch(State* st, const std::vector<Gate2>& gates_in, const tnqs_apply_opts& o, double* e, bool allow_spec)
         : s(st), g(*st->g), ao(o), errs(e), esz(st->esz()), sharded(st->sharded()), qr2(!F32 && use_qr2()), ng((int)gates_in.size()) {
@@ -337,7 +346,8 @@
         { ProfScope ps(s, TNQS_PROF_SMALL, 0, 0); launch_env_finish<T>(s->stream, df, (int)fi.size()); }
     }
 
-    void gauge() {
+    void gauge() { plan_gauge(); run_gauge(); }
+    void plan_gauge() {
         for (size_t i = 0; i < sj.size(); ++i) if (sj[i].owned) own_idx.push_back((int)i);
         chains.resize(own_idx.size());
         fused_M.assign(own_idx.size(), nullptr);
@@ -351,6 +361,8 @@
             const bool legs16 = j.sd.n >= (size_t)(1u << 14) && gauge_gram32_covers(j.sd.d, j.sd.z, j.sd.chi.data(), j.bleg, c.steps[0].first);
             if (bulk || legs16) { fused_M[q] = c.steps[0].second; c.steps.erase(c.steps.begin()); }
         }
+    }
+    void run_gauge() {
         if (!may_defer) settle(s, true);
         run_chains<T>(s, chains, TNQS_PROF_GATE_MODEPROD);
         GA.resize(sj.size()); GV.resize(sj.size()); GW.resize(sj.size()); is_chol.assign(sj.size(), 0); is_small.assign(sj.size(), 0); small_done.assign(sj.size(), 0);
@@ -366,12 +378,18 @@
         sji.push_back(JacobiItem{M->p, nullptr, n, (int)Nout, nullptr});
     }
 
+    bool small_early(size_t q) const { return !sharded && small_shape(own_idx[q]) && !fused_M[q]; }
+    int gram_group(size_t q) const {
+        if (small_early(q)) return -1;
+        const SiteJob& j = sj[own_idx[q]];
+        return !fused_M[q] ? 2 : j.sd.chi[j.bleg] == 16 ? 1 : 0;
+    }
     void early_small_svd() {
         if (sharded) return;
         std::vector<SmallSvdItem> si; std::vector<JacobiItem> sji;
         for (size_t q = 0; q < own_idx.size(); ++q) {
             const size_t i = own_idx[q];
-            if (!small_shape(i) || fused_M[q]) continue;
+            if (!small_early(q)) continue;
             const int n = nof(i);
             GA[i] = dalloc(s, (size_t)n * n * 16); GV[i] = dalloc(s, (size_t)n * n * 16); GW[i] = GV[i]; is_small[i] = 1; small_done[i] = 1;
             add_small_svd(i, si, sji);
@@ -407,9 +425,9 @@
                 if (jobs[q].M && jobs[q].sd.chi[jobs[q].leg] == 16) { jf16.push_back(jobs[q]); idf16.push_back(q); }
                 else if (jobs[q].M) { jf.push_back(jobs[q]); idf.push_back(q); } else { jp.push_back(jobs[q]); idp.push_back(q); }
             }
-            run_grams<T, double>(s, jf, TNQS_PROF_GATE_GRAM);
-            run_grams<T, double>(s, jf16, TNQS_PROF_GATE_GRAM);
-            run_grams<T, double>(s, jp, TNQS_PROF_GATE_GRAM);
+            run_grams<T, double>(s, jf, TNQS_PROF_GATE_GRAM, pins ? pins->gram_items[0] : 0);
+            run_grams<T, double>(s, jf16, TNQS_PROF_GATE_GRAM, pins ? pins->gram_items[1] : 0);
+            run_grams<T, double>(s, jp, TNQS_PROF_GATE_GRAM, pins ? pins->gram_items[2] : 0);
             for (size_t q = 0; q < jf.size(); ++q) jobs[idf[q]] = jf[q];
             for (size_t q = 0; q < jf16.size(); ++q) jobs[idf16[q]] = jf16[q];
             for (size_t q = 0; q < jp.size(); ++q) jobs[idp[q]] = jp[q];
@@ -632,16 +650,22 @@
         { ProfScope ps(s, TNQS_PROF_SMALL, 0, 0); launch_gate_finish<T>(s->stream, d_gitems, npg); }
     }
 
+    void take_results() {
+        if (npg) { const int* a = rb.info_of(st_all); const double* b = rb.terr_of(st_all);
+                   std::copy(a, a + (size_t)npg * 8, hinfo.begin()); std::copy(b, b + npg, hterr.begin()); }
+    }
+    void take_flags() {
+        if (!envs.empty()) std::copy(rb.env_of(st_all), rb.env_of(st_all) + 2 * envs.size(), h_flags.begin());
+        if (!sj.empty()) std::copy(rb.chol_of(st_all), rb.chol_of(st_all) + sj.size(), h_cholfail.begin());
+    }
     void read_results() {
         st_all = readback<char>(s, d_rb->p, rb.total);
         HIPCHK(hipStreamSynchronize(s->stream)); drained(s);
-        if (npg) { const int* a = rb.info_of(st_all); const double* b = rb.terr_of(st_all);
-                   std::copy(a, a + (size_t)npg * 8, hinfo.begin()); std::copy(b, b + npg, hterr.begin()); }
+        take_results();
     }
     void read_and_settle() {
         read_results();
-        if (!envs.empty()) std::copy(rb.env_of(st_all), rb.env_of(st_all) + 2 * envs.size(), h_flags.begin());
-        if (!sj.empty()) std::copy(rb.chol_of(st_all), rb.chol_of(st_all) + sj.size(), h_cholfail.begin());
+        take_flags();
         settle(s, true);
     }
     void retheta() {
@@ -746,11 +770,32 @@
         s->stats.n_spec_batches += 1;
     }
 
-    void theta_svd(HostTimer& ht_a, HostTimer& ht_s4) {
+    void begin_theta() {
         if (ev_small) { HIPCHK(hipStreamWaitEvent(s->stream, ev_small, 0)); ev_small = nullptr; }
         run_theta();
         info.assign(8 * (size_t)ng, 0); terr.assign(ng, 0.0);
         hinfo.assign(8 * (size_t)std::max(1, npg), 0); hterr.assign(std::max(1, npg), 0.0);
+    }
+    static bool sized_from_bounds(const State* s, const std::vector<Gate2>& gs) {
+        for (auto& g2 : gs) {
+            const int chi = s->chi[s->g->edge(g2.v1, g2.v2)], a = s->d[g2.v1] * s->d[g2.v1] * chi, b = s->d[g2.v2] * s->d[g2.v2] * chi;
+            if (!(jacobi_lds(jacobi_lds_bytes(std::max(a, b), std::min(a, b), false, s->esz())) > 0 && std::max(a, b) <= 256)) return false;
+        }
+        return true;
+    }
+    void enqueue_chain() {
+        begin_theta();
+        route = ReadRoute::one_trip;
+        svd_and_finish(nullptr);
+        if (ao.maxdim > 0) spec_plan = plan_epilogue([&](int gi) { return ws[gi].cap; }, [&](size_t q) { return (const void*)s->site[sj[own_idx[q]].v]->p; }, nullptr);
+        st_all = readback<char>(s, d_rb->p, rb.total);
+    }
+    void await_chain() {
+        take_results(); take_flags();
+        if (chol_failures()) { redo_with_eigen(); svd_and_finish(hinfo.data()); read_results(); }
+    }
+    void theta_svd(HostTimer& ht_a, HostTimer& ht_s4) {
+        begin_theta();
         bool one_trip = (!qr2 || may_defer) && npg > 0;
         for (int q = 0; q < npg && one_trip; ++q) {
             const int gi = pg[q];
@@ -845,6 +890,45 @@
         }
     }
 
+    bool rg_shape(size_t q, int chin, FiberItem& it) const {
+        const SiteJob& j = sj[own_idx[q]];
+        it.D = j.sd.d; it.PA = (int)(j.sd.pre(j.bleg) / j.sd.d); it.K = j.sd.chi[j.bleg]; it.PB = (int)j.sd.post(j.bleg); it.Do = j.sd.d; it.No = chin;
+        return F32 && use_mfma() && rowgemm_covers(it) && it.D == 2 && !(it.K == 64 && !use_chi64());
+    }
+    int cap_of(int gi) const {
+        const SiteJob& a = sj[2 * gi]; const SiteJob& b = sj[2 * gi + 1]; const int chi = a.sd.chi[a.bleg];
+        int cap = std::min(a.sd.d * a.sd.d * chi, b.sd.d * b.sd.d * chi); if (ao.maxdim > 0) cap = std::min(cap, ao.maxdim);
+        return cap;
+    }
+    template <class ChiOf> void epilogue_demand(ChiOf chi_of, BatchPins& P) const {
+        for (size_t q = 0; q < own_idx.size(); ++q) {
+            const size_t i = own_idx[q]; const int chin = chi_of((int)i / 2);
+            P.KKmax = std::max<size_t>(P.KKmax, (size_t)sj[i].sd.d * sj[i].sd.chi[sj[i].bleg]); P.NNmax = std::max<size_t>(P.NNmax, (size_t)sj[i].sd.d * chin);
+            FiberItem it{};
+            if (!rg_shape(q, chin, it)) continue;
+            rowgemm_tiles(it); P.rg_tiles[it.K == 64 ? 0 : 1] += (double)it.nta * it.ntb;
+        }
+    }
+    bool rg_stable() const {
+        for (size_t q = 0; q < own_idx.size(); ++q) { FiberItem it{}; const int gi = (int)own_idx[q] / 2; if (!rg_shape(q, cap_of(gi), it) || cap_of(gi) > it.K) return false; }
+        return true;
+    }
+    void build_pch() {
+        if (pch_built) return;
+        pch_built = true; pch.resize(own_idx.size());
+        for (size_t q = 0; q < own_idx.size(); ++q) {
+            const SiteJob& j = sj[own_idx[q]];
+            Chain& c = pch[q]; c.v = j.v; c.src = s->site[j.v]->p; c.sd = j.sd;
+            for (size_t e = 0; e < j.env_idx.size(); ++e)
+                if (!h_flags[2 * j.env_idx[e]]) c.steps.push_back({j.env_leg[e], envs[j.env_idx[e]].prj});
+        }
+    }
+    bool spec_holds() {
+        build_pch();
+        bool ok = spec_plan.valid;
+        for (size_t q = 0; q < own_idx.size() && ok; ++q) { const int gi = (int)own_idx[q] / 2; ok = info[8 * gi + 2] == ws[gi].cap && pch[q].steps.empty(); }
+        return ok;
+    }
     template <class ChiOf, class InOf> RgPlan plan_epilogue(ChiOf chi_of, InOf in_of, std::vector<char>* skip) {
         RgPlan P; P.via.assign(own_idx.size(), 0);
         std::vector<FiberItem> rg; std::vector<int> rverts; std::vector<Buf> routs;
@@ -853,8 +937,7 @@
                 if (skip && (*skip)[q]) continue;
                 size_t i = own_idx[q]; int gi = (int)i / 2; int chin = chi_of(gi); const SiteJob& j = sj[i];
                 FiberItem it{};
-                it.D = j.sd.d; it.PA = (int)(j.sd.pre(j.bleg) / j.sd.d); it.K = j.sd.chi[j.bleg]; it.PB = (int)j.sd.post(j.bleg); it.Do = j.sd.d; it.No = chin;
-                if (!rowgemm_covers(it) || it.D != 2 || (it.K == 64 && !use_chi64())) continue;
+                if (!rg_shape(q, chin, it)) continue;
                 const size_t nout = j.sd.n / it.K * chin;
                 Buf out = dalloc(s, nout * esz);
                 it.in = in_of(q); it.out = out->p; it.X = (i & 1) ? ws[gi].X2->p : ws[gi].X1->p;
@@ -867,7 +950,7 @@
             for (size_t q = 0; q < rg.size(); ++q) if (rg[q].K == kk) { G.sub.push_back(rg[q]); G.sv.push_back(rverts[q]); G.so.push_back(routs[q]); }
             if (G.sub.empty()) continue;
             G.snt.resize(G.sub.size());
-            G.wgs = tnqs::plan_rowgemm(G.sub.data(), (int)G.sub.size(), 32, G.snt.data());
+            G.wgs = tnqs::plan_rowgemm(G.sub.data(), (int)G.sub.size(), 32, G.snt.data(), pins ? rowgemm_tpw(pins->rg_tiles[kk == 64 ? 0 : 1], 32) : 0);
             for (auto& it : G.sub) G.stb.push_back(it.tile_begin);
             G.npr = dalloc(s, (size_t)G.wgs * sizeof(double));
             G.d = upload(s, G.sub);
@@ -877,14 +960,8 @@
         return P;
     }
 
-    void epilogue() {
-        pch.resize(own_idx.size());
-        for (size_t q = 0; q < own_idx.size(); ++q) {
-            const SiteJob& j = sj[own_idx[q]];
-            Chain& c = pch[q]; c.v = j.v; c.src = s->site[j.v]->p; c.sd = j.sd;
-            for (size_t e = 0; e < j.env_idx.size(); ++e)
-                if (!h_flags[2 * j.env_idx[e]]) c.steps.push_back({j.env_leg[e], envs[j.env_idx[e]].prj});
-        }
+    void epilogue(bool may_use_spec = true) {
+        build_pch();
         run_chains<T>(s, pch, TNQS_PROF_GATE_MODEPROD);
         if (own_idx.empty()) return;
         std::vector<FiberItem> items; std::vector<int> verts, tb, nt; std::vector<Buf> outs;
@@ -894,13 +971,15 @@
             KKmax = std::max<size_t>(KKmax, (size_t)sj[i].sd.d * sj[i].sd.chi[sj[i].bleg]);
             NNmax = std::max<size_t>(NNmax, (size_t)sj[i].sd.d * info[8 * (i / 2) + 2]);
         }
+        if (pins) { KKmax = pins->KKmax; NNmax = pins->NNmax; }
+        std::vector<HeldSite>* hold = pins ? &held : nullptr;
         int TR = pick_TR(KKmax, esz, 1);
         bool mf = false;
         if (F32 && use_mfma() && KKmax >= 8) { int t = mfma_fiber_tile_rows((int)KKmax, (int)NNmax); if (t > 0) { TR = t; mf = true; } }
         const bool f64mf = !F32 && use_mfma() && KKmax >= 4 && KKmax <= 64 && NNmax <= 64;
         std::vector<char> via64(own_idx.size(), 0);
         {
-            bool spec_ok = spec_plan.valid;
+            bool spec_ok = spec_plan.valid && may_use_spec;
             for (size_t q = 0; q < own_idx.size() && spec_ok; ++q) { const int gi = (int)own_idx[q] / 2; spec_ok = info[8 * gi + 2] == ws[gi].cap && pch[q].steps.empty() && pch[q].result == s->site[sj[own_idx[q]].v]->p; }
             RgPlan fresh_plan;
             if (!spec_ok) {
@@ -911,7 +990,7 @@
             bool booked = false;
             for (auto& G : P.groups) {
                 { ProfScope ps(s, TNQS_PROF_GATE_APPLY, booked ? 0.0 : P.rby, booked ? 0.0 : P.rfl); booked = true; launch_mfma_rowgemm(s->stream, G.d, (int)G.sub.size(), G.wgs, 2, G.kk, reinterpret_cast<double*>(G.npr->p)); }
-                norm_and_replace<T>(s, G.sv, G.so, G.npr, G.stb, G.snt, ao.normalize_tensors != 0);
+                norm_and_replace<T>(s, G.sv, G.so, G.npr, G.stb, G.snt, ao.normalize_tensors != 0, hold);
             }
         }
         for (size_t q = 0; q < own_idx.size(); ++q) {
@@ -940,7 +1019,7 @@
           if (f64mf) launch_mfma_fiber_gemm_f64(s->stream, d, (int)items.size(), tiles, (int)KKmax, (int)NNmax, reinterpret_cast<double*>(np->p), true);
           else if (mf) launch_mfma_fiber_gemm(s->stream, d, (int)items.size(), tiles, (int)KKmax, (int)NNmax, reinterpret_cast<double*>(np->p));
           else launch_fiber_gemm<T>(s->stream, d, (int)items.size(), tiles, TR, (int)KKmax, reinterpret_cast<double*>(np->p)); }
-        norm_and_replace<T>(s, verts, outs, np, tb, nt, ao.normalize_tensors != 0);
+        norm_and_replace<T>(s, verts, outs, np, tb, nt, ao.normalize_tensors != 0, hold);
     }
 
     void bond_messages() {
@@ -962,9 +1041,121 @@
     }
 };
 
+static std::atomic<long long> g_pipelined_batches{0};
+long long pipelined_batches() { return g_pipelined_batches.load(); }
+
+constexpr int kPipeMinBulkSitesPerHalf = 96;
+constexpr size_t kPipeBulkElems = size_t(1) << 21;
+constexpr size_t kPipeStagingPerGate = size_t(32) << 10;
+
+template <class T> static bool pipeline_applies(State* s, const std::vector<Gate2>& gates, bool deferred) {
+    if (!std::is_same<T, float>::value || !use_batch_pipeline() || s->sharded() || gates.size() < 2) return false;
+    const bool forced = force_batch_pipeline();
+    if (deferred && !forced) return false;
+    if (!TwoSiteBatch<T>::sized_from_bounds(s, gates)) return false;
+    const size_t nA = (gates.size() + 1) / 2;
+    std::set<int> chis, ds;
+    for (auto& g2 : gates) for (int v : {g2.v1, g2.v2}) { ds.insert(s->d[v]); for (int e : s->g->nbr_e[v]) chis.insert(s->chi[e]); }
+    const bool uniform = chis.size() == 1 && ds.size() == 1;
+    std::set<std::vector<int>> shapes[2]; int bulk[2] = {0, 0};
+    for (size_t k = 0; k < gates.size(); ++k) for (int side = 0; side < 2; ++side) {
+        const int v = side ? gates[k].v2 : gates[k].v1, w = side ? gates[k].v1 : gates[k].v2; const Graph& g = *s->g;
+        const int bleg = g.leg(v, w);
+        std::vector<int> sh;
+        if (uniform) { int nmsg = 0; for (size_t l = 0; l < g.nbr[v].size(); ++l) if ((int)l != bleg && s->msg[g.dedge(g.nbr[v][l], v)]) ++nmsg; sh = {(int)g.nbr[v].size(), nmsg}; }
+        else { sh = {s->d[v], bleg}; for (size_t l = 0; l < g.nbr[v].size(); ++l) { sh.push_back(s->chi[g.nbr_e[v][l]]); sh.push_back(s->msg[g.dedge(g.nbr[v][l], v)] ? 1 : 0); } }
+        shapes[k < nA ? 0 : 1].insert(std::move(sh));
+        if (site_nelem(s, v) >= kPipeBulkElems) bulk[k < nA ? 0 : 1] += 1;
+    }
+    if (shapes[0] != shapes[1]) return false;
+    if (!forced && std::min(bulk[0], bulk[1]) < kPipeMinBulkSitesPerHalf) return false;
+    if (!s->arena.base) s->arena = acquire_arena();
+    return gates.size() * kPipeStagingPerGate + (size_t(1) << 20) <= s->arena.cap;
+}
+
+struct PipeRegion {
+    State* s; hipStream_t main, side; hipEvent_t* ev;
+    enum { kFork, kEnvB, kFactorA, kReadA, kFactorB, kReadB, kJoin };
+    explicit PipeRegion(State* st) : s(st), main(st->stream), side(pipe_stream_of(st)), ev(st->ev_pipe) {
+        for (int k = 0; k < 7; ++k) if (!ev[k]) HIPCHK(hipEventCreateWithFlags(&ev[k], hipEventDisableTiming));
+        record(kFork); wait(side, kFork);
+        s->pool->set_defer(true); s->in_pipe = true;
+    }
+    void on(hipStream_t st) { s->stream = st; s->prof->chain = false; }
+    void record(int k) { HIPCHK(hipEventRecord(ev[k], s->stream)); }
+    void wait(hipStream_t st, int k) { HIPCHK(hipStreamWaitEvent(st, ev[k], 0)); }
+    void join() { on(side); record(kJoin); on(main); wait(main, kJoin); }
+    ~PipeRegion() {
+        s->stream = main; s->prof->chain = false;
+        (void)hipEventRecord(ev[kJoin], side); (void)hipStreamWaitEvent(main, ev[kJoin], 0);
+        s->in_pipe = false; s->pool->set_defer(false);
+    }
+};
+
+template <class T> static void apply_two_site_batch_pipelined(State* s, const std::vector<Gate2>& gates_in, const tnqs_apply_opts& ao, double* errs) {
+    const size_t nA = (gates_in.size() + 1) / 2;
+    const std::vector<Gate2> ga(gates_in.begin(), gates_in.begin() + (std::ptrdiff_t)nA), gb(gates_in.begin() + (std::ptrdiff_t)nA, gates_in.end());
+    PhaseScope phase_scope(s, TNQS_PROF_PHASE_GATE_BATCH);
+    g_pipelined_batches += 1;
+    reserve_readback(s, gates_in.size() * kPipeStagingPerGate + (size_t(1) << 20));
+    BatchPins pins;
+    PipeRegion reg(s);
+    TwoSiteBatch<T> A(s, ga, ao, errs, false), B(s, gb, ao, errs, false);
+    A.pins = B.pins = &pins;
+    using R = PipeRegion;
+    auto status_check = [](const TwoSiteBatch<T>& h) { for (int gi = 0; gi < h.ng; ++gi) if (h.info[8 * gi + 3] != 0) throw Err(TNQS_ERR_NUMERIC, "simple_update: internal bond capacity exceeded"); };
+    if (!ao.normalize_tensors) { A.materialize_inputs(); B.materialize_inputs(); }
+    A.environments();
+    reg.on(reg.side); B.environments(); reg.record(R::kEnvB); reg.on(reg.main);
+    A.plan_gauge(); B.plan_gauge();
+    for (auto* h : {&A, &B}) {
+        for (size_t q = 0; q < h->own_idx.size(); ++q) { const int grp = h->gram_group(q); if (grp >= 0) pins.gram_items[grp] += 1; }
+        h->epilogue_demand([&](int gi) { return h->cap_of(gi); }, pins);
+    }
+    const bool rg_stable = A.rg_stable() && B.rg_stable();
+    A.run_gauge();
+    A.early_small_svd();
+    A.grams(); A.factor_G(use_chol());
+    A.gate_items();
+    reg.record(R::kFactorA);
+    reg.on(reg.side); reg.wait(reg.side, R::kFactorA);
+    A.enqueue_chain(); reg.record(R::kReadA);
+    reg.on(reg.main); reg.wait(reg.main, R::kEnvB);
+    B.run_gauge(); B.early_small_svd();
+    B.grams(); B.factor_G(use_chol());
+    B.gate_items();
+    reg.record(R::kFactorB);
+    HIPCHK(hipEventSynchronize(reg.ev[R::kReadA])); s->prof->chain = false;
+    reg.on(reg.side);
+    A.await_chain(); A.book_results(); A.share_records(); status_check(A);
+    reg.wait(reg.side, R::kFactorB);
+    B.enqueue_chain(); reg.record(R::kReadB);
+    const bool early = rg_stable && A.spec_holds();
+    reg.on(reg.main);
+    if (early) A.epilogue();
+    HIPCHK(hipEventSynchronize(reg.ev[R::kReadB])); s->prof->chain = false;
+    reg.on(reg.side);
+    B.await_chain(); B.book_results(); B.share_records(); status_check(B);
+    reg.join();
+    const bool both_spec = A.spec_holds() && B.spec_holds();
+    if (!early) {
+        pins.rg_tiles[0] = pins.rg_tiles[1] = 0; pins.KKmax = pins.NNmax = 1;
+        for (auto* h : {&A, &B}) h->epilogue_demand([&](int gi) { return h->info[8 * gi + 2]; }, pins);
+        A.epilogue(both_spec);
+    } else {
+        BatchPins dims; for (auto* h : {&A, &B}) h->epilogue_demand([&](int gi) { return h->info[8 * gi + 2]; }, dims);
+        pins.KKmax = dims.KKmax; pins.NNmax = dims.NNmax;
+    }
+    B.epilogue(both_spec || rg_stable);
+    for (auto* h : {&A, &B}) for (const HeldSite& hs : h->held) hs.commit(s);
+    A.bond_messages(); B.bond_messages();
+    soft_sync(s);
+}
+
 template <class T> static void apply_two_site_batch(State* s, const std::vector<Gate2>& gates_in, const tnqs_apply_opts& ao, double* errs, bool allow_spec = false) {
     if (gates_in.empty()) return;
     TwoSiteBatch<T> b(s, gates_in, ao, errs, allow_spec);
+    if (pipeline_applies<T>(s, gates_in, b.may_defer)) { apply_two_site_batch_pipelined<T>(s, gates_in, ao, errs); return; }
     PhaseScope phase_scope(s, TNQS_PROF_PHASE_GATE_BATCH);
     HostTimer ht_a(3);
     if (!ao.normalize_tensors) b.materialize_inputs();
diff --git a/tensornetworkquantumsimulator.jl_amd/csrc/engine_internal.hpp b/tensornetworkquantumsimulator.jl_amd/csrc/engine_internal.hpp
--- a/tensornetworkquantumsimulator.jl_amd/csrc/engine_internal.hpp
+++ b/tensornetworkquantumsimulator.jl_amd/csrc/engine_internal.hpp
@@ -36,6 +36,8 @@
 TNQS_SWITCH(use_small_svd, !envflag("TNQS_NO_SMALLSVD"))
 TNQS_SWITCH(defer_site1, !envflag("TNQS_NO_DEFER_1SITE"))
 TNQS_SWITCH(use_chi64, !envflag("TNQS_NO_CHI64"))
+TNQS_SWITCH(use_batch_pipeline, !envflag("TNQS_NO_BATCH_PIPELINE"))
+TNQS_SWITCH(force_batch_pipeline, envflag("TNQS_FORCE_BATCH_PIPELINE"))
 TNQS_SWITCH(speculation_on, !envflag("TNQS_NO_SPECULATION"))
 #undef TNQS_SWITCH
 inline size_t bp_cache_budget() { static const size_t v = [] { const char* e = std::getenv("TNQS_BP_CACHE_MB"); return (e ? (size_t)std::atoll(e) : (size_t)49152) << 20; }(); return v; }
@@ -52,6 +54,7 @@
 };
 
 void sync(State* s);
+hipStream_t pipe_stream_of(State* s);
 hipStream_t aux_stream_of(State* s);
 void recycle_arena(HostArena ar);
 HostArena acquire_arena();
@@ -59,13 +62,14 @@
     HIPCHK(hipStreamSynchronize(s->stream));
     if (s->aux_stream && s->aux_stream != s->stream) HIPCHK(hipStreamSynchronize(s->aux_stream));
 }
+inline void arena_wrap_allowed(const State* s) { if (s->in_pipe) throw Err(TNQS_ERR_UNSUPPORTED, "internal: the staging reserved for a pipelined gate batch did not suffice (TNQS_NO_BATCH_PIPELINE=1 selects the single-batch route)"); }
 template <class X> const X* readback(State* s, const void* dsrc, size_t count) {
     const size_t bytes = count * sizeof(X);
     HostArena& ar = s->arena;
     if (!ar.base) ar = acquire_arena();
     const size_t aligned = (std::max<size_t>(bytes, 1) + 255) & ~size_t(255);
     if (aligned > ar.cap) throw Err(TNQS_ERR_UNSUPPORTED, "read-back too large for the staging arena");
-    if (ar.off + aligned > ar.cap) { drain_for_arena_reuse(s); ar.off = 0; }
+    if (ar.off + aligned > ar.cap) { arena_wrap_allowed(s); drain_for_arena_reuse(s); ar.off = 0; }
     char* h = ar.base + ar.off; ar.off += aligned;
     if (bytes) HIPCHK(hipMemcpyAsync(h, dsrc, bytes, hipMemcpyDeviceToHost, s->stream));
     return reinterpret_cast<const X*>(h);
@@ -74,11 +78,12 @@
     HostArena& ar = s->arena;
     if (!ar.base) ar = acquire_arena();
     if (bytes > ar.cap) throw Err(TNQS_ERR_UNSUPPORTED, "read-backs of one batch too large for the staging arena");
-    if (ar.off + bytes > ar.cap) { drain_for_arena_reuse(s); ar.off = 0; }
+    if (ar.off + bytes > ar.cap) { arena_wrap_allowed(s); drain_for_arena_reuse(s); ar.off = 0; }
 }
 inline void soft_sync(State* s) { s->keep_mark = s->keepalive.size(); }
 inline void drained(State* s) {
     s->prof->chain = false;
+    if (s->in_pipe) return;
     s->arena.off = 0;
     if (s->keep_mark) { s->keepalive.erase(s->keepalive.begin(), s->keepalive.begin() + (std::ptrdiff_t)std::min(s->keep_mark, s->keepalive.size())); s->keep_mark = 0; }
 }
@@ -99,7 +104,7 @@
     if (!ar.base) ar = acquire_arena();
     size_t aligned = (bytes + 255) & ~size_t(255);
     if (aligned > ar.cap) throw Err(TNQS_ERR_UNSUPPORTED, "descriptor batch too large");
-    if (ar.off + aligned > ar.cap) { drain_for_arena_reuse(s); ar.off = 0; s->prof->chain = false; }
+    if (ar.off + aligned > ar.cap) { arena_wrap_allowed(s); drain_for_arena_reuse(s); ar.off = 0; s->prof->chain = false; }
     char* h = ar.base + ar.off; ar.off += aligned;
     std::memcpy(h, v.data(), bytes);
     Buf b = dalloc(s, bytes);
@@ -115,7 +120,7 @@
     if (!ar.base) ar = acquire_arena();
     const size_t aligned = (bytes + 255) & ~size_t(255);
     if (aligned > ar.cap) throw Err(TNQS_ERR_UNSUPPORTED, "descriptor batch too large");
-    if (ar.off + aligned > ar.cap) { drain_for_arena_reuse(s); ar.off = 0; s->prof->chain = false; }
+    if (ar.off + aligned > ar.cap) { arena_wrap_allowed(s); drain_for_arena_reuse(s); ar.off = 0; s->prof->chain = false; }
     char* h = ar.base + ar.off; ar.off += aligned;
     std::memcpy(h, v.data(), bytes);
     return reinterpret_cast<const Item*>(h);
@@ -208,7 +213,7 @@
 };
 
 template <class T> void run_chains(State* s, std::vector<Chain>& chains, int cls, int cls_pair = -1);
-template <class T, class Acc> void run_grams(State* s, std::vector<GramJob>& jobs, int cls);
+template <class T, class Acc> void run_grams(State* s, std::vector<GramJob>& jobs, int cls, int plan_items = 0);
 template <class T> void svd_batch(State* s, const std::vector<JacobiItem>& all, bool with_v);
 void svd_tall(State* s, const std::vector<JacobiItem>& tall, int* d_fail = nullptr, int* d_polish_sweeps = nullptr);
 template <class T> void bp_update_t(State* s, const tnqs_bp_opts* o, int* niter_out, double* diff_out, bool optimistic = false, int iters_before = 0);
diff --git a/tensornetworkquantumsimulator.jl_amd/csrc/kernels.hip b/tensornetworkquantumsimulator.jl_amd/csrc/kernels.hip
--- a/tensornetworkquantumsimulator.jl_amd/csrc/kernels.hip
+++ b/tensornetworkquantumsimulator.jl_amd/csrc/kernels.hip
@@ -174,7 +174,7 @@
     return r == GramRoute::Generic ? tr : r == GramRoute::F64In ? 32 : 64;
 }
 int plan_gram(GramItem* it, int n, GramRoute r, bool f32_acc64, int max_chunks, int* npart) {
-    if (max_chunks <= 0) max_chunks = std::max(1, (f32_acc64 ? 1024 : 2048) / n);
+    if (max_chunks <= 0) max_chunks = gram_max_chunks(n, f32_acc64);
     const int per_chunk = (r == GramRoute::Mfma32 || r == GramRoute::Fused32) ? 4 : (r == GramRoute::F64x64 || r == GramRoute::Gauge64) ? 2 : 1;
     const int chunks = lay_out(it, n, &GramItem::chunk_begin, npart, [&](GramItem& g) {
         const int ntiles = g.nta * g.ntb, nch = std::min(max_chunks, ntiles);
diff --git a/tensornetworkquantumsimulator.jl_amd/csrc/kernels.hpp b/tensornetworkquantumsimulator.jl_amd/csrc/kernels.hpp
--- a/tensornetworkquantumsimulator.jl_amd/csrc/kernels.hpp
+++ b/tensornetworkquantumsimulator.jl_amd/csrc/kernels.hpp
@@ -154,6 +154,7 @@
 enum class GramRoute { Generic, Mfma32, Mfma64, Fused32, F64x64, F64x128, F64In, Gauge64, Gauge32 };
 int gram_tile_rows(GramRoute r, size_t KKmax, size_t esz);
 int plan_gram(GramItem* it, int n, GramRoute r, bool f32_acc64, int max_chunks, int* npart);
+inline int gram_max_chunks(int n, bool f32_acc64) { return std::max(1, (f32_acc64 ? 1024 : 2048) / std::max(1, n)); }
 template <class T, class Acc> void launch_gram_route(hipStream_t s, GramRoute r, const GramItem* d_items, int nitems, int total_chunks, int TR, int KKmax,
                                                      bool all_full = false);
 template <class Acc, class Out> void launch_reduce(hipStream_t s, const ReduceItem* d_items, int nitems, int total_elems);
@@ -175,6 +176,7 @@
 bool rowgemm_covers(const FiberItem& it);
 void rowgemm_tiles(FiberItem& it);
 int plan_rowgemm(FiberItem* it, int n, int cap, int* nwg = nullptr, int tpw = 0);
+inline int rowgemm_tpw(double tiles, int cap) { return (int)std::max(4.0, std::min((double)cap, tiles / 2048.0)) & ~3; }
 void launch_mfma_rowgemm(hipStream_t s, const FiberItem* d_items, int nitems, int total_wgs, int D, int K, double* d_norm_partials);
 bool launch_x3_gram64(hipStream_t s, const GramItem* d_items, int nitems, int total_chunks, int KKmax);
 void launch_x3_rowgemm64(hipStream_t s, const FiberItem* d_items, int nitems, int total_wgs, int D, double* d_norm_partials);
diff --git a/tensornetworkquantumsimulator.jl_amd/csrc/kernels_chi64.hip b/tensornetworkquantumsimulator.jl_amd/csrc/kernels_chi64.hip
--- a/tensornetworkquantumsimulator.jl_amd/csrc/kernels_chi64.hip
+++ b/tensornetworkquantumsimulator.jl_amd/csrc/kernels_chi64.hip
@@ -440,7 +440,7 @@
     if (it.PA >= 32) { it.nta = it.PA / 32; it.ntb = it.PB; } else { it.nta = 1; it.ntb = it.PB / (32 / it.PA); }
 }
 int plan_rowgemm(FiberItem* it, int n, int cap, int* nwg, int tpw) {
-    if (tpw <= 0) { double t = 0; for (int i = 0; i < n; ++i) t += (double)it[i].nta * it[i].ntb; tpw = (int)std::max(4.0, std::min((double)cap, t / 2048.0)); tpw &= ~3; }
+    if (tpw <= 0) { double t = 0; for (int i = 0; i < n; ++i) t += (double)it[i].nta * it[i].ntb; tpw = rowgemm_tpw(t, cap); }
     return lay_out(it, n, &FiberItem::tile_begin, nwg, [&](FiberItem& f) { f.tpw = tpw; return (f.nta * f.ntb + tpw - 1) / tpw; });
 }
 template <int KB, int NB, int D> static void launch_rowgemm_t(hipStream_t s, const FiberItem* d_items, int nitems, int total_wgs, double* d_norm_partials) {
```

Result: slower. 6473 (-2.5%).
